# ActiveVisionLab/gaussctrl

Measured on AMD Instinct MI355X. Metric: edited views/sec @512x512 (ControlNet denoise + splat render+bwd), higher is better.
Workload: dtype bf16

## Files before the change

gaussctrl_amd/csrc/dn_gemm.hip:

```cpp
#include "dn_gemm_kernels.h"

namespace {

struct GemmVariant {
    int force_mt;
    int use8;
    int convsplit;
    bool no_wg2, no_persist, full_epilogue, no_lean_ln, tap_outer;
    int forced_pw, slice_mt, epi_abl;
    int undefined;
};
GemmVariant decode_variant(int kv)
{
    const auto bit = [kv](int b) { return (kv & b) != 0; };
    const auto field = [kv](int mask, int shift) { return (kv & mask) >> shift; };
    constexpr int flags = GC_GEMM_VAR_K4_ONLY | GC_GEMM_VAR_FORCE_K8 | GC_GEMM_VAR_NO_CONV_SLICES | GC_GEMM_VAR_NO_SMALL_CONV_SLICES | GC_GEMM_VAR_NO_WG2 |
                          GC_GEMM_VAR_NO_PERSIST | GC_GEMM_VAR_FULL_EPILOGUE | GC_GEMM_VAR_NO_LEAN_LN | GC_GEMM_VAR_TAP_OUTER;
    return {field(GC_GEMM_VAR_MT_MASK, GC_GEMM_VAR_MT_SHIFT), bit(GC_GEMM_VAR_K4_ONLY) ? 0 : bit(GC_GEMM_VAR_FORCE_K8) ? 2 : 1,
            bit(GC_GEMM_VAR_NO_CONV_SLICES) ? 0 : bit(GC_GEMM_VAR_NO_SMALL_CONV_SLICES) ? 1 : 2,
            bit(GC_GEMM_VAR_NO_WG2), bit(GC_GEMM_VAR_NO_PERSIST), bit(GC_GEMM_VAR_FULL_EPILOGUE), bit(GC_GEMM_VAR_NO_LEAN_LN), bit(GC_GEMM_VAR_TAP_OUTER),
            field(GC_GEMM_VAR_PW_MASK, GC_GEMM_VAR_PW_SHIFT), field(GC_GEMM_VAR_SLICE_MT_MASK, GC_GEMM_VAR_SLICE_MT_SHIFT), field(GC_GEMM_VAR_EPI_ABL_MASK, GC_GEMM_VAR_EPI_ABL_SHIFT),
            kv & ~(flags | GC_GEMM_VAR_MT_MASK | GC_GEMM_VAR_PW_MASK | GC_GEMM_VAR_SLICE_MT_MASK | GC_GEMM_VAR_EPI_ABL_MASK)};
}

int choose_splits(int64_t blocks, int nk)
{
    if (blocks >= 128 || nk < 32) return 1;
    int s = (int)((448 + blocks - 1) / blocks);
    if (s > nk / 8) s = nk / 8;
    if (s > 16) s = 16;
    return s < 2 ? 1 : s;
}

int choose_mt(int64_t M, int64_t N, int ntw, bool forced)
{
    const int64_t nbn = (N + 32 * ntw - 1) / (32 * ntw);
    if (((M + 127) / 128) * nbn < 96 && !forced) return 0;
    int best = 2;
    int64_t best_cost = -1;
    for (int mt = 2; mt <= 4; ++mt) {
        const int64_t tiles = ((M + 64 * mt - 1) / (64 * mt)) * nbn;
        const int64_t cost = ((tiles + 255) / 256) * (mt + 1);
        if (best_cost < 0 || cost < best_cost || (cost == best_cost && mt == 4)) { best = mt; best_cost = cost; }
    }
    return best;
}

int choose_pw(int64_t nbm, int64_t nbn, int64_t total_wgs, int conc, int64_t bm, int64_t bn, bool conv)
{
    int64_t r = total_wgs / 8 < 1 ? 1 : total_wgs / 8;
    if (r > conc) r = conc;
    const int64_t tiles = nbm * nbn;
    if (r >= tiles) return 0;
    const int64_t ca = conv ? bm : 9 * bm, cw = 9 * bn;
    int best = 0;
    int64_t best_cost = -1;
    for (int64_t pw = nbn; pw >= 1; --pw) {
        const int64_t per = nbm * pw;
        const int64_t cols = std::min<int64_t>(nbn, pw * ((r + per - 1) / per)), rows = std::min<int64_t>(nbm, (r + pw - 1) / pw);
        const int64_t cost = rows * ca + cols * cw;
        if (best_cost < 0 || cost < best_cost) { best = pw == nbn ? 0 : (int)pw; best_cost = cost; }
    }
    return best;
}

int pw_of(const gc_gemm_desc *d, const GemmVariant &v, int64_t nbm, int64_t nbn, int64_t total_wgs, int conc, int64_t bm, int64_t bn)
{
    if (v.forced_pw) return v.forced_pw - 1;
    return choose_pw(nbm, nbn, total_wgs, conc, bm, bn, d->mode == 1);
}

void plan(const gc_gemm_desc *d, int *ntw, int *splits, int *tps)
{
    *ntw = (d->N % 160 == 0 && d->N % 128 != 0 && !d->geglu) ? 5 : 4;
    if (d->softmax_keys > 0) *ntw = 5;
    const int bn = 32 * *ntw;
    const int64_t Msel = d->plan_rows > 0 ? d->plan_rows : d->M;
    const int64_t blocks = ((Msel + BM - 1) / BM) * ((d->N + bn - 1) / bn);
    const int nk = (int)((d->K + BK - 1) / BK);
    *splits = (d->geglu || d->w_set_rows > 0 || d->softmax_keys > 0) ? 1 : choose_splits(blocks, nk);
    *tps = (nk + *splits - 1) / *splits;
    *splits = (nk + *tps - 1) / *tps;
}


struct SelQ { int ntw, mt, splits, tps; };
void select_fp8(const gc_gemm_desc *d, const GemmVariant &v, SelQ *o, bool assume_ws)
{
    const int force_mt = v.force_mt;
    o->ntw = (d->N % 160 == 0 && d->N % 128 != 0 && !d->geglu) ? 5 : 4;
    int mt = force_mt ? force_mt : choose_mt(d->M, d->N, o->ntw, true);
    if (o->ntw == 5) mt = 2; else if (mt > 3) mt = 3;
    if (mt < 2) mt = 2;
    const int nkq = (int)(d->K / 128);
    o->splits = 1; o->tps = nkq;
    const bool plain = !d->geglu && !d->out_t && !d->out_fp8 && !d->out_f32 && d->out && !d->ln_row_stats && !d->out_row_stats && !d->out_group_stats && d->act == 0;
    const int64_t Msel = d->plan_rows > 0 ? d->plan_rows : d->M;
    const int64_t nbn = (d->N + 32 * o->ntw - 1) / (32 * o->ntw), tiles = ((Msel + 127) / 128) * nbn;
    if (plain && !force_mt && v.convsplit && tiles <= 128 && nkq >= 16) {
        int s = (int)std::min<int64_t>(tiles < 96 ? (256 + tiles - 1) / tiles : 256 / tiles, nkq / 8);
        if (s > 16) s = 16;
        if (s >= 2 && (assume_ws || (d->workspace && d->workspace_bytes >= sizeof(float) * (size_t)s * (size_t)d->M * (size_t)d->N))) {
            mt = 2; o->tps = (nkq + s - 1) / s; o->splits = (nkq + o->tps - 1) / o->tps;
        }
    }
    o->mt = mt;
}
}

extern "C" size_t gc_dn_gemm_workspace_bytes(const gc_gemm_desc *d)
{
    if (!d || d->M <= 0 || d->N <= 0 || d->K <= 0) return 0;
    if (d->fp8) {
        if (d->K % 128 != 0) return 0;
        const GemmVariant v = decode_variant(d->kernel_variant);
        SelQ q;
        select_fp8(d, v, &q, true);
        return q.splits > 1 ? sizeof(float) * (size_t)q.splits * (size_t)d->M * (size_t)d->N : 0;
    }
    int ntw, splits, tps;
    plan(d, &ntw, &splits, &tps);
    return splits > 1 ? sizeof(float) * (size_t)splits * (size_t)d->M * (size_t)d->N : 0;
}

namespace {
int ln_lean_kind(const gc_gemm_desc *d, const GemmVariant &v)
{
    if (v.no_lean_ln || d->fp8 || d->mode != 0 || d->K % 64 != 0 || d->out_group_stats || d->out_chan_parts || d->N < 4) return 0;
    if (d->out_row_stats && !d->ln_row_stats)
        return (!d->geglu && d->act == 0 && !d->out_f32 && !d->out_t && d->out && (!d->rowvec || d->rows_per_batch >= 256)) ? 1 : 0;
    if (d->ln_row_stats && !d->out_row_stats) return d->softmax_keys > 0 ? 3 : 2;
    return 0;
}
struct Sel { int mode, ntw, splits, tps, mt8; };
int select(const gc_gemm_desc *d, const GemmVariant &v, Sel *o, bool want_parts)
{
    int mode = 0;
    if (d->mode == 1) mode = (d->Cin % 64 == 0) ? 2 : 1;
    int ntw, splits, tps;
    plan(d, &ntw, &splits, &tps);
    if (splits > 1 && (!d->workspace || d->workspace_bytes < sizeof(float) * (size_t)splits * (size_t)d->M * (size_t)d->N)) {
        splits = 1; tps = (int)((d->K + BK - 1) / BK);
    }
    const int bn = 32 * ntw;
    const int64_t nbn = (d->N + bn - 1) / bn;
    const int nk_host = (int)((d->K + BK - 1) / BK);
    const int force_mt = v.force_mt, use8 = v.use8;
    o->mode = mode; o->ntw = ntw; o->splits = splits; o->tps = tps; o->mt8 = 0;
    if (use8 && d->zeros) {
        const int64_t Msel = d->plan_rows > 0 ? d->plan_rows : d->M;
        int mt = force_mt ? force_mt : choose_mt(Msel, d->N, ntw, use8 == 2);
        if (mt && !force_mt && Msel != d->M) mt = choose_mt(d->M, d->N, ntw, true);
        const int64_t tiles8 = ((Msel + 127) / 128) * nbn;
        const bool small = tiles8 < 96;
        if (!mt && mode == 0 && !force_mt) mt = 2;
        if (mode == 0 && !force_mt && ntw == 4 && d->K % 64 == 0 && !d->geglu && !d->out_t && !v.no_wg2 &&
            (!(d->ln_row_stats || d->out_row_stats || d->out_group_stats) || ln_lean_kind(d, v)) && !want_parts) {
            const int64_t t1 = ((d->M + 63) / 64) * nbn, t2 = ((d->M + 127) / 128) * nbn;
            if (mt == 2 && t2 <= 256 && t1 <= 512 && t1 > 128 && nk_host <= 24) mt = 1;
        }
        if (d->w_set_rows > 0 && mt) {
            int pick = 0;
            const int cand[5] = {mt, 4, 3, 2, (ntw == 4 && d->softmax_keys == 0) ? 1 : 2};
            for (int c = 0; c < 5 && !pick; ++c) if (d->w_set_rows % (64 * cand[c]) == 0) pick = cand[c];
            mt = pick ? pick : mt;
        }
        const bool want_split = !force_mt && use8 != 2 && !d->geglu && d->w_set_rows == 0 && d->softmax_keys == 0 && d->workspace && tiles8 <= 128 && (mode == 0 ? (!small || nk_host >= 24) : (v.convsplit >= (small ? 2 : 1)));
        int s8 = 1, tps8 = nk_host;
        if (want_split) {
            const bool img8 = mode != 0 && !small && d->Ho * d->Wo <= 64 && Msel % 256 == 0;
            const int mts = (v.slice_mt >= 2 && v.slice_mt <= 4) ? v.slice_mt : (img8 ? 4 : ((mode != 0 && !small) ? 3 : 2));
            const int64_t tiles_s = ((Msel + 64 * mts - 1) / (64 * mts)) * nbn;
            s8 = (int)std::min<int64_t>(std::max<int64_t>(256 / tiles_s, 2), nk_host / 12);
            if (s8 >= 2 && d->workspace_bytes >= sizeof(float) * (size_t)s8 * (size_t)d->M * (size_t)d->N) {
                mt = mts; tps8 = (nk_host + s8 - 1) / s8; s8 = (nk_host + tps8 - 1) / tps8;
            } else s8 = 1;
        }
        if (splits > 1 && s8 == 1 && !force_mt && use8 != 2) mt = 0;
        if (mt) { o->mt8 = mt; o->splits = s8; o->tps = tps8; }
    }
    return 0;
}
}

extern "C" int gc_dn_gemm_row_stat_slots(const gc_gemm_desc *d)
{
    if (!d || d->M <= 0 || d->N <= 0 || d->K <= 0) return 0;
    if (d->fp8) { const int ntw = (d->N % 160 == 0 && d->N % 128 != 0) ? 5 : 4; return (int)((d->N + 16 * ntw - 1) / (16 * ntw)); }
    const GemmVariant v = decode_variant(d->kernel_variant);
    Sel sel;
    select(d, v, &sel, false);
    return sel.splits > 1 ? (int)((d->N / 4 + 63) / 64) : (int)((d->N + 16 * sel.ntw - 1) / (16 * sel.ntw));
}

namespace {
void chan_parts_layout(const gc_gemm_desc *d, const GemmVariant &v, const Sel &sel, int64_t *rows, int *nslab, int *col_tile)
{
    *rows = 0; *nslab = 0; *col_tile = 0;
    const int64_t rpb = d->rows_per_batch;
    if (d->fp8) {
        SelQ q;
        select_fp8(d, v, &q, false);
        if (d->K % 128 != 0 || rpb < 256 || rpb % 32 != 0 || d->M % rpb != 0 || d->gn_groups < 1 || d->N % d->gn_groups != 0) return;
        const int64_t cpg = d->N / d->gn_groups;
        if (q.splits > 1) {
            if (cpg > 64) return;
            *rows = CS_RB; *nslab = (int)(rpb / CS_RB); *col_tile = 64;
            return;
        }
        const bool lean = d->mode == 1 && !d->upsample && !d->geglu && !d->out_t && !d->out_fp8 && !d->out_f32 && d->out && d->act == 0 &&
                          !d->ln_row_stats && !d->out_row_stats && !d->out_group_stats;
        const int64_t bm = 64 * q.mt;
        if (!lean || bm > rpb || cpg > 32 * q.ntw) return;
        *rows = bm;
        *nslab = (int)(rpb % bm == 0 ? rpb / bm : (rpb + bm - 1) / bm + 1);
        *col_tile = 32 * q.ntw;
        return;
    }
    if (d->geglu || d->act != 0 || d->out_t || !d->out || d->out_f32 || d->ln_row_stats || d->out_row_stats || d->out_group_stats) return;
    if (rpb < 256 || rpb % 32 != 0 || d->M % rpb != 0) return;
    if (d->gn_groups < 1 || d->N % d->gn_groups != 0) return;
    const int64_t cpg = d->N / d->gn_groups;
    if (sel.splits > 1) {
        if (cpg > 64) return;
        *rows = CS_RB; *nslab = (int)(rpb / CS_RB); *col_tile = 64;
        return;
    }
    if (!sel.mt8) return;
    if ((d->mode == 1 && d->upsample) || (d->mode == 0 && d->K % 64 != 0)) return;
    const int64_t bm = 64 * (sel.mt8 < 2 ? 2 : sel.mt8);
    if (bm > rpb || cpg > 32 * sel.ntw) return;
    *rows = bm;
    *nslab = (int)(rpb % bm == 0 ? rpb / bm : (rpb + bm - 1) / bm + 1);
    *col_tile = 32 * sel.ntw;
}
}

extern "C" int gc_dn_gemm_chan_parts_layout(const gc_gemm_desc *d, int64_t *rows_per_slab, int *nslab, int *col_tile)
{
    GC_REQUIRE(d && rows_per_slab && nslab && col_tile, "null argument");
    *rows_per_slab = 0; *nslab = 0; *col_tile = 0;
    if (d->M <= 0 || d->N <= 0 || d->K <= 0 || d->rows_per_batch <= 0) return GC_OK;
    const GemmVariant v = decode_variant(d->kernel_variant);
    Sel sel;
    select(d, v, &sel, true);
    chan_parts_layout(d, v, sel, rows_per_slab, nslab, col_tile);
    return GC_OK;
}

namespace {
struct Route { Sel sel; int lnk, persist; };
void route(const gc_gemm_desc *d, const GemmVariant &v, Route *r)
{
    Sel &sel = r->sel;
    select(d, v, &sel, d->out_chan_parts != nullptr);
    if (d->out_chan_parts && sel.mt8 == 1) sel.mt8 = 2;
    const bool fuse = d->ln_row_stats || d->out_row_stats || d->out_group_stats;
    r->lnk = (sel.mt8 && sel.splits == 1) ? ln_lean_kind(d, v) : 0;
    r->persist = 0;
    if (sel.mt8 == 4 && sel.ntw == 4 && sel.mode == 0 && sel.splits == 1 && d->K % 64 == 0 && d->K <= 64 * 24 && (!fuse || r->lnk == 2) && !d->out_chan_parts &&
        !d->rowvec && !d->out_t && !d->out_f32 && d->out && d->act != 2 && !v.no_persist) {
        const int64_t tiles = ((d->M + 255) / 256) * ((d->N + 32 * sel.ntw - 1) / (32 * sel.ntw));
        if (tiles > 256) r->persist = 256;
    }
}
}

extern "C" int gc_dn_gemm_selection(const gc_gemm_desc *d, gc_gemm_selection *out)
{
    GC_REQUIRE(d && out, "null argument");
    GC_REQUIRE(d->M > 0 && d->N > 0 && d->K > 0, "empty problem");
    const GemmVariant v = decode_variant(d->kernel_variant);
    if (const int rc = refuse_variant_bits(__func__, v.undefined)) return rc;
    *out = gc_gemm_selection{};
    int64_t rows = 0; int ns = 0, ct = 0;
    if (d->fp8) {
        GC_REQUIRE(d->K % 128 == 0, "fp8: K % 128 == 0");
        SelQ q;
        select_fp8(d, v, &q, false);
        out->kernel = GC_GEMM_SEL_FP8; out->m_tiles = q.mt; out->splits = q.splits; out->ntw = q.ntw;
        if (d->out_chan_parts) {
            chan_parts_layout(d, v, Sel{}, &rows, &ns, &ct);
            out->parts = rows > 0 ? (q.splits > 1 ? 1 : 2) : -1;
        }
        return GC_OK;
    }
    Route r;
    route(d, v, &r);
    out->kernel = !r.sel.mt8 ? GC_GEMM_SEL_K4 : r.sel.splits > 1 ? GC_GEMM_SEL_K8_SLICED : GC_GEMM_SEL_K8;
    out->m_tiles = r.sel.mt8; out->splits = r.sel.splits; out->ntw = r.sel.ntw; out->ln_kind = r.lnk; out->persist = r.persist;
    if (d->out_chan_parts) {
        chan_parts_layout(d, v, r.sel, &rows, &ns, &ct);
        out->parts = rows > 0 ? (r.sel.splits > 1 ? 1 : 2) : -1;
    }
    return GC_OK;
}

extern "C" int gc_dn_gemm(const gc_gemm_desc *d, void *stream)
{
    GC_REQUIRE(d && d->W && d->A, "null descriptor / operand");
    GC_REQUIRE(d->M > 0 && d->N > 0 && d->K > 0, "empty problem");
    GC_REQUIRE(d->K % 8 == 0, "K must be a multiple of 8 (pad channels on the host)");
    GC_REQUIRE(d->N % 4 == 0, "N must be a multiple of 4 (pad output channels on the host)");
    GC_REQUIRE(d->dtype == DT_BF16 || d->dtype == DT_F16, "dtype must be 0 (bf16) or 1 (f16)");
    const GemmVariant v = decode_variant(d->kernel_variant);
    if (const int rc = refuse_variant_bits(__func__, v.undefined)) return rc;
    GemmArgs g;
    g.pw = 0;
    g.M = d->M; g.N = d->N; g.K = d->K; g.A = d->A; g.lda = d->lda;
    g.B = d->B; g.Hi = d->Hi; g.Wi = d->Wi; g.Cin = d->Cin; g.Ho = d->Ho; g.Wo = d->Wo; g.stride = d->stride; g.ups = d->upsample; g.pad = d->pad_lo;
    g.W = d->W; g.bias = d->bias; g.rowvec = d->rowvec; g.ld_rowvec = d->ld_rowvec;
    g.rows_per_batch = d->rows_per_batch > 0 ? d->rows_per_batch : 1;
    g.residual = d->residual; g.ldr = d->ldr; g.out_scale = d->out_scale; g.act = d->act; g.geglu = d->geglu;
    g.out = d->out; g.ldc = d->ldc; g.out_f32 = d->out_f32; g.out_t = d->out_t; g.ldt = d->ldt; g.t_batch_stride = d->t_batch_stride; g.t_col0 = d->t_col0;
    g.row_stats = d->ln_row_stats; g.row_stat_slots = d->ln_row_stat_slots > 0 ? d->ln_row_stat_slots : 1;
    g.colsum = d->ln_colsum; g.ln_eps = d->ln_eps; g.ln_inv_k = 1.f / (float)d->K;
    g.out_row_stats = d->out_row_stats; g.out_group_stats = d->out_group_stats; g.gn_groups = d->gn_groups;
    g.gn_cpg = d->gn_groups > 0 ? (int)(d->N / d->gn_groups) : 1;
    g.w_scale = (const unsigned char *)d->w_scale; g.a_scale = d->a_scale;
    g.out_fp8 = d->out_fp8; g.out_qscale = d->out_fp8 > 0 ? exp2f((float)(127 - d->out_fp8)) : 1.f;
    GC_REQUIRE(d->out_fp8 >= 0 && d->out_fp8 < 255, "out_fp8 must be 0 (off) or an E8M0 byte 1 .. 254");
    GC_REQUIRE(!d->out_fp8 || (d->fp8 && d->mode == 0 && d->out && !d->out_f32 && !d->out_t && !d->out_chan_parts && !d->ln_row_stats && !d->out_row_stats &&
                               !d->out_group_stats && d->ldc % 4 == 0),
               "out_fp8: an fp8 linear with a plain output (no fp32 / transposed output, no statistics, no LayerNorm fold), ldc % 4 == 0");
    g.dbg = v.epi_abl;
    g.conv_korder = v.tap_outer ? 0 : 1;
    g.w_set_rows = d->w_set_rows; g.w_set_stride = d->w_set_stride; g.sm_keys = d->softmax_keys;
    GC_REQUIRE(d->w_set_rows >= 0 && d->softmax_keys >= 0 && d->softmax_keys <= 80, "bad weight-set / softmax arguments");
    GC_REQUIRE(!d->softmax_keys || (d->ln_row_stats && d->N % 80 == 0 && d->out && !d->out_f32 && !d->out_t && !d->geglu && !d->residual && d->act == 0),
               "softmax_keys: a LayerNorm-folded linear with N % 80 == 0 and a plain 2-byte output");
    GC_REQUIRE((d->ln_row_stats == nullptr) == (d->ln_colsum == nullptr), "ln_row_stats and ln_colsum must be given together");
    GC_REQUIRE(!d->ln_row_stats || d->mode == 0, "LayerNorm folding applies to linear GEMMs");
    GC_REQUIRE(!(d->out_row_stats || d->out_group_stats) || (!d->geglu && !d->out_t && d->out), "output statistics need a plain (non-GEGLU, non-transposed) output");
    GC_REQUIRE(!d->out_group_stats || (g.rows_per_batch % 16 == 0 && d->gn_groups >= 1 && d->gn_groups <= GS_MAXG && d->N % d->gn_groups == 0),
               "out_group_stats needs rows_per_batch % 16 == 0 and 1 <= gn_groups <= 32 dividing N");
    if (d->mode == 1) {
        GC_REQUIRE(d->Cin % 8 == 0 && d->K == 9 * (int64_t)d->Cin, "conv3x3: K must be 9*Cin with Cin % 8 == 0");
        GC_REQUIRE(d->M == (int64_t)d->B * d->Ho * d->Wo, "conv3x3: M must be B*Ho*Wo");
        GC_REQUIRE(d->pad_lo == 0 || d->pad_lo == 1, "conv3x3: pad_lo must be 0 or 1");
    } else {
        GC_REQUIRE(d->lda >= d->K && d->lda % 8 == 0, "linear: lda must be >= K and a multiple of 8");
    }
    GC_REQUIRE((d->mode == 1 ? (int64_t)d->B * d->Hi * d->Wi * d->Cin : d->M * d->lda) < ((int64_t)1 << 31) && (int64_t)d->N * d->K < ((int64_t)1 << 31),
               "operand too large for 32-bit element offsets: split the batch");
    if (d->geglu) GC_REQUIRE(d->N % 32 == 0 && !d->out_t, "geglu needs N % 32 == 0");
    GC_REQUIRE(v.force_mt <= 4, "kernel_variant: MT must be 0 .. 4");
    Route rt;
    route(d, v, &rt);
    const Sel &sel = rt.sel;
    g.chan_parts = d->out_chan_parts; g.cp_nslab = 0; g.cp_rows = 0;
    if (d->out_chan_parts) {
        int64_t rows; int ns, ct;
        chan_parts_layout(d, v, sel, &rows, &ns, &ct);
        GC_REQUIRE(rows > 0, "out_chan_parts: this problem cannot produce channel partials (see gc_dn_gemm_chan_parts_layout)");
        g.cp_nslab = ns; g.cp_rows = (int)rows;
    }
    if (fuse_of(g) && sel.mt8) {
        const bool upsampled = d->mode == 1 && d->upsample, ragged = d->mode == 0 && d->K % 64 != 0;
        GC_REQUIRE(!upsampled && !ragged, "row / group statistics and LayerNorm folding: not with upsample-fused convs or K % 64 != 0 linears");
    }
    hipStream_t s = gc::S(stream);
    g.zeros = d->zeros;
    if (d->fp8) {
        GC_REQUIRE(d->zeros && d->w_scale, "fp8: zeros page and per-row weight scales are required");
        GC_REQUIRE(d->K % 128 == 0, "fp8: K % 128 == 0");
        GC_REQUIRE(!(d->geglu || d->out_t) || (d->mode == 0 && !fuse_of(g)), "fp8: GEGLU / transposed output on linears with the plain epilogue only");
        GC_REQUIRE(d->mode == 0 || (d->Cin % 128 == 0 && !d->upsample), "fp8 conv: Cin (padded) % 128 == 0, no fused upsample");
        GC_REQUIRE(d->mode == 1 || d->lda % 16 == 0, "fp8 linear: lda % 16 == 0");
        GC_REQUIRE((int64_t)d->N * d->K < ((int64_t)1 << 31) && (d->mode == 1 ? (int64_t)d->B * d->Hi * d->Wi * d->Cin : d->M * d->lda) < ((int64_t)1 << 31), "fp8: 32-bit offsets");
        SelQ q;
        select_fp8(d, v, &q, false);
        const int ntw = q.ntw, mt = q.mt;
        g.splits = q.splits; g.tiles_per_split = q.tps; g.ws = q.splits > 1 ? (float *)d->workspace : nullptr;
        GC_REQUIRE(!d->out_chan_parts || q.splits > 1 || (d->mode == 1 && !fuse_of(g)), "fp8: channel partials come from k-sliced problems and fast convs");
        const int64_t nbn_q = (d->N + 32 * ntw - 1) / (32 * ntw), nbm_q = (d->M + 64 * mt - 1) / (64 * mt);
        const dim3 gq((unsigned)(nbm_q * nbn_q), (unsigned)q.splits);
        g.pw = pw_of(d, v, nbm_q, nbn_q, nbm_q * nbn_q * q.splits, 32, 64 * mt, 32 * ntw);
        dn_gemm_launch_fp8(g, d->dtype, d->mode == 1 ? 2 : 3, ntw, mt, gq, s);
        if (q.splits > 1) { if (g.chan_parts) dn_gemm_launch_splitk_epilogue_cs(g, d->dtype, s); else dn_gemm_launch_splitk_epilogue(g, d->dtype, s); }
        return gc::check_launch("gc_dn_gemm(fp8)");
    }
    g.splits = sel.splits; g.tiles_per_split = sel.tps; g.ws = (float *)d->workspace;
    const int bn = 32 * sel.ntw;
    const int64_t nbn = (d->N + bn - 1) / bn;
    g.persist = rt.persist;
    const int lnk = rt.lnk;
    if (d->w_set_rows > 0 || d->softmax_keys > 0) {
        GC_REQUIRE(lnk != 0, "weight sets / softmax_keys need a lean LayerNorm-fold problem (K % 64 == 0 linear with ln_row_stats or out_row_stats, no forced variant)");
        GC_REQUIRE(d->w_set_rows == 0 || (d->w_set_rows % (64 * sel.mt8) == 0 && d->M % d->w_set_rows == 0), "w_set_rows must be a multiple of the row tile and divide M");
    }
    if (sel.mt8) {
        const int64_t nbm8 = (d->M + 64 * sel.mt8 - 1) / (64 * sel.mt8);
        const dim3 grid8((unsigned)(nbm8 * nbn), (unsigned)sel.splits);
        g.pw = pw_of(d, v, nbm8, nbn, g.persist ? 8 * 32 : nbm8 * nbn * sel.splits, sel.mt8 == 1 ? 64 : 32, 64 * sel.mt8, bn);
        if (lnk) dn_gemm_launch_ln(g, d->dtype, lnk, lean_of(g, sel.mode) && g.persist == 0, sel.ntw, sel.mt8, grid8, s);
        else if (fuse_of(g)) dn_gemm_launch_fuse(g, d->dtype, sel.mode, sel.ntw, sel.mt8 < 2 ? 2 : sel.mt8, grid8, s);
        else if (g.chan_parts && sel.splits == 1) dn_gemm_launch_cs(g, d->dtype, sel.mode, sel.ntw, sel.mt8, grid8, s);
        else if (lean_of(g, sel.mode) && g.persist == 0 && !v.full_epilogue) dn_gemm_launch_lean(g, d->dtype, sel.mode, sel.ntw, sel.mt8, grid8, s);
        else dn_gemm_launch_plain(g, d->dtype, sel.mode, sel.ntw, sel.mt8, grid8, s);
    } else {
        const int64_t nbm = (d->M + BM - 1) / BM;
        const dim3 grid((unsigned)(nbm * nbn), (unsigned)sel.splits);
        g.pw = pw_of(d, v, nbm, nbn, nbm * nbn * sel.splits, 64, BM, bn);
        if (fuse_of(g)) dn_gemm_launch_fuse(g, d->dtype, sel.mode, sel.ntw, 0, grid, s); else dn_gemm_launch_plain(g, d->dtype, sel.mode, sel.ntw, 0, grid, s);
    }
    if (sel.splits > 1) { if (g.chan_parts) dn_gemm_launch_splitk_epilogue_cs(g, d->dtype, s); else dn_gemm_launch_splitk_epilogue(g, d->dtype, s); }
    return gc::check_launch("gc_dn_gemm");
}
```

gaussctrl_amd/csrc/dn_gemm_kernels.h:

```cpp
#pragma once
#include "dn_common.h"
#include <type_traits>

namespace dng {
struct GemmArgs {
    int64_t M, N, K;
    const void *A; int64_t lda;
    int B, Hi, Wi, Cin, Ho, Wo, stride, ups, pad;
    const void *W;
    const float *bias;
    const float *rowvec; int64_t ld_rowvec; int64_t rows_per_batch;
    const void *residual; int64_t ldr;
    float out_scale;
    int act, geglu;
    void *out; int64_t ldc; int out_f32;
    void *out_t; int64_t ldt; int64_t t_batch_stride; int64_t t_col0;
    int splits; int tiles_per_split;
    int persist;
    float *ws;
    const void *zeros;
    const float *row_stats; int row_stat_slots; const float *colsum; float ln_eps, ln_inv_k;
    float *out_row_stats;
    float *out_group_stats;
    int gn_groups, gn_cpg;
    const unsigned char *w_scale;
    int a_scale;
    int out_fp8; float out_qscale;
    int dbg;
    float *chan_parts; int cp_nslab; int cp_rows;
    int64_t w_set_rows, w_set_stride;
    int pw;
    int sm_keys;
    int conv_korder;
};

__device__ __forceinline__ void tile_coords(int64_t bid, int nbm, int nbn, int pw, int64_t &mblk, int64_t &nblk)
{
    if (pw <= 0 || pw >= nbn) { mblk = bid / nbn; nblk = bid % nbn; return; }
    const int64_t per = (int64_t)nbm * pw, p = bid / per, within = bid - p * per;
    const int64_t w = (nbn - p * pw) < pw ? (nbn - p * pw) : pw;
    mblk = within / w; nblk = p * pw + within % w;
}
__device__ __forceinline__ void wg_tile(const GemmArgs &g, int nbm, int nbn, int64_t &mblk, int64_t &nblk, int &slice)
{
    const int64_t tiles = gridDim.x, total = tiles * gridDim.y, lin = blockIdx.x + tiles * blockIdx.y;
    const int64_t xcd = lin & 7, qq = total >> 3, rr = total & 7;
    const int64_t L = (xcd < rr ? xcd * (qq + 1) : rr * (qq + 1) + (xcd - rr) * qq) + (lin >> 3);
    slice = (int)(L / tiles);
    tile_coords(L - (int64_t)slice * tiles, nbm, nbn, g.pw, mblk, nblk);
}
}

namespace {
using namespace dn;
using dng::GemmArgs;

template <int I, int N, class F> __device__ __forceinline__ void static_for(F &&f)
{
    if constexpr (I < N) {
        f(std::integral_constant<int, I>{});
        static_for<I + 1, N>(f);
    }
}

constexpr int BM = 128, BK = 64;
constexpr int NT = 256;


constexpr int GS_SLOTS = 20, GS_MAXG = 32;

__device__ __forceinline__ float row16_sum(float v)
{
    v += __builtin_bit_cast(float, __builtin_amdgcn_update_dpp(0, __builtin_bit_cast(int, v), 0x128, 0xf, 0xf, false));
    v += __builtin_bit_cast(float, __builtin_amdgcn_update_dpp(0, __builtin_bit_cast(int, v), 0x124, 0xf, 0xf, false));
    v += __builtin_bit_cast(float, __builtin_amdgcn_update_dpp(0, __builtin_bit_cast(int, v), 0x122, 0xf, 0xf, false));
    v += __builtin_bit_cast(float, __builtin_amdgcn_update_dpp(0, __builtin_bit_cast(int, v), 0x121, 0xf, 0xf, false));
    return v;
}

__device__ __forceinline__ int lds_off(int r, int c) { return r * 128 + ((c ^ ((r >> 1) & 7)) << 4); }

template <class T>
__device__ __forceinline__ void epilogue_store(const GemmArgs &g, int64_t m, int64_t n, int64_t on, float *v, const float *gate, const uint2 *res_pre = nullptr)
{
    const int64_t bidx = g.rowvec ? m / g.rows_per_batch : 0;
    if (g.row_stats) {
        float2 rs = make_float2(0.f, 0.f);
        for (int sl = 0; sl < g.row_stat_slots; ++sl) {
            const float2 t = *reinterpret_cast<const float2 *>(g.row_stats + ((int64_t)sl * g.M + m) * 2);
            rs.x += t.x; rs.y += t.y;
        }
        const float mean = rs.x * g.ln_inv_k, rstd = rsqrtf(fmaxf(rs.y * g.ln_inv_k - mean * mean, 0.f) + g.ln_eps);
#pragma unroll
        for (int r = 0; r < 4; ++r) v[r] = rstd * (v[r] - mean * g.colsum[n + r]);
    }
#pragma unroll
    for (int r = 0; r < 4; ++r) {
        if (g.bias) v[r] += g.bias[n + r];
        if (g.rowvec) v[r] += g.rowvec[bidx * g.ld_rowvec + n + r];
    }
    if (g.geglu) {
#pragma unroll
        for (int r = 0; r < 4; ++r) {
            float gt = gate[r];
            if (g.bias) gt += g.bias[n + 16 + r];
            v[r] = v[r] * gelu_erf(gt);
        }
    }
    if (g.act == 1) {
#pragma unroll
        for (int r = 0; r < 4; ++r) v[r] = silu(v[r]);
    } else if (g.act == 2) {
#pragma unroll
        for (int r = 0; r < 4; ++r) v[r] = fminf(fmaxf(v[r] * 0.5f + 0.5f, 0.f), 1.f);
    }
#pragma unroll
    for (int r = 0; r < 4; ++r) v[r] *= g.out_scale;
    if (g.residual) {
        const uint2 rr = res_pre ? *res_pre : *reinterpret_cast<const uint2 *>((const unsigned char *)g.residual + (m * g.ldr + on) * 2);
        v[0] += T::to_f((unsigned short)(rr.x & 0xffff)); v[1] += T::to_f((unsigned short)(rr.x >> 16));
        v[2] += T::to_f((unsigned short)(rr.y & 0xffff)); v[3] += T::to_f((unsigned short)(rr.y >> 16));
    }
    const bool to_t = g.out_t && on >= g.t_col0;
    const uint2 pk = make_uint2(pack2<T>(v[0], v[1]), pack2<T>(v[2], v[3]));
    if (g.out && !(to_t && g.t_col0 > 0)) {
        if (g.out_f32)
            *reinterpret_cast<float4 *>((float *)g.out + m * g.ldc + on) = make_float4(v[0], v[1], v[2], v[3]);
        else
            *reinterpret_cast<uint2 *>((unsigned char *)g.out + (m * g.ldc + on) * 2) = pk;
    }
    if (to_t) {
        const int64_t b = m / g.rows_per_batch, tok = m - b * g.rows_per_batch;
        unsigned short *o = (unsigned short *)g.out_t + b * g.t_batch_stride + tok;
#pragma unroll
        for (int r = 0; r < 4; ++r) o[(on - g.t_col0 + r) * g.ldt] = T::from_f(v[r]);
    }
    if (!g.out_f32) {
        v[0] = T::to_f((unsigned short)(pk.x & 0xffff)); v[1] = T::to_f((unsigned short)(pk.x >> 16));
        v[2] = T::to_f((unsigned short)(pk.y & 0xffff)); v[3] = T::to_f((unsigned short)(pk.y >> 16));
    }
}

template <int BM>
__device__ __forceinline__ void row_stats_prologue(const GemmArgs &g, int64_t m_base, float *srow)
{
    const int t = threadIdx.x, r = t & 255, half = t >> 8;
    if (t < 2 * BM) srow[t] = 0.f;
    asm volatile("s_waitcnt lgkmcnt(0)" ::: "memory");
    __builtin_amdgcn_s_barrier();
    if (r < BM) {
        const int64_t m = m_base + r < g.M ? m_base + r : g.M - 1;
        const float *rp = g.row_stats + m * 2;
        const int64_t st = g.M * 2;
        float sx = 0.f, sy = 0.f;
        int sl = half;
        for (; sl + 6 < g.row_stat_slots; sl += 8) {
            const float2 a = *reinterpret_cast<const float2 *>(rp + sl * st), b = *reinterpret_cast<const float2 *>(rp + (sl + 2) * st);
            const float2 c = *reinterpret_cast<const float2 *>(rp + (sl + 4) * st), d = *reinterpret_cast<const float2 *>(rp + (sl + 6) * st);
            sx += (a.x + b.x) + (c.x + d.x); sy += (a.y + b.y) + (c.y + d.y);
        }
        for (; sl < g.row_stat_slots; sl += 2) {
            const float2 a = *reinterpret_cast<const float2 *>(rp + sl * st);
            sx += a.x; sy += a.y;
        }
        __hip_atomic_fetch_add(srow + 2 * r, sx, __ATOMIC_RELAXED, __HIP_MEMORY_SCOPE_WORKGROUP);
        __hip_atomic_fetch_add(srow + 2 * r + 1, sy, __ATOMIC_RELAXED, __HIP_MEMORY_SCOPE_WORKGROUP);
    }
    asm volatile("s_waitcnt vmcnt(0) lgkmcnt(0)" ::: "memory");
}

template <class T, int NTW, int MT, int NTHREADS>
__device__ __forceinline__ void wave_epilogue(const GemmArgs &g, f32x4 (&acc)[NTW][MT], int64_t m_base, int64_t m_wave, int64_t n_wave, int lane,
// ... 40 lines not shown
        for (int nt = 0; nt < NTW; ++nt) {
            const int64_t n = n_lane + nt * 16;
            const bool okn = okm && n < g.N && !(g.geglu && (nt & 1));
            const int64_t on = g.geglu ? (n_wave + nt * 16) / 2 + fc * 4 : n;
            rs_all[mt][nt] = (g.residual && okn) ? *reinterpret_cast<const uint2 *>((const unsigned char *)g.residual + (mc * g.ldr + on) * 2) : make_uint2(0u, 0u);
        }
    }
    const bool want_cs = g.out_group_stats != nullptr;
    float *red = reinterpret_cast<float *>(smem);
    const int64_t b0 = want_cs ? m_base / g.rows_per_batch : 0;
    float cs[NTW][4], css[NTW][4];
#pragma unroll
    for (int nt = 0; nt < NTW; ++nt)
#pragma unroll
        for (int r = 0; r < 4; ++r) { cs[nt][r] = 0.f; css[nt][r] = 0.f; }
    int64_t cs_b = -1;
    auto flush_cs = [&]() __attribute__((always_inline)) {
        float *rb = red + (cs_b - b0) * (GS_MAXG * 2);
#pragma unroll
        for (int nt = 0; nt < NTW; ++nt) {
            const int64_t n = n_lane + nt * 16;
#pragma unroll
            for (int r = 0; r < 4; ++r) {
                const float a = (g.dbg & 4) ? cs[nt][r] : row16_sum(cs[nt][r]), b = (g.dbg & 4) ? css[nt][r] : row16_sum(css[nt][r]);
                if (fr == 0 && n + r < g.N && !(g.dbg & 2)) {
                    const int gi = (int)(n + r) / g.gn_cpg;
                    __hip_atomic_fetch_add(rb + 2 * gi, a, __ATOMIC_RELAXED, __HIP_MEMORY_SCOPE_WORKGROUP);
                    __hip_atomic_fetch_add(rb + 2 * gi + 1, b, __ATOMIC_RELAXED, __HIP_MEMORY_SCOPE_WORKGROUP);
                }
                cs[nt][r] = 0.f; css[nt][r] = 0.f;
            }
        }
    };
#pragma unroll
    for (int mt = 0; mt < MT; ++mt) {
        const int64_t m = m_wave + mt * 16 + fr;
        const int64_t m_tile = m_wave + mt * 16;
        if (m_tile >= g.M) break;
        const bool okm = m < g.M;
        if (want_cs) {
            const int64_t b = m_tile / g.rows_per_batch;
            if (cs_b >= 0 && b != cs_b) flush_cs();
            cs_b = b;
        }
        const uint2 *rs = rs_all[mt];
        float mean = 0.f, rstd = 1.f;
        if (g.row_stats) {
            float sx = 0.f, sy = 0.f;
            if (srow) {
                const float2 t = *reinterpret_cast<const float2 *>(srow + 2 * (okm ? (int)(m - m_base) : 0));
                sx = t.x; sy = t.y;
            } else {
                const float *rp = g.row_stats + (okm ? m : 0) * 2;
                for (int sl = 0; sl < g.row_stat_slots; ++sl) {
                    const float2 t = *reinterpret_cast<const float2 *>(rp + (int64_t)sl * g.M * 2);
                    sx += t.x; sy += t.y;
                }
            }
            mean = sx * g.ln_inv_k;
            rstd = rsqrtf(fmaxf(sy * g.ln_inv_k - mean * mean, 0.f) + g.ln_eps);
        }
        float4 rv[NTW];
        const int64_t bidx = (g.rowvec && okm) ? m / g.rows_per_batch : 0;
#pragma unroll
        for (int nt = 0; nt < NTW; ++nt) {
            const int64_t n = n_lane + nt * 16;
            rv[nt] = (g.rowvec && n < g.N) ? *reinterpret_cast<const float4 *>(g.rowvec + bidx * g.ld_rowvec + n) : make_float4(0.f, 0.f, 0.f, 0.f);
        }
        float rsum = 0.f, rsq = 0.f;
#pragma unroll
        for (int nt = 0; nt < NTW; ++nt) {
            const int64_t n = n_lane + nt * 16;
            if (n >= g.N) continue;
            if (g.geglu && (nt & 1)) continue;
            float a0 = acc[nt][mt][0], a1 = acc[nt][mt][1], a2 = acc[nt][mt][2], a3 = acc[nt][mt][3];
            if (g.row_stats) {
                a0 = rstd * (a0 - mean * csm[nt].x); a1 = rstd * (a1 - mean * csm[nt].y);
                a2 = rstd * (a2 - mean * csm[nt].z); a3 = rstd * (a3 - mean * csm[nt].w);
            }
            float v[4] = {a0 + bia[nt].x + rv[nt].x, a1 + bia[nt].y + rv[nt].y, a2 + bia[nt].z + rv[nt].z, a3 + bia[nt].w + rv[nt].w};
            int64_t on = n;
            if (g.geglu) {
                constexpr int NP = NTW - 1;
                const int np = nt + 1 < NTW ? nt + 1 : NP;
                float g0 = acc[np][mt][0], g1 = acc[np][mt][1], g2 = acc[np][mt][2], g3 = acc[np][mt][3];
                if (g.row_stats) {
                    g0 = rstd * (g0 - mean * csm[np].x); g1 = rstd * (g1 - mean * csm[np].y);
                    g2 = rstd * (g2 - mean * csm[np].z); g3 = rstd * (g3 - mean * csm[np].w);
                }
                v[0] *= gelu_erf(g0 + bia[np].x); v[1] *= gelu_erf(g1 + bia[np].y);
                v[2] *= gelu_erf(g2 + bia[np].z); v[3] *= gelu_erf(g3 + bia[np].w);
                on = (n_wave + nt * 16) / 2 + fc * 4;
            }
            if (g.act == 1) {
#pragma unroll
                for (int r = 0; r < 4; ++r) v[r] = silu(v[r]);
            } else if (g.act == 2) {
#pragma unroll
                for (int r = 0; r < 4; ++r) v[r] = fminf(fmaxf(v[r] * 0.5f + 0.5f, 0.f), 1.f);
            }
#pragma unroll
            for (int r = 0; r < 4; ++r) v[r] *= g.out_scale;
            if (g.residual) {
                v[0] += T::to_f((unsigned short)(rs[nt].x & 0xffff)); v[1] += T::to_f((unsigned short)(rs[nt].x >> 16));
                v[2] += T::to_f((unsigned short)(rs[nt].y & 0xffff)); v[3] += T::to_f((unsigned short)(rs[nt].y >> 16));
            }
            if (!okm) continue;
            const bool to_t = g.out_t && on >= g.t_col0;
            const uint2 pk = make_uint2(pack2<T>(v[0], v[1]), pack2<T>(v[2], v[3]));
            if (g.out && !(to_t && g.t_col0 > 0)) {
                if (g.out_f32)
                    *reinterpret_cast<float4 *>((float *)g.out + m * g.ldc + on) = make_float4(v[0], v[1], v[2], v[3]);
                else
                    *reinterpret_cast<uint2 *>((unsigned char *)g.out + (m * g.ldc + on) * 2) = pk;
            }
            if (to_t) {
                const int64_t b = m / g.rows_per_batch, tok = m - b * g.rows_per_batch;
                unsigned short *o = (unsigned short *)g.out_t + b * g.t_batch_stride + tok;
#pragma unroll
                for (int r = 0; r < 4; ++r) o[(on - g.t_col0 + r) * g.ldt] = T::from_f(v[r]);
            }
            if (g.out_row_stats || want_cs) {
                float t[4];
                if (g.out_f32) { t[0] = v[0]; t[1] = v[1]; t[2] = v[2]; t[3] = v[3]; }
                else {
                    t[0] = T::to_f((unsigned short)(pk.x & 0xffff)); t[1] = T::to_f((unsigned short)(pk.x >> 16));
                    t[2] = T::to_f((unsigned short)(pk.y & 0xffff)); t[3] = T::to_f((unsigned short)(pk.y >> 16));
                }
#pragma unroll
                for (int r = 0; r < 4; ++r) {
                    rsum += t[r]; rsq += t[r] * t[r];
                    cs[nt][r] += t[r]; css[nt][r] += t[r] * t[r];
                }
            }
        }
        if (g.out_row_stats && n_wave < g.N) {
            rsum += __shfl_xor(rsum, 16, 64); rsq += __shfl_xor(rsq, 16, 64);
            rsum += __shfl_xor(rsum, 32, 64); rsq += __shfl_xor(rsq, 32, 64);
            const int64_t slot = n_wave / (16 * NTW);
            if (fc == 0 && okm) *reinterpret_cast<float2 *>(g.out_row_stats + (slot * g.M + m) * 2) = make_float2(rsum, rsq);
        }
    }
    if (want_cs) {
        if (cs_b >= 0) flush_cs();
        asm volatile("s_waitcnt lgkmcnt(0)" ::: "memory");
        __builtin_amdgcn_s_barrier();
        for (int idx = threadIdx.x; idx < GS_SLOTS * GS_MAXG * 2; idx += NTHREADS) {
            const float v = red[idx];
            if (v != 0.f && !(g.dbg & 1)) {
                const int sl = idx / (GS_MAXG * 2), rem = idx - sl * (GS_MAXG * 2);
                unsafeAtomicAdd(g.out_group_stats + ((b0 + sl) * g.gn_groups) * 2 + rem, v);
            }
        }
    }
}

template <class T, int MODE, int NTW, bool FUSE>
__global__ __launch_bounds__(NT, 2) void k_gemm(const GemmArgs g)
{
    constexpr int BN = 32 * NTW;
    constexpr int WCH = BN * 8 / NT;
    constexpr int STAGE = BM * 128 + BN * 128;
    extern __shared__ __attribute__((aligned(16))) unsigned char smem[];
    const int tid = threadIdx.x, lane = tid & 63, wid = tid >> 6;
    const int wm = wid >> 1, wn = wid & 1;
    const int nbn = (int)((g.N + BN - 1) / BN);
    int64_t mblk, nblk;
    int slice;
    wg_tile(g, (int)((g.M + BM - 1) / BM), nbn, mblk, nblk, slice);
    const int64_t m_base = mblk * BM, n_base = nblk * BN;
    const int nk = (int)((g.K + BK - 1) / BK);
    const int kt0 = slice * g.tiles_per_split, kt1 = min(nk, kt0 + g.tiles_per_split);
    if (kt0 >= kt1) return;

    int a_row[4], a_chunk[4];
    int a_off[4];
    int a_y[4], a_x[4];
    bool a_ok[4];
    int w_off[WCH];
    bool w_ok[WCH];
#pragma unroll
    for (int i = 0; i < 4; ++i) {
        const int q = tid + NT * i;
        a_row[i] = q >> 3; a_chunk[i] = q & 7;
        const int64_t m = m_base + a_row[i];
        a_ok[i] = m < g.M;
        const int mm = a_ok[i] ? (int)m : 0;
        if (MODE != 0) {
            const int hw = g.Ho * g.Wo;
            const int b = mm / hw;
            const int rem = mm - b * hw;
            const int oy = rem / g.Wo;
            a_y[i] = oy * g.stride - g.pad; a_x[i] = (rem - oy * g.Wo) * g.stride - g.pad;
            a_off[i] = b * g.Hi * g.Wi * g.Cin + (MODE == 2 ? a_chunk[i] * 8 : 0);
            if (MODE == 2 && !g.ups) a_off[i] += (a_y[i] * g.Wi + a_x[i]) * g.Cin;
        } else {
            a_off[i] = mm * (int)g.lda + a_chunk[i] * 8;
            a_y[i] = a_x[i] = 0;
        }
    }
#pragma unroll
    for (int i = 0; i < WCH; ++i) {
        const int q = tid + NT * i;
        const int64_t n = n_base + (q >> 3);
        w_ok[i] = n < g.N;
        w_off[i] = (w_ok[i] ? (int)n : 0) * (int)g.K + (q & 7) * 8;
    }
    const int Hin = g.ups ? g.Hi * 2 : g.Hi, Win = g.ups ? g.Wi * 2 : g.Wi;
    const unsigned char *Ab = (const unsigned char *)g.A, *Wb = (const unsigned char *)g.W;
    const int ktl = kt1 - 1;
    int ld_tap = 0, ld_ci = 0;
    if (MODE == 2) { ld_tap = (kt0 * BK) / g.Cin; ld_ci = kt0 * BK - ld_tap * g.Cin; }

    auto load_tile = [&](int kt, uint4 *ra, uint4 *rw, unsigned &mask) __attribute__((always_inline)) {
        const int kb = kt * BK;
        int dy_u = 0, dx_u = 0, tap_off = 0;
        if (MODE == 2) {
            dy_u = ld_tap / 3; dx_u = ld_tap - dy_u * 3;
            tap_off = g.ups ? ld_ci : (dy_u * g.Wi + dx_u) * g.Cin + ld_ci;
            if (kt < ktl) { ld_ci += BK; if (ld_ci >= g.Cin) { ld_ci -= g.Cin; ++ld_tap; } }
        }
        unsigned mk = 0;
#pragma unroll
        for (int i = 0; i < 4; ++i) {
            bool ok;
            int off;
            if (MODE == 2) {
                int yi = a_y[i] + dy_u, xi = a_x[i] + dx_u;
                ok = a_ok[i] && (unsigned)yi < (unsigned)Hin && (unsigned)xi < (unsigned)Win;
                off = a_off[i] + tap_off;
                if (g.ups) off += ((yi >> 1) * g.Wi + (xi >> 1)) * g.Cin;
            } else if (MODE == 1) {
                const int k0 = kb + a_chunk[i] * 8;
                const int kc = k0 < (int)g.K ? k0 : 0;
                const int tap = kc / g.Cin;
                const int ci = kc - tap * g.Cin;
                const int dy = tap / 3, dx = tap - dy * 3;
                int yi = a_y[i] + dy, xi = a_x[i] + dx;
                ok = a_ok[i] && k0 < (int)g.K && (unsigned)yi < (unsigned)Hin && (unsigned)xi < (unsigned)Win;
                if (g.ups) { yi >>= 1; xi >>= 1; }
                off = a_off[i] + (yi * g.Wi + xi) * g.Cin + ci;
            } else {
                ok = a_ok[i] && (kb + a_chunk[i] * 8) < (int)g.K;
                off = a_off[i] + kb;
            }
            ra[i] = *reinterpret_cast<const uint4 *>(Ab + (size_t)(unsigned)((ok ? off : 0) * 2));
            mk |= (ok ? 1u : 0u) << i;
        }
#pragma unroll
        for (int i = 0; i < WCH; ++i) {
            const int q = tid + NT * i;
            const bool ok = w_ok[i] && (kb + (q & 7) * 8) < (int)g.K;
            rw[i] = *reinterpret_cast<const uint4 *>(Wb + (size_t)(unsigned)((ok ? w_off[i] + kb : 0) * 2));
            mk |= (ok ? 1u : 0u) << (8 + i);
        }
        mask = mk;
    };
    constexpr unsigned FULL = 0xFu | (((1u << WCH) - 1u) << 8);
    int sa_off[4], sw_off[WCH];
#pragma unroll
    for (int i = 0; i < 4; ++i) sa_off[i] = lds_off(a_row[i], a_chunk[i]);
#pragma unroll
    for (int i = 0; i < WCH; ++i) { const int q = tid + NT * i; sw_off[i] = BM * 128 + lds_off(q >> 3, q & 7); }
    auto store_tile = [&](int buf, uint4 *ra, uint4 *rw, unsigned mask) __attribute__((always_inline)) {
        unsigned char *sa = smem + buf * STAGE;
        if (!__all(mask == FULL)) {
#pragma unroll
            for (int i = 0; i < 4; ++i) {
                const unsigned km = 0u - ((mask >> i) & 1u);
                ra[i] = make_uint4(ra[i].x & km, ra[i].y & km, ra[i].z & km, ra[i].w & km);
            }
#pragma unroll
            for (int i = 0; i < WCH; ++i) {
                const unsigned km = 0u - ((mask >> (8 + i)) & 1u);
                rw[i] = make_uint4(rw[i].x & km, rw[i].y & km, rw[i].z & km, rw[i].w & km);
            }
        }
#pragma unroll
        for (int i = 0; i < 4; ++i) *reinterpret_cast<uint4 *>(sa + sa_off[i]) = ra[i];
#pragma unroll
        for (int i = 0; i < WCH; ++i) *reinterpret_cast<uint4 *>(sa + sw_off[i]) = rw[i];
    };

    f32x4 acc[NTW][4];
#pragma unroll
    for (int a = 0; a < NTW; ++a)
#pragma unroll
        for (int b = 0; b < 4; ++b) acc[a][b] = f32x4{0.f, 0.f, 0.f, 0.f};
    const int fr = lane & 15, fc = lane >> 4;
    const int swz = (fr >> 1) & 7;
    const int fx0 = ((fc ^ swz) << 4), fx1 = (((fc + 4) ^ swz) << 4);
    const int aw0 = BM * 128 + (wn * (16 * NTW) + fr) * 128, aa0 = (wm * 64 + fr) * 128;
    auto compute = [&](int buf) __attribute__((always_inline)) {
        const unsigned char *sb = smem + buf * STAGE;
#pragma unroll
        for (int ks = 0; ks < 2; ++ks) {
            const int fx = ks ? fx1 : fx0;
            uint4 fw[NTW], fa[4];
#pragma unroll
            for (int t = 0; t < NTW; ++t) fw[t] = *reinterpret_cast<const uint4 *>(sb + aw0 + fx + t * 2048);
#pragma unroll
            for (int t = 0; t < 4; ++t) fa[t] = *reinterpret_cast<const uint4 *>(sb + aa0 + fx + t * 2048);
#pragma unroll
            for (int nt = 0; nt < NTW; ++nt)
#pragma unroll
                for (int mt = 0; mt < 4; ++mt) acc[nt][mt] = T::mfma(fw[nt], fa[mt], acc[nt][mt]);
        }
    };

    uint4 raA[4], rwA[WCH], raB[4], rwB[WCH];
    unsigned mkA = 0, mkB = 0;
    load_tile(kt0, raA, rwA, mkA);
    load_tile(min(kt0 + 1, ktl), raB, rwB, mkB);
    store_tile(0, raA, rwA, mkA);
    __syncthreads();
    for (int kt = kt0; kt < kt1; kt += 2) {
        load_tile(min(kt + 2, ktl), raA, rwA, mkA);
        compute(0);
        store_tile(1, raB, rwB, mkB);
        __syncthreads();
        if (kt + 1 >= kt1) break;
        load_tile(min(kt + 3, ktl), raB, rwB, mkB);
        compute(1);
        store_tile(0, raA, rwA, mkA);
        __syncthreads();
    }

    if constexpr (FUSE) {
        wave_epilogue<T, NTW, 4, NT>(g, acc, m_base, m_base + wm * 64, n_base + wn * (16 * NTW), lane, smem, nullptr, slice);
        return;
    }
    const int64_t n_lane = n_base + wn * (16 * NTW) + fc * 4;
    if (g.splits > 1) {
#pragma unroll
        for (int mt = 0; mt < 4; ++mt) {
            const int64_t m = m_base + wm * 64 + mt * 16 + fr;
            if (m >= g.M) continue;
#pragma unroll
            for (int nt = 0; nt < NTW; ++nt) {
                const int64_t n = n_lane + nt * 16;
                if (n < g.N)
                    *reinterpret_cast<float4 *>(g.ws + ((int64_t)slice * g.M + m) * g.N + n) =
                        make_float4(acc[nt][mt][0], acc[nt][mt][1], acc[nt][mt][2], acc[nt][mt][3]);
            }
        }
        return;
    }
    float4 bia[NTW];
#pragma unroll
    for (int nt = 0; nt < NTW; ++nt) {
        const int64_t n = n_lane + nt * 16;
        bia[nt] = (g.bias && n < g.N) ? *reinterpret_cast<const float4 *>(g.bias + n) : make_float4(0.f, 0.f, 0.f, 0.f);
    }
    uint2 rs_all[4][NTW];
#pragma unroll
    for (int mt = 0; mt < 4; ++mt) {
        const int64_t m = m_base + wm * 64 + mt * 16 + fr;
        const bool okm = m < g.M;
        const int64_t mc = okm ? m : 0;
#pragma unroll
        for (int nt = 0; nt < NTW; ++nt) {
            const int64_t n = n_lane + nt * 16;
            const bool okn = okm && n < g.N && !(g.geglu && (nt & 1));
            const int64_t on = g.geglu ? (n_base + wn * (16 * NTW) + nt * 16) / 2 + fc * 4 : n;
            rs_all[mt][nt] = (g.residual && okn) ? *reinterpret_cast<const uint2 *>((const unsigned char *)g.residual + (mc * g.ldr + on) * 2) : make_uint2(0u, 0u);
        }
    }
#pragma unroll
    for (int mt = 0; mt < 4; ++mt) {
        const int64_t m = m_base + wm * 64 + mt * 16 + fr;
        if (m >= g.M) continue;
        const uint2 *rs = rs_all[mt];
        float4 rv[NTW];
        const int64_t bidx = g.rowvec ? m / g.rows_per_batch : 0;
#pragma unroll
        for (int nt = 0; nt < NTW; ++nt) {
            const int64_t n = n_lane + nt * 16;
            rv[nt] = (g.rowvec && n < g.N) ? *reinterpret_cast<const float4 *>(g.rowvec + bidx * g.ld_rowvec + n) : make_float4(0.f, 0.f, 0.f, 0.f);
        }
#pragma unroll
        for (int nt = 0; nt < NTW; ++nt) {
            const int64_t n = n_lane + nt * 16;
            if (n >= g.N) continue;
            if (g.geglu && (nt & 1)) continue;
            float v[4] = {acc[nt][mt][0] + bia[nt].x + rv[nt].x, acc[nt][mt][1] + bia[nt].y + rv[nt].y,
                          acc[nt][mt][2] + bia[nt].z + rv[nt].z, acc[nt][mt][3] + bia[nt].w + rv[nt].w};
            int64_t on = n;
            if (g.geglu) {
                constexpr int NP = NTW - 1;
                const int np = nt + 1 < NTW ? nt + 1 : NP;
                v[0] *= gelu_erf(acc[np][mt][0] + bia[np].x); v[1] *= gelu_erf(acc[np][mt][1] + bia[np].y);
                v[2] *= gelu_erf(acc[np][mt][2] + bia[np].z); v[3] *= gelu_erf(acc[np][mt][3] + bia[np].w);
                on = (n_base + wn * (16 * NTW) + nt * 16) / 2 + fc * 4;
            }
            if (g.act == 1) {
#pragma unroll
                for (int r = 0; r < 4; ++r) v[r] = silu(v[r]);
            } else if (g.act == 2) {
#pragma unroll
                for (int r = 0; r < 4; ++r) v[r] = fminf(fmaxf(v[r] * 0.5f + 0.5f, 0.f), 1.f);
            }
#pragma unroll
            for (int r = 0; r < 4; ++r) v[r] *= g.out_scale;
            if (g.residual) {
                v[0] += T::to_f((unsigned short)(rs[nt].x & 0xffff)); v[1] += T::to_f((unsigned short)(rs[nt].x >> 16));
                v[2] += T::to_f((unsigned short)(rs[nt].y & 0xffff)); v[3] += T::to_f((unsigned short)(rs[nt].y >> 16));
            }
            const bool to_t = g.out_t && on >= g.t_col0;
            if (g.out && !(to_t && g.t_col0 > 0)) {
                if (g.out_f32)
                    *reinterpret_cast<float4 *>((float *)g.out + m * g.ldc + on) = make_float4(v[0], v[1], v[2], v[3]);
                else
                    *reinterpret_cast<uint2 *>((unsigned char *)g.out + (m * g.ldc + on) * 2) = make_uint2(pack2<T>(v[0], v[1]), pack2<T>(v[2], v[3]));
            }
            if (to_t) {
                const int64_t b = m / g.rows_per_batch, tok = m - b * g.rows_per_batch;
                unsigned short *o = (unsigned short *)g.out_t + b * g.t_batch_stride + tok;
#pragma unroll
                for (int r = 0; r < 4; ++r) o[(on - g.t_col0 + r) * g.ldt] = T::from_f(v[r]);
            }
        }
    }
}

__device__ __forceinline__ void glds16(const void *gsrc, unsigned lds_dst)
{
    unsigned keep;
    asm volatile("s_mov_b32 %0, m0\n\ts_mov_b32 m0, %2\n\ts_nop 0\n\tglobal_load_lds_dwordx4 %1, off\n\ts_mov_b32 m0, %0"
                 : "=&s"(keep) : "v"(gsrc), "s"(lds_dst) : "memory");
}

__device__ __forceinline__ void glds16_s(const void *sbase, unsigned voff, unsigned lds_dst)
{
    asm volatile("s_mov_b32 m0, %2\n\ts_nop 0\n\tglobal_load_lds_dwordx4 %0, %1" :: "v"(voff), "s"(sbase), "s"(lds_dst) : "memory");
}

template <class T, int MODE, int NTW, int MT, bool FUSE, bool CS = false, bool LEAN_ = false, int LNV = 0>
__global__ __launch_bounds__(512, MT <= 2 ? 2 : 1) void k_gemm8(const GemmArgs g)
{
    static_assert(!(FUSE && CS), "one statistics epilogue at a time");
    static_assert(LNV == 0 || (!FUSE && !CS && MODE == 3), "lean LayerNorm fold: K % 64 == 0 linears on the non-FUSE epilogues");
    static_assert(LNV != 1 || LEAN_, "row partials come from the lean epilogue");
    static_assert(LNV != 3 || (NTW == 5 && !LEAN_), "softmax-heads epilogue: one 80-column head block per wave column");
    constexpr bool LNIN = LNV >= 2;
    constexpr bool LEAN = LEAN_ || CS;
    constexpr int BM = 64 * MT;
    constexpr bool CONVF = MODE == 2 || MODE == 4, UPS = MODE == 4;
    constexpr int BN = 32 * NTW;
    constexpr int STAGE = BM * 128 + BN * 128;
    constexpr int NS = 3;
    constexpr int AG = BM / 8, WG = BN / 8;
    constexpr int AI = AG / 8, WI = (WG + 7) / 8;
    extern __shared__ __attribute__((aligned(16))) unsigned char smem[];
    const int tid = threadIdx.x, lane = tid & 63;
    const int wid = __builtin_amdgcn_readfirstlane(tid >> 6);
    const int wm = wid >> 1, wn = wid & 1;
    const int nbn = (int)((g.N + BN - 1) / BN);
    int64_t mblk, nblk;
    int slice;
    wg_tile(g, (int)((g.M + BM - 1) / BM), nbn, mblk, nblk, slice);
    const int64_t m_base = mblk * BM, n_base = nblk * BN;
    const int nk_all = (int)((g.K + BK - 1) / BK);
    const int kt0 = slice * g.tiles_per_split;
    const int nk = min(nk_all, kt0 + g.tiles_per_split) - kt0;
    const unsigned lds0 = (unsigned)(size_t)(__attribute__((address_space(3))) unsigned char *)smem;
    float *srow = reinterpret_cast<float *>(smem + NS * STAGE);
    if constexpr (FUSE) {
        if (g.row_stats && g.splits == 1) row_stats_prologue<BM>(g, m_base, srow);
    }
    float *ctab = reinterpret_cast<float *>(smem + NS * STAGE);
    if constexpr (CS) {
        for (int i = tid; i < 4 * BN; i += 512) ctab[i] = 0.f;
    }

    const int lr = lane >> 3, ls = lane & 7;
    int a_off[AI], a_y[AI], a_x[AI], a_ck[AI];
    bool a_ok[AI];
#pragma unroll
    for (int i = 0; i < AI; ++i) {
        const int row = (wid + 8 * i) * 8 + lr;
        a_ck[i] = ls ^ ((row >> 1) & 7);
        const int64_t m = m_base + row;
        a_ok[i] = m < g.M;
        const int mm = a_ok[i] ? (int)m : 0;
        if (MODE == 1 || CONVF) {
            const int hw = g.Ho * g.Wo;
            const int b = mm / hw;
            const int rem = mm - b * hw;
            const int oy = rem / g.Wo;
            a_y[i] = oy * g.stride - g.pad; a_x[i] = (rem - oy * g.Wo) * g.stride - g.pad;
            a_off[i] = b * g.Hi * g.Wi * g.Cin + (CONVF ? a_ck[i] * 8 : 0);
            if (MODE == 2) a_off[i] += (a_y[i] * g.Wi + a_x[i]) * g.Cin;
        } else {
            a_off[i] = mm * (int)g.lda + a_ck[i] * 8;
            if (MODE == 3) a_off[i] = (int)(m < g.M ? m : g.M - 1) * (int)g.lda + a_ck[i] * 8;
            a_y[i] = a_x[i] = 0;
        }
    }
// ... 53 lines not shown
    };
    auto issue_a = [&](const TileSrc &t, int i) __attribute__((always_inline)) {
        const unsigned dst = t.sbase + (unsigned)((wid + 8 * i) * 1024);
        if (MODE == 3) { glds16_s(Ab + (size_t)t.kb * 2, (unsigned)(a_off[i] * 2), dst); return; }
        if (MODE == 2) {
            const bool okm = (a_vm[i] >> t.tap) & 1u;
            glds16(okm ? a_ptr[i] + (int64_t)t.tap_off * 2 : Zp, dst);
            return;
        }
        bool ok;
        int off;
        if (MODE == 4) {
            int yi = a_y[i] + t.dy_u, xi = a_x[i] + t.dx_u;
            ok = a_ok[i] && (unsigned)yi < (unsigned)Hin && (unsigned)xi < (unsigned)Win;
            off = a_off[i] + t.tap_off;
            off += ((yi >> 1) * g.Wi + (xi >> 1)) * g.Cin;
        } else if (MODE == 1) {
            const int k0 = t.kb + a_ck[i] * 8;
            const int kc = k0 < (int)g.K ? k0 : 0;
            const int tap = kc / g.Cin;
            const int ci = kc - tap * g.Cin;
            const int dy = tap / 3, dx = tap - dy * 3;
            int yi = a_y[i] + dy, xi = a_x[i] + dx;
            ok = a_ok[i] && k0 < (int)g.K && (unsigned)yi < (unsigned)Hin && (unsigned)xi < (unsigned)Win;
            if (g.ups) { yi >>= 1; xi >>= 1; }
            off = a_off[i] + (yi * g.Wi + xi) * g.Cin + ci;
        } else {
            ok = a_ok[i] && (t.kb + a_ck[i] * 8) < (int)g.K;
            off = a_off[i] + t.kb;
        }
        const unsigned char *src = ok ? Ab + (size_t)(unsigned)(off * 2) : Zp;
        glds16(src, dst);
    };
    auto issue_w = [&](const TileSrc &t, int i, bool has) __attribute__((always_inline)) {
        if (has) {
            const unsigned dst = t.sbase + (unsigned)(BM * 128 + (wid + 8 * i) * 1024);
            if (MODE == 3 || CONVF) { glds16_s(Wb + (size_t)t.kb * 2, (unsigned)(w_off[i] * 2), dst); return; }
            const bool ok = w_ok[i] && (t.kb + w_ck[i] * 8) < (int)g.K;
            const unsigned char *src = ok ? Wb + (size_t)(unsigned)((w_off[i] + t.kb) * 2) : Zp;
            glds16(src, dst);
        }
    };
    auto issue = [&](int kt, int stage) __attribute__((always_inline)) {
        const TileSrc t = issue_begin(kt, stage);
#pragma unroll
        for (int i = 0; i < AI; ++i) issue_a(t, i);
#pragma unroll
        for (int i = 0; i < WI; ++i) issue_w(t, i, wid + 8 * i < WG);
    };

    f32x4 acc[NTW][MT];
#pragma unroll
    for (int a = 0; a < NTW; ++a)
#pragma unroll
        for (int b = 0; b < MT; ++b) acc[a][b] = f32x4{0.f, 0.f, 0.f, 0.f};
    const int fr = lane & 15, fc = lane >> 4;
    const int swz = (fr >> 1) & 7;
    const int fx0 = ((fc ^ swz) << 4), fx1 = (((fc + 4) ^ swz) << 4);
    const int aw0 = BM * 128 + (wn * (16 * NTW) + fr) * 128, aa0 = (wm * (16 * MT) + fr) * 128;
    struct Frag { uint4 w[NTW], a[MT]; };
    auto load_frag = [&](Frag &f, int stage, int ks) __attribute__((always_inline)) {
        const unsigned char *sb = smem + stage * STAGE;
        const int fx = ks ? fx1 : fx0;
#pragma unroll
        for (int t = 0; t < NTW; ++t) f.w[t] = *reinterpret_cast<const uint4 *>(sb + aw0 + fx + t * 2048);
#pragma unroll
        for (int t = 0; t < MT; ++t) f.a[t] = *reinterpret_cast<const uint4 *>(sb + aa0 + fx + t * 2048);
    };
    constexpr int NMM = NTW * MT, NPC = AI + WI;
    auto block = [&](const Frag &f, Frag &fn, int st_next, int ks_next, bool load_next, const TileSrc &t, auto dma_tag, auto w3_tag) __attribute__((always_inline)) {
        constexpr bool DMA = decltype(dma_tag)::value, W3 = decltype(w3_tag)::value;
        static_for<0, NMM>([&](auto m_) __attribute__((always_inline)) {
            constexpr int m = decltype(m_)::value, nt = m / MT, mt = m % MT;
            acc[nt][mt] = T::mfma(f.w[nt], f.a[mt], acc[nt][mt]);
            if constexpr (m == 0) {
                __builtin_amdgcn_sched_barrier(0);
                if (load_next) load_frag(fn, st_next, ks_next);
                __builtin_amdgcn_sched_barrier(0);
            } else if constexpr (DMA && m >= 2) {
                static_for<0, NPC>([&](auto p_) __attribute__((always_inline)) {
                    constexpr int pp = decltype(p_)::value;
                    if constexpr (m == 2 + (pp * (NMM - 3)) / NPC) {
                        __builtin_amdgcn_sched_barrier(0);
                        if constexpr (pp < AI) issue_a(t, pp); else issue_w(t, pp - AI, (pp - AI) < WI - 1 || W3 || WG % 8 == 0);
                        __builtin_amdgcn_sched_barrier(0);
                    }
                });
            }
        });
    };

    const bool w3 = (wid + 8 * (WI - 1)) < WG;
    Frag f0, f1;
    const TileSrc tnone = {0, 0, 0, 0, 0, 0u};
    auto run = [&](auto w3_tag) __attribute__((always_inline)) {
        constexpr bool W3 = decltype(w3_tag)::value;
        constexpr int GRPW = AI + ((W3 || WG % 8 == 0) ? WI : WI - 1);
        static_assert(2 * GRPW < 64, "vmcnt range");
        auto wait_tiles = [&](auto n_) __attribute__((always_inline)) {
            asm volatile("s_waitcnt vmcnt(%0)" ::"n"(decltype(n_)::value * GRPW) : "memory");
        };
        issue(0, 0);
        if (nk > 1) issue(1, 1);
        if (nk > 2) issue(2, 2);
        if constexpr (LNIN) row_stats_prologue<BM>(g, m_base, srow);
        if (nk > 2) wait_tiles(std::integral_constant<int, 2>{}); else if (nk > 1) wait_tiles(std::integral_constant<int, 1>{}); else wait_tiles(std::integral_constant<int, 0>{});
        __builtin_amdgcn_s_barrier();
        load_frag(f0, 0, 0);
        int st = 0, kt = 0;
        for (; kt + 3 < nk; ++kt) {
            const int st1 = st + 1 == NS ? 0 : st + 1;
            block(f0, f1, st, 1, true, tnone, std::false_type{}, w3_tag);
            wait_tiles(std::integral_constant<int, 1>{});
            asm volatile("s_waitcnt lgkmcnt(0)" ::: "memory");
            __builtin_amdgcn_s_barrier();
            const TileSrc t = issue_begin(kt + 3, st);
            block(f1, f0, st1, 0, true, t, std::true_type{}, w3_tag);
            st = st1;
        }
        for (; kt < nk; ++kt) {
            const int st1 = st + 1 == NS ? 0 : st + 1;
            block(f0, f1, st, 1, true, tnone, std::false_type{}, w3_tag);
            if (kt + 1 < nk) {
                if (kt + 2 < nk) wait_tiles(std::integral_constant<int, 1>{}); else wait_tiles(std::integral_constant<int, 0>{});
                asm volatile("s_waitcnt lgkmcnt(0)" ::: "memory");
                __builtin_amdgcn_s_barrier();
                block(f1, f0, st1, 0, true, tnone, std::false_type{}, w3_tag);
            } else {
                block(f1, f0, st1, 0, false, tnone, std::false_type{}, w3_tag);
            }
            st = st1;
        }
    };
    if (w3) run(std::true_type{}); else run(std::false_type{});

    if constexpr (FUSE) {
        wave_epilogue<T, NTW, MT, 512>(g, acc, m_base, m_base + wm * (16 * MT), n_base + wn * (16 * NTW), lane, smem,
                                       (g.row_stats && g.splits == 1) ? srow : nullptr, slice);
        return;
    }
    const int64_t n_lane = n_base + wn * (16 * NTW) + fc * 4;
    if (g.splits > 1) {
#pragma unroll
        for (int mt = 0; mt < MT; ++mt) {
            const int64_t m = m_base + wm * (16 * MT) + mt * 16 + fr;
            if (m >= g.M) continue;
#pragma unroll
            for (int nt = 0; nt < NTW; ++nt) {
                const int64_t n = n_lane + nt * 16;
                if (n < g.N)
                    *reinterpret_cast<float4 *>(g.ws + ((int64_t)slice * g.M + m) * g.N + n) =
                        make_float4(acc[nt][mt][0], acc[nt][mt][1], acc[nt][mt][2], acc[nt][mt][3]);
            }
        }
        return;
    }
    if constexpr (LNV == 3) {
        const float *biasp = g.bias + wset * g.N, *csp = g.colsum + wset * g.N;
        float4 bia[NTW], csm[NTW];
#pragma unroll
        for (int nt = 0; nt < NTW; ++nt) {
            const int64_t n = n_lane + nt * 16, nc = n < g.N ? n : g.N - 4;
            bia[nt] = *reinterpret_cast<const float4 *>(biasp + nc);
            csm[nt] = *reinterpret_cast<const float4 *>(csp + nc);
        }
#pragma unroll
        for (int mt = 0; mt < MT; ++mt) {
            const int64_t m = m_base + wm * (16 * MT) + mt * 16 + fr;
            const float2 st = *reinterpret_cast<const float2 *>(srow + 2 * (wm * (16 * MT) + mt * 16 + fr));
            const float mean = st.x * g.ln_inv_k, rstd = rsqrtf(fmaxf(st.y * g.ln_inv_k - mean * mean, 0.f) + g.ln_eps);
            float v[NTW][4];
            float mx = -3.0e38f;
#pragma unroll
            for (int nt = 0; nt < NTW; ++nt) {
                v[nt][0] = rstd * (acc[nt][mt][0] - mean * csm[nt].x) + bia[nt].x; v[nt][1] = rstd * (acc[nt][mt][1] - mean * csm[nt].y) + bia[nt].y;
                v[nt][2] = rstd * (acc[nt][mt][2] - mean * csm[nt].z) + bia[nt].z; v[nt][3] = rstd * (acc[nt][mt][3] - mean * csm[nt].w) + bia[nt].w;
#pragma unroll
                for (int r = 0; r < 4; ++r) {
                    const bool key = nt * 16 + fc * 4 + r < g.sm_keys;
                    v[nt][r] = key ? v[nt][r] : -3.0e38f;
                    mx = fmaxf(mx, v[nt][r]);
                }
            }
            mx = fmaxf(mx, __shfl_xor(mx, 16, 64)); mx = fmaxf(mx, __shfl_xor(mx, 32, 64));
            float sum = 0.f;
#pragma unroll
            for (int nt = 0; nt < NTW; ++nt)
#pragma unroll
                for (int r = 0; r < 4; ++r) { v[nt][r] = exp2f(v[nt][r] - mx); sum += v[nt][r]; }
            sum += __shfl_xor(sum, 16, 64); sum += __shfl_xor(sum, 32, 64);
            const float inv = 1.f / sum;
#pragma unroll
            for (int nt = 0; nt < NTW; ++nt) {
                const int64_t n = n_lane + nt * 16;
                if (m < g.M && n < g.N)
                    *reinterpret_cast<uint2 *>((unsigned char *)g.out + (m * g.ldc + n) * 2) =
                        make_uint2(pack2<T>(v[nt][0] * inv, v[nt][1] * inv), pack2<T>(v[nt][2] * inv, v[nt][3] * inv));
            }
        }
        return;
    }
    if constexpr (LEAN) {
        const unsigned char *zp = (const unsigned char *)g.zeros;
        const bool has_b = g.bias != nullptr, has_rv = g.rowvec != nullptr, has_res = g.residual != nullptr;
        const float *biasp = has_b ? g.bias + (LNV != 0 ? wset * g.N : 0) : reinterpret_cast<const float *>(zp);
        const float *rvp = has_rv ? g.rowvec : reinterpret_cast<const float *>(zp);
        const unsigned char *resp = has_res ? (const unsigned char *)g.residual : zp;
        const int64_t bA = m_base / g.rows_per_batch, b_last = (g.M - 1) / g.rows_per_batch;
        const int64_t bB = bA + 1 < b_last ? bA + 1 : b_last;
        const int64_t m_rv = (bA + 1) * g.rows_per_batch;
        float4 bia[NTW], rvA[NTW], rvB[NTW];
        uint2 rs[MT][NTW];
#pragma unroll
        for (int nt = 0; nt < NTW; ++nt) {
            const int64_t n = n_lane + nt * 16, nc = n < g.N ? n : g.N - 4;
            bia[nt] = *reinterpret_cast<const float4 *>(biasp + (has_b ? nc : 0));
            rvA[nt] = *reinterpret_cast<const float4 *>(rvp + (has_rv ? bA * g.ld_rowvec + nc : 0));
            rvB[nt] = *reinterpret_cast<const float4 *>(rvp + (has_rv ? bB * g.ld_rowvec + nc : 0));
        }
#pragma unroll
        for (int mt = 0; mt < MT; ++mt) {
            const int64_t m = m_base + wm * (16 * MT) + mt * 16 + fr, mc = m < g.M ? m : g.M - 1;
#pragma unroll
            for (int nt = 0; nt < NTW; ++nt) {
                const int64_t n = n_lane + nt * 16, nc = n < g.N ? n : g.N - 4;
                rs[mt][nt] = *reinterpret_cast<const uint2 *>(resp + (has_res ? (mc * g.ldr + nc) * 2 : 0));
            }
        }
        float4 csm[LNV == 2 ? NTW : 1];
        if constexpr (LNV == 2) {
#pragma unroll
            for (int nt = 0; nt < NTW; ++nt) {
                const int64_t n = n_lane + nt * 16, nc = n < g.N ? n : g.N - 4;
                csm[nt] = *reinterpret_cast<const float4 *>(g.colsum + wset * g.N + nc);
            }
        }
        uint2 pks[CS ? MT : 1][CS ? NTW : 1];
#pragma unroll
        for (int mt = 0; mt < MT; ++mt) {
            const int64_t m = m_base + wm * (16 * MT) + mt * 16 + fr;
            const bool second = m >= m_rv;
            float mean = 0.f, rstd = 1.f;
            if constexpr (LNV == 2) {
                const float2 st = *reinterpret_cast<const float2 *>(srow + 2 * (wm * (16 * MT) + mt * 16 + fr));
                mean = st.x * g.ln_inv_k;
                rstd = rsqrtf(fmaxf(st.y * g.ln_inv_k - mean * mean, 0.f) + g.ln_eps);
            }
            float rsum = 0.f, rsq = 0.f;
#pragma unroll
            for (int nt = 0; nt < NTW; ++nt) {
                const int64_t n = n_lane + nt * 16;
                const float4 rv = second ? rvB[nt] : rvA[nt];
                float a0 = acc[nt][mt][0], a1 = acc[nt][mt][1], a2 = acc[nt][mt][2], a3 = acc[nt][mt][3];
                if constexpr (LNV == 2) {
                    a0 = rstd * (a0 - mean * csm[nt].x); a1 = rstd * (a1 - mean * csm[nt].y);
                    a2 = rstd * (a2 - mean * csm[nt].z); a3 = rstd * (a3 - mean * csm[nt].w);
                }
                float v[4] = {a0 + bia[nt].x + rv.x, a1 + bia[nt].y + rv.y, a2 + bia[nt].z + rv.z, a3 + bia[nt].w + rv.w};
#pragma unroll
                for (int r = 0; r < 4; ++r) v[r] *= g.out_scale;
                v[0] += T::to_f((unsigned short)(rs[mt][nt].x & 0xffff)); v[1] += T::to_f((unsigned short)(rs[mt][nt].x >> 16));
                v[2] += T::to_f((unsigned short)(rs[mt][nt].y & 0xffff)); v[3] += T::to_f((unsigned short)(rs[mt][nt].y >> 16));
                const uint2 pk = make_uint2(pack2<T>(v[0], v[1]), pack2<T>(v[2], v[3]));
                const bool ok = m < g.M && n < g.N;
                if (ok) *reinterpret_cast<uint2 *>((unsigned char *)g.out + (m * g.ldc + n) * 2) = pk;
                if constexpr (CS) pks[mt][nt] = ok ? pk : make_uint2(0u, 0u);
                if constexpr (LNV == 1) {
                    const float w_ = n < g.N ? 1.f : 0.f;
                    const float t0 = w_ * T::to_f((unsigned short)(pk.x & 0xffff)), t1 = w_ * T::to_f((unsigned short)(pk.x >> 16));
                    const float t2 = w_ * T::to_f((unsigned short)(pk.y & 0xffff)), t3 = w_ * T::to_f((unsigned short)(pk.y >> 16));
                    rsum += (t0 + t1) + (t2 + t3); rsq += (t0 * t0 + t1 * t1) + (t2 * t2 + t3 * t3);
                }
            }
            if constexpr (LNV == 1) {
                rsum += __shfl_xor(rsum, 16, 64); rsq += __shfl_xor(rsq, 16, 64);
                rsum += __shfl_xor(rsum, 32, 64); rsq += __shfl_xor(rsq, 32, 64);
                const int64_t slot = (n_base + wn * (16 * NTW)) / (16 * NTW);
                if (fc == 0 && m < g.M && n_base + wn * (16 * NTW) < g.N)
                    *reinterpret_cast<float2 *>(g.out_row_stats + (slot * g.M + m) * 2) = make_float2(rsum, rsq);
            }
        }
        if constexpr (CS) {
            const int64_t m_split = (m_base / g.rows_per_batch + 1) * g.rows_per_batch;
            const int64_t m_end = m_base + BM < g.M ? m_base + BM : g.M;
            const int npass = m_split < m_end ? 2 : 1;
    #pragma unroll 1
            for (int pass = 0; pass < npass; ++pass) {
                float cs[NTW][4], cq[NTW][4];
    #pragma unroll
                for (int nt = 0; nt < NTW; ++nt)
    #pragma unroll
                    for (int r = 0; r < 4; ++r) { cs[nt][r] = 0.f; cq[nt][r] = 0.f; }
    #pragma unroll
                for (int mt = 0; mt < MT; ++mt) {
                    const int64_t m_tile = m_base + wm * (16 * MT) + mt * 16;
                    const float wgt = ((m_tile >= m_split ? 1 : 0) == pass) ? 1.f : 0.f;
    #pragma unroll
                    for (int nt = 0; nt < NTW; ++nt) {
                        const uint2 pk = pks[mt][nt];
                        const float t0 = wgt != 0.f ? T::to_f((unsigned short)(pk.x & 0xffff)) : 0.f, t1 = wgt != 0.f ? T::to_f((unsigned short)(pk.x >> 16)) : 0.f;
                        const float t2 = wgt != 0.f ? T::to_f((unsigned short)(pk.y & 0xffff)) : 0.f, t3 = wgt != 0.f ? T::to_f((unsigned short)(pk.y >> 16)) : 0.f;
                        cs[nt][0] += t0; cq[nt][0] += t0 * t0; cs[nt][1] += t1; cq[nt][1] += t1 * t1;
                        cs[nt][2] += t2; cq[nt][2] += t2 * t2; cs[nt][3] += t3; cq[nt][3] += t3 * t3;
                    }
                }
                float *tb = ctab + (pass * BN + wn * (16 * NTW) + fc * 4) * 2;
// ... 391 lines not shown
        w_off[i] = (int)(n < g.N ? n : g.N - 1) * (int)g.K + (ls ^ ((row >> 1) & 7)) * 16;
    }
    const unsigned char *Ab = (const unsigned char *)g.A, *Wb = (const unsigned char *)g.W, *Zp = (const unsigned char *)g.zeros;
    const bool tap_inner = MODE == 2 && g.conv_korder != 0;
    int ld_tap = 0, ld_ci = 0;
    if (MODE == 2) {
        if (tap_inner) { ld_tap = k0 % 9; ld_ci = (k0 / 9) * BKB; }
        else { ld_tap = (k0 * BKB) / g.Cin; ld_ci = (k0 * BKB) % g.Cin; }
    }
    struct TileSrc { int kb, tap, tap_off; unsigned sbase; };
    auto issue_begin = [&](int kt, int stage) __attribute__((always_inline)) -> TileSrc {
        TileSrc t;
        t.kb = (k0 + kt) * BKB; t.tap = 0; t.tap_off = 0;
        if (MODE == 2) {
            t.tap = ld_tap;
            t.kb = __builtin_amdgcn_readfirstlane(ld_tap * g.Cin + ld_ci);
            const int dy = ld_tap / 3, dx = ld_tap - dy * 3;
            t.tap_off = (dy * g.Wi + dx) * g.Cin + ld_ci;
            if (tap_inner) { if (++ld_tap == 9) { ld_tap = 0; ld_ci += BKB; } }
            else { ld_ci += BKB; if (ld_ci >= g.Cin) { ld_ci -= g.Cin; ++ld_tap; } }
        }
        t.sbase = lds0 + stage * STAGE;
        return t;
    };
    auto issue_a = [&](const TileSrc &t, int i) __attribute__((always_inline)) {
        const unsigned dst = t.sbase + (unsigned)((wid + 8 * i) * 1024);
        if (MODE == 3) { glds16_s(Ab + (size_t)t.kb, (unsigned)a_off[i], dst); return; }
        const bool okm = (a_vm[i] >> t.tap) & 1u;
        glds16(okm ? a_ptr[i] + (int64_t)t.tap_off : Zp, dst);
    };
    auto issue_w = [&](const TileSrc &t, int i, bool has) __attribute__((always_inline)) {
        if (has) glds16_s(Wb + (size_t)t.kb, (unsigned)w_off[i], t.sbase + (unsigned)(BM * 128 + (wid + 8 * i) * 1024));
    };
    auto issue = [&](int kt, int stage) __attribute__((always_inline)) {
        const TileSrc t = issue_begin(kt, stage);
#pragma unroll
        for (int i = 0; i < AI; ++i) issue_a(t, i);
#pragma unroll
        for (int i = 0; i < WI; ++i) issue_w(t, i, wid + 8 * i < WG);
    };

    f32x4 acc[NTW][MT];
#pragma unroll
    for (int a = 0; a < NTW; ++a)
#pragma unroll
        for (int b = 0; b < MT; ++b) acc[a][b] = f32x4{0.f, 0.f, 0.f, 0.f};
    const int fr = lane & 15, fc = lane >> 4;
    const int swz = (fr >> 1) & 7;
    const int fx0 = ((fc ^ swz) << 4), fx1 = (((fc + 4) ^ swz) << 4);
    const int aw0 = BM * 128 + (wn * (16 * NTW) + fr) * 128, aa0 = (wm * (16 * MT) + fr) * 128;
    typedef __attribute__((ext_vector_type(4))) int i32x4;
    struct Frag { i32x8 w[NTW], a[MT]; };
    auto ld32 = [&](const unsigned char *p0, const unsigned char *p1) __attribute__((always_inline)) -> i32x8 {
        const i32x4 lo = *reinterpret_cast<const i32x4 *>(p0), hi = *reinterpret_cast<const i32x4 *>(p1);
        return __builtin_shufflevector(lo, hi, 0, 1, 2, 3, 4, 5, 6, 7);
    };
    auto load_frag = [&](Frag &f, int stage) __attribute__((always_inline)) {
        const unsigned char *sb = smem + stage * STAGE;
#pragma unroll
        for (int t = 0; t < NTW; ++t) f.w[t] = ld32(sb + aw0 + fx0 + t * 2048, sb + aw0 + fx1 + t * 2048);
#pragma unroll
        for (int t = 0; t < MT; ++t) f.a[t] = ld32(sb + aa0 + fx0 + t * 2048, sb + aa0 + fx1 + t * 2048);
    };
    int sw[NTW];
#pragma unroll
    for (int t = 0; t < NTW; ++t) {
        const int64_t n = n_base + wn * (16 * NTW) + t * 16 + fr;
        sw[t] = g.w_scale[n < g.N ? n : g.N - 1];
    }
    asm volatile("s_waitcnt vmcnt(0)" ::: "memory");
#pragma unroll
    for (int t = 0; t < NTW; ++t) asm volatile("" : "+v"(sw[t]));
    const int sa = g.a_scale;
    constexpr int NMM = NTW * MT, NPC = AI + WI;
    auto block = [&](const Frag &f, Frag &fn, int st_next, bool load_next, const TileSrc &t, auto dma_tag, auto w3_tag) __attribute__((always_inline)) {
        constexpr bool DMA = decltype(dma_tag)::value, W3 = decltype(w3_tag)::value;
        static_for<0, NMM>([&](auto m_) __attribute__((always_inline)) {
            constexpr int m = decltype(m_)::value, nt = m / MT, mt = m % MT;
            acc[nt][mt] = __builtin_amdgcn_mfma_scale_f32_16x16x128_f8f6f4(f.w[nt], f.a[mt], acc[nt][mt], 0, 0, 0, sw[nt], 0, sa);
            if constexpr (m == 0) {
                __builtin_amdgcn_sched_barrier(0);
                if (load_next) load_frag(fn, st_next);
                __builtin_amdgcn_sched_barrier(0);
            } else if constexpr (DMA && m >= 2) {
                static_for<0, NPC>([&](auto p_) __attribute__((always_inline)) {
                    constexpr int pp = decltype(p_)::value;
                    if constexpr (m == 2 + (pp * (NMM - 3)) / NPC) {
                        __builtin_amdgcn_sched_barrier(0);
                        if constexpr (pp < AI) issue_a(t, pp); else issue_w(t, pp - AI, (pp - AI) < WI - 1 || W3 || WG % 8 == 0);
                        __builtin_amdgcn_sched_barrier(0);
                    }
                });
            }
        });
    };
    const bool w3 = (wid + 8 * (WI - 1)) < WG;
    Frag f0, f1;
    const TileSrc tnone = {0, 0, 0, 0u};
    auto run = [&](auto w3_tag) __attribute__((always_inline)) {
        constexpr bool W3 = decltype(w3_tag)::value;
        constexpr int GRPW = AI + ((W3 || WG % 8 == 0) ? WI : WI - 1);
        auto wait_tiles = [&](auto n_) __attribute__((always_inline)) {
            asm volatile("s_waitcnt vmcnt(%0)" ::"n"(decltype(n_)::value * GRPW) : "memory");
        };
        issue(0, 0);
        if (nk > 1) issue(1, 1);
        if (nk > 2) issue(2, 2);
        if (nk > 2) wait_tiles(std::integral_constant<int, 2>{}); else if (nk > 1) wait_tiles(std::integral_constant<int, 1>{}); else wait_tiles(std::integral_constant<int, 0>{});
        __builtin_amdgcn_s_barrier();
        load_frag(f0, 0);
        int st = 0, kt = 0;
        auto step = [&](Frag &fc_, Frag &fn_) __attribute__((always_inline)) {
            const int st1 = st + 1 == NS ? 0 : st + 1;
            if (kt + 3 < nk) {
                wait_tiles(std::integral_constant<int, 1>{});
                asm volatile("s_waitcnt lgkmcnt(0)" ::: "memory");
                __builtin_amdgcn_s_barrier();
                const TileSrc t = issue_begin(kt + 3, st);
                block(fc_, fn_, st1, true, t, std::true_type{}, w3_tag);
            } else if (kt + 1 < nk) {
                if (kt + 2 < nk) wait_tiles(std::integral_constant<int, 1>{}); else wait_tiles(std::integral_constant<int, 0>{});
                asm volatile("s_waitcnt lgkmcnt(0)" ::: "memory");
                __builtin_amdgcn_s_barrier();
                block(fc_, fn_, st1, true, tnone, std::false_type{}, w3_tag);
            } else {
                block(fc_, fn_, st1, false, tnone, std::false_type{}, w3_tag);
            }
            st = st1; ++kt;
        };
        while (kt < nk) {
            step(f0, f1);
            if (kt < nk) step(f1, f0);
        }
    };
    if (w3) run(std::true_type{}); else run(std::false_type{});
    if constexpr (FUSE) {
        wave_epilogue<T, NTW, MT, 512>(g, acc, m_base, m_base + wm * (16 * MT), n_base + wn * (16 * NTW), lane, smem, g.row_stats ? srow : nullptr, slice);
        return;
    }
    const int64_t n_lane = n_base + wn * (16 * NTW) + fc * 4;
    if (g.splits > 1) {
#pragma unroll
        for (int mt = 0; mt < MT; ++mt) {
            const int64_t m = m_base + wm * (16 * MT) + mt * 16 + fr;
            if (m >= g.M) continue;
#pragma unroll
            for (int nt = 0; nt < NTW; ++nt) {
                const int64_t n = n_lane + nt * 16;
                if (n < g.N)
                    *reinterpret_cast<float4 *>(g.ws + ((int64_t)slice * g.M + m) * g.N + n) =
                        make_float4(acc[nt][mt][0], acc[nt][mt][1], acc[nt][mt][2], acc[nt][mt][3]);
            }
        }
        return;
    }
    if constexpr (CS) {
        const unsigned char *zp = (const unsigned char *)g.zeros;
        const bool has_b = g.bias != nullptr, has_rv = g.rowvec != nullptr, has_res = g.residual != nullptr;
        const float *biasp = has_b ? g.bias : reinterpret_cast<const float *>(zp);
        const float *rvp = has_rv ? g.rowvec : reinterpret_cast<const float *>(zp);
        const unsigned char *resp = has_res ? (const unsigned char *)g.residual : zp;
        const int64_t bA = m_base / g.rows_per_batch, b_last = (g.M - 1) / g.rows_per_batch;
        const int64_t bB = bA + 1 < b_last ? bA + 1 : b_last;
        const int64_t m_rv = (bA + 1) * g.rows_per_batch;
        float4 bia[NTW], rvA[NTW], rvB[NTW];
        uint2 rs[MT][NTW];
#pragma unroll
        for (int nt = 0; nt < NTW; ++nt) {
            const int64_t n = n_lane + nt * 16, nc = n < g.N ? n : g.N - 4;
            bia[nt] = *reinterpret_cast<const float4 *>(biasp + (has_b ? nc : 0));
            rvA[nt] = *reinterpret_cast<const float4 *>(rvp + (has_rv ? bA * g.ld_rowvec + nc : 0));
            rvB[nt] = *reinterpret_cast<const float4 *>(rvp + (has_rv ? bB * g.ld_rowvec + nc : 0));
        }
#pragma unroll
        for (int mt = 0; mt < MT; ++mt) {
            const int64_t m = m_base + wm * (16 * MT) + mt * 16 + fr, mc = m < g.M ? m : g.M - 1;
#pragma unroll
            for (int nt = 0; nt < NTW; ++nt) {
                const int64_t n = n_lane + nt * 16, nc = n < g.N ? n : g.N - 4;
                rs[mt][nt] = *reinterpret_cast<const uint2 *>(resp + (has_res ? (mc * g.ldr + nc) * 2 : 0));
            }
        }
        uint2 pks[MT][NTW];
#pragma unroll
        for (int mt = 0; mt < MT; ++mt) {
            const int64_t m = m_base + wm * (16 * MT) + mt * 16 + fr;
            const bool second = m >= m_rv;
#pragma unroll
            for (int nt = 0; nt < NTW; ++nt) {
                const int64_t n = n_lane + nt * 16;
                const float4 rv = second ? rvB[nt] : rvA[nt];
                float v[4] = {acc[nt][mt][0] + bia[nt].x + rv.x, acc[nt][mt][1] + bia[nt].y + rv.y,
                              acc[nt][mt][2] + bia[nt].z + rv.z, acc[nt][mt][3] + bia[nt].w + rv.w};
#pragma unroll
                for (int r = 0; r < 4; ++r) v[r] *= g.out_scale;
                v[0] += T::to_f((unsigned short)(rs[mt][nt].x & 0xffff)); v[1] += T::to_f((unsigned short)(rs[mt][nt].x >> 16));
                v[2] += T::to_f((unsigned short)(rs[mt][nt].y & 0xffff)); v[3] += T::to_f((unsigned short)(rs[mt][nt].y >> 16));
                const uint2 pk = make_uint2(pack2<T>(v[0], v[1]), pack2<T>(v[2], v[3]));
                const bool ok = m < g.M && n < g.N;
                if (ok) *reinterpret_cast<uint2 *>((unsigned char *)g.out + (m * g.ldc + n) * 2) = pk;
                pks[mt][nt] = ok ? pk : make_uint2(0u, 0u);
            }
        }
        {
            const int64_t m_split = (m_base / g.rows_per_batch + 1) * g.rows_per_batch;
            const int64_t m_end = m_base + BM < g.M ? m_base + BM : g.M;
            const int npass = m_split < m_end ? 2 : 1;
    #pragma unroll 1
            for (int pass = 0; pass < npass; ++pass) {
                float cs[NTW][4], cq[NTW][4];
    #pragma unroll
                for (int nt = 0; nt < NTW; ++nt)
    #pragma unroll
                    for (int r = 0; r < 4; ++r) { cs[nt][r] = 0.f; cq[nt][r] = 0.f; }
    #pragma unroll
                for (int mt = 0; mt < MT; ++mt) {
                    const int64_t m_tile = m_base + wm * (16 * MT) + mt * 16;
                    const float wgt = ((m_tile >= m_split ? 1 : 0) == pass) ? 1.f : 0.f;
    #pragma unroll
                    for (int nt = 0; nt < NTW; ++nt) {
                        const uint2 pk = pks[mt][nt];
                        const float t0 = wgt != 0.f ? T::to_f((unsigned short)(pk.x & 0xffff)) : 0.f, t1 = wgt != 0.f ? T::to_f((unsigned short)(pk.x >> 16)) : 0.f;
                        const float t2 = wgt != 0.f ? T::to_f((unsigned short)(pk.y & 0xffff)) : 0.f, t3 = wgt != 0.f ? T::to_f((unsigned short)(pk.y >> 16)) : 0.f;
                        cs[nt][0] += t0; cq[nt][0] += t0 * t0; cs[nt][1] += t1; cq[nt][1] += t1 * t1;
                        cs[nt][2] += t2; cq[nt][2] += t2 * t2; cs[nt][3] += t3; cq[nt][3] += t3 * t3;
                    }
                }
                float *tb = ctab + (pass * BN + wn * (16 * NTW) + fc * 4) * 2;
    #pragma unroll
                for (int nt = 0; nt < NTW; ++nt)
    #pragma unroll
                    for (int r = 0; r < 4; ++r) {
                        const float sa = row16_sum(cs[nt][r]), sb = row16_sum(cq[nt][r]);
                        if (fr == 0) {
                            __hip_atomic_fetch_add(tb + (nt * 16 + r) * 2, sa, __ATOMIC_RELAXED, __HIP_MEMORY_SCOPE_WORKGROUP);
                            __hip_atomic_fetch_add(tb + (nt * 16 + r) * 2 + 1, sb, __ATOMIC_RELAXED, __HIP_MEMORY_SCOPE_WORKGROUP);
                        }
                    }
            }
            asm volatile("s_waitcnt lgkmcnt(0)" ::: "memory");
            __builtin_amdgcn_s_barrier();
            const int64_t b0 = m_base / g.rows_per_batch;
            const int cpg = g.gn_cpg, G = (int)(g.N / cpg);
            const int n_hi = (int)(n_base + BN < g.N ? n_base + BN : g.N);
            const int g_first = (int)n_base / cpg, ng = (n_hi - 1) / cpg - g_first + 1;
            for (int i = tid; i < 2 * ng; i += 512) {
                const int slot = i >= ng ? 1 : 0, gg = g_first + i - slot * ng;
                if (slot == 1 && !(m_split < m_end)) continue;
                const int c_lo = gg * cpg > (int)n_base ? gg * cpg : (int)n_base, c_hi = (gg + 1) * cpg < n_hi ? (gg + 1) * cpg : n_hi;
                float s1 = 0.f, s2 = 0.f;
                for (int c = c_lo; c < c_hi; ++c) { const float2 t = *reinterpret_cast<const float2 *>(ctab + (slot * BN + c - (int)n_base) * 2); s1 += t.x; s2 += t.y; }
                const int64_t b = b0 + slot;
                const int64_t slab = mblk - (b * g.rows_per_batch) / BM;
                const int half = gg * cpg < (int)n_base ? 1 : 0;
                *reinterpret_cast<float2 *>(g.chan_parts + ((((b * g.cp_nslab + slab) * G + gg) * 2 + half) * 2)) = make_float2(s1, s2);
            }
        }
        return;
    }
    float4 bia[NTW];
#pragma unroll
    for (int nt = 0; nt < NTW; ++nt) {
        const int64_t n = n_lane + nt * 16;
        bia[nt] = (g.bias && n < g.N) ? *reinterpret_cast<const float4 *>(g.bias + n) : make_float4(0.f, 0.f, 0.f, 0.f);
    }
#pragma unroll
    for (int mt = 0; mt < MT; ++mt) {
        const int64_t m = m_base + wm * (16 * MT) + mt * 16 + fr;
        if (m >= g.M) continue;
        float4 rv[NTW];
        uint2 rs[NTW];
        const int64_t bidx = g.rowvec ? m / g.rows_per_batch : 0;
#pragma unroll
        for (int nt = 0; nt < NTW; ++nt) {
            const int64_t n = n_lane + nt * 16;
            const bool okn = n < g.N && !(g.geglu && (nt & 1));
            const int64_t on = g.geglu ? (n_base + wn * (16 * NTW) + nt * 16) / 2 + fc * 4 : n;
            rv[nt] = (g.rowvec && n < g.N) ? *reinterpret_cast<const float4 *>(g.rowvec + bidx * g.ld_rowvec + n) : make_float4(0.f, 0.f, 0.f, 0.f);
            rs[nt] = (g.residual && okn) ? *reinterpret_cast<const uint2 *>((const unsigned char *)g.residual + (m * g.ldr + on) * 2) : make_uint2(0u, 0u);
        }
#pragma unroll
        for (int nt = 0; nt < NTW; ++nt) {
            const int64_t n = n_lane + nt * 16;
            if (n >= g.N) continue;
            if (g.geglu && (nt & 1)) continue;
            float v[4] = {acc[nt][mt][0] + bia[nt].x + rv[nt].x, acc[nt][mt][1] + bia[nt].y + rv[nt].y,
                          acc[nt][mt][2] + bia[nt].z + rv[nt].z, acc[nt][mt][3] + bia[nt].w + rv[nt].w};
            int64_t on = n;
            if (g.geglu) {
                constexpr int NP = NTW - 1;
                const int np = nt + 1 < NTW ? nt + 1 : NP;
                v[0] *= gelu_erf(acc[np][mt][0] + bia[np].x); v[1] *= gelu_erf(acc[np][mt][1] + bia[np].y);
                v[2] *= gelu_erf(acc[np][mt][2] + bia[np].z); v[3] *= gelu_erf(acc[np][mt][3] + bia[np].w);
                on = (n_base + wn * (16 * NTW) + nt * 16) / 2 + fc * 4;
            }
            if (g.act == 1) {
#pragma unroll
                for (int r = 0; r < 4; ++r) v[r] = silu(v[r]);
            } else if (g.act == 2) {
#pragma unroll
                for (int r = 0; r < 4; ++r) v[r] = fminf(fmaxf(v[r] * 0.5f + 0.5f, 0.f), 1.f);
            }
#pragma unroll
            for (int r = 0; r < 4; ++r) v[r] *= g.out_scale;
            if (g.residual) {
                v[0] += T::to_f((unsigned short)(rs[nt].x & 0xffff)); v[1] += T::to_f((unsigned short)(rs[nt].x >> 16));
                v[2] += T::to_f((unsigned short)(rs[nt].y & 0xffff)); v[3] += T::to_f((unsigned short)(rs[nt].y >> 16));
            }
            const bool to_t = g.out_t && on >= g.t_col0;
            if (g.out_fp8) {
                const float q0 = fminf(fmaxf(v[0] * g.out_qscale, -448.f), 448.f), q1 = fminf(fmaxf(v[1] * g.out_qscale, -448.f), 448.f);
                const float q2 = fminf(fmaxf(v[2] * g.out_qscale, -448.f), 448.f), q3 = fminf(fmaxf(v[3] * g.out_qscale, -448.f), 448.f);
                int w8 = 0;
                w8 = __builtin_amdgcn_cvt_pk_fp8_f32(q0, q1, w8, false); w8 = __builtin_amdgcn_cvt_pk_fp8_f32(q2, q3, w8, true);
                *reinterpret_cast<int *>((unsigned char *)g.out + m * g.ldc + on) = w8;
            } else if (g.out && !(to_t && g.t_col0 > 0)) {
                if (g.out_f32)
                    *reinterpret_cast<float4 *>((float *)g.out + m * g.ldc + on) = make_float4(v[0], v[1], v[2], v[3]);
                else
                    *reinterpret_cast<uint2 *>((unsigned char *)g.out + (m * g.ldc + on) * 2) = make_uint2(pack2<T>(v[0], v[1]), pack2<T>(v[2], v[3]));
            }
            if (to_t) {
                const int64_t b = m / g.rows_per_batch, tok = m - b * g.rows_per_batch;
                unsigned short *o = (unsigned short *)g.out_t + b * g.t_batch_stride + tok;
#pragma unroll
                for (int r = 0; r < 4; ++r) o[(on - g.t_col0 + r) * g.ldt] = T::from_f(v[r]);
            }
        }
    }
}

constexpr int ZC = 8;
template <class T>
__global__ __launch_bounds__(256) void k_splitk_epilogue_plain(const GemmArgs g)
{
    const int64_t nq = g.N / 4;
    for (int64_t q = (int64_t)blockIdx.x * 256 + threadIdx.x; q < g.M * nq; q += (int64_t)gridDim.x * 256) {
        const int64_t m = q / nq, n = (q - m * nq) * 4;
        float v[4] = {0.f, 0.f, 0.f, 0.f};
        const uint2 rpre = g.residual ? *reinterpret_cast<const uint2 *>((const unsigned char *)g.residual + (m * g.ldr + n) * 2) : make_uint2(0u, 0u);
        for (int z0 = 0; z0 < g.splits; z0 += ZC) {
            float4 a[ZC];
#pragma unroll
            for (int u = 0; u < ZC; ++u)
                if (z0 + u < g.splits) a[u] = *reinterpret_cast<const float4 *>(g.ws + ((int64_t)(z0 + u) * g.M + m) * g.N + n);
#pragma unroll
            for (int u = 0; u < ZC; ++u)
                if (z0 + u < g.splits) { v[0] += a[u].x; v[1] += a[u].y; v[2] += a[u].z; v[3] += a[u].w; }
        }
        float gate[4] = {0.f, 0.f, 0.f, 0.f};
        epilogue_store<T>(g, m, n, n, v, gate, &rpre);
    }
}

template <class T>
__global__ __launch_bounds__(256) void k_splitk_epilogue(const GemmArgs g)
{
    __shared__ float red[GS_MAXG * 2];
    constexpr int RPB = 16;
    const int64_t nq = g.N / 4;
    const int cl = threadIdx.x & 63, rl = threadIdx.x >> 6;
    const int64_t cq = (int64_t)blockIdx.x * 64 + cl;
    const int64_t m0 = (int64_t)blockIdx.y * RPB;
    const bool okc = cq < nq;
    const int64_t n = (okc ? cq : 0) * 4;
    if (g.out_group_stats) {
        if (threadIdx.x < GS_MAXG * 2) red[threadIdx.x] = 0.f;
        __syncthreads();
    }
    float v[4][4];
#pragma unroll
    for (int i = 0; i < 4; ++i) { v[i][0] = 0.f; v[i][1] = 0.f; v[i][2] = 0.f; v[i][3] = 0.f; }
    if (okc) {
        for (int z0 = 0; z0 < g.splits; z0 += ZC / 2) {
            float4 a[ZC / 2][4];
#pragma unroll
            for (int u = 0; u < ZC / 2; ++u)
#pragma unroll
                for (int i = 0; i < 4; ++i) {
                    const int64_t m = m0 + rl + 4 * i;
                    if (z0 + u < g.splits && m < g.M) a[u][i] = *reinterpret_cast<const float4 *>(g.ws + ((int64_t)(z0 + u) * g.M + m) * g.N + n);
                }
#pragma unroll
            for (int u = 0; u < ZC / 2; ++u)
#pragma unroll
                for (int i = 0; i < 4; ++i) {
                    const int64_t m = m0 + rl + 4 * i;
                    if (z0 + u < g.splits && m < g.M) { v[i][0] += a[u][i].x; v[i][1] += a[u][i].y; v[i][2] += a[u][i].z; v[i][3] += a[u][i].w; }
                }
        }
    }
    float cs[8] = {0.f, 0.f, 0.f, 0.f, 0.f, 0.f, 0.f, 0.f};
#pragma unroll
    for (int i = 0; i < 4; ++i) {
        const int64_t m = m0 + rl + 4 * i;
        if (m >= g.M) break;
        if (okc) {
            float gate[4] = {0.f, 0.f, 0.f, 0.f};
            epilogue_store<T>(g, m, n, n, v[i], gate);
        }
        if (g.out_row_stats) {
            const float a = wave_sum_f(okc ? (v[i][0] + v[i][1]) + (v[i][2] + v[i][3]) : 0.f);
            const float b = wave_sum_f(okc ? (v[i][0] * v[i][0] + v[i][1] * v[i][1]) + (v[i][2] * v[i][2] + v[i][3] * v[i][3]) : 0.f);
            if (cl == 0) *reinterpret_cast<float2 *>(g.out_row_stats + ((int64_t)blockIdx.x * g.M + m) * 2) = make_float2(a, b);
        }
        if (okc) {
#pragma unroll
            for (int r = 0; r < 4; ++r) { cs[2 * r] += v[i][r]; cs[2 * r + 1] += v[i][r] * v[i][r]; }
        }
    }
    if (g.out_group_stats) {
        if (okc) {
#pragma unroll
            for (int r = 0; r < 4; ++r) {
                const int gi = (int)(n + r) / g.gn_cpg;
                __hip_atomic_fetch_add(red + 2 * gi, cs[2 * r], __ATOMIC_RELAXED, __HIP_MEMORY_SCOPE_WORKGROUP);
                __hip_atomic_fetch_add(red + 2 * gi + 1, cs[2 * r + 1], __ATOMIC_RELAXED, __HIP_MEMORY_SCOPE_WORKGROUP);
            }
        }
        __syncthreads();
        if (threadIdx.x < GS_MAXG * 2) {
            const float t = red[threadIdx.x];
            if (t != 0.f) unsafeAtomicAdd(g.out_group_stats + (m0 / g.rows_per_batch) * g.gn_groups * 2 + threadIdx.x, t);
        }
    }
}


constexpr int CS_RB = 32;
template <class T>
__global__ __launch_bounds__(256) void k_splitk_epilogue_cs(const GemmArgs g)
{
    __shared__ float red[16][16][8];
    constexpr int RPT = CS_RB / 16;
    const int64_t nq = g.N / 4;
    const int cl = threadIdx.x & 15, rl = threadIdx.x >> 4;
    const int64_t cq4 = (int64_t)blockIdx.x * 16 + cl;
    const int64_t m0 = (int64_t)blockIdx.y * CS_RB;
    const bool okc = cq4 < nq;
    const int64_t n = (okc ? cq4 : 0) * 4;
    float cs[8] = {0.f, 0.f, 0.f, 0.f, 0.f, 0.f, 0.f, 0.f};
    float v[RPT][4];
#pragma unroll
    for (int i = 0; i < RPT; ++i) { v[i][0] = 0.f; v[i][1] = 0.f; v[i][2] = 0.f; v[i][3] = 0.f; }
    if (okc) {
        uint2 rpre[RPT];
#pragma unroll
        for (int i = 0; i < RPT; ++i) {
            const int64_t m = m0 + rl + 16 * i;
            rpre[i] = (g.residual && m < g.M) ? *reinterpret_cast<const uint2 *>((const unsigned char *)g.residual + (m * g.ldr + n) * 2) : make_uint2(0u, 0u);
        }
        for (int z0 = 0; z0 < g.splits; z0 += ZC) {
            float4 a[ZC][RPT];
#pragma unroll
            for (int u = 0; u < ZC; ++u)
#pragma unroll
                for (int i = 0; i < RPT; ++i) {
                    const int64_t m = m0 + rl + 16 * i;
                    if (z0 + u < g.splits && m < g.M) a[u][i] = *reinterpret_cast<const float4 *>(g.ws + ((int64_t)(z0 + u) * g.M + m) * g.N + n);
                }
#pragma unroll
            for (int u = 0; u < ZC; ++u)
#pragma unroll
                for (int i = 0; i < RPT; ++i) {
                    const int64_t m = m0 + rl + 16 * i;
                    if (z0 + u < g.splits && m < g.M) { v[i][0] += a[u][i].x; v[i][1] += a[u][i].y; v[i][2] += a[u][i].z; v[i][3] += a[u][i].w; }
                }
        }
#pragma unroll
        for (int i = 0; i < RPT; ++i) {
            const int64_t m = m0 + rl + 16 * i;
            if (m >= g.M) break;
            float gate[4] = {0.f, 0.f, 0.f, 0.f};
            epilogue_store<T>(g, m, n, n, v[i], gate, &rpre[i]);
#pragma unroll
            for (int r = 0; r < 4; ++r) { cs[2 * r] += v[i][r]; cs[2 * r + 1] += v[i][r] * v[i][r]; }
        }
    }
#pragma unroll
    for (int j = 0; j < 8; ++j) red[rl][cl][j] = cs[j];
    __syncthreads();
    __shared__ float chs[64][2];
    if (threadIdx.x < 128) {
        const int c2 = threadIdx.x >> 3, j = threadIdx.x & 7;
        float o = 0.f;
#pragma unroll
        for (int r = 0; r < 16; ++r) o += red[r][c2][j];
        chs[c2 * 4 + (j >> 1)][j & 1] = o;
    }
    __syncthreads();
    if (m0 < g.M) {
        const int cpg = g.gn_cpg, G = (int)(g.N / cpg);
        const int n_base = (int)blockIdx.x * 64, n_hi = n_base + 64 < (int)g.N ? n_base + 64 : (int)g.N;
        const int g_first = n_base / cpg, ng = (n_hi - 1) / cpg - g_first + 1;
        if ((int)threadIdx.x < ng) {
            const int gg = g_first + threadIdx.x;
            const int c_lo = gg * cpg > n_base ? gg * cpg : n_base, c_hi = (gg + 1) * cpg < n_hi ? (gg + 1) * cpg : n_hi;
            float s1 = 0.f, s2 = 0.f;
            for (int c = c_lo; c < c_hi; ++c) { s1 += chs[c - n_base][0]; s2 += chs[c - n_base][1]; }
            const int64_t b = m0 / g.rows_per_batch, slab = (m0 - b * g.rows_per_batch) / CS_RB;
            const int half = gg * cpg < n_base ? 1 : 0;
            *reinterpret_cast<float2 *>(g.chan_parts + ((((b * g.cp_nslab + slab) * G + gg) * 2 + half) * 2)) = make_float2(s1, s2);
        }
    }
}


inline bool fuse_of(const GemmArgs &g) { return g.row_stats || g.out_row_stats || g.out_group_stats; }

template <class F>
void with_wave_tile(int ntw, int mt, F &&f)
{
    const auto with_mt = [&](auto ntw_) {
        if (mt == 4) f(ntw_, std::integral_constant<int, 4>{}); else if (mt == 3) f(ntw_, std::integral_constant<int, 3>{}); else f(ntw_, std::integral_constant<int, 2>{});
    };
    if (ntw == 5) with_mt(std::integral_constant<int, 5>{}); else with_mt(std::integral_constant<int, 4>{});
}

template <class T, int MODE, int NTW, bool FUSE>
void launch4(const GemmArgs &g, dim3 grid, hipStream_t s)
{
    constexpr size_t lds = 2 * (BM * 128 + 32 * NTW * 128);
    static gc::AttrOnce once;
    gc::ensure_dynamic_lds(once, (const void *)k_gemm<T, MODE, NTW, FUSE>, (int)lds);
    hipLaunchKernelGGL((k_gemm<T, MODE, NTW, FUSE>), grid, dim3(NT), lds, s, g);
}

template <class T, int MODE, int NTW, int MT, bool FUSE, bool CS = false, bool LEAN = false, int LNV = 0>
void launch8(const GemmArgs &g, dim3 grid, hipStream_t s)
{
    constexpr size_t lds = 3 * (64 * MT * 128 + 32 * NTW * 128) + ((FUSE || LNV >= 2) ? 64 * MT * 8 : 0) + (CS ? 32 * NTW * 16 : 0);
    static_assert(lds <= 160 * 1024, "LDS ring");
    static gc::AttrOnce once;
    gc::ensure_dynamic_lds(once, (const void *)k_gemm8<T, MODE, NTW, MT, FUSE, CS, LEAN, LNV>, (int)lds);
    hipLaunchKernelGGL((k_gemm8<T, MODE, NTW, MT, FUSE, CS, LEAN, LNV>), grid, dim3(512), lds, s, g);
}

inline bool ln_lean_producer_of(const GemmArgs &g, int mode, int splits)
{
    return g.out_row_stats && !g.row_stats && !g.out_group_stats && !g.chan_parts && splits == 1 && mode == 0 && g.K % 64 == 0 && !g.geglu &&
           g.act == 0 && !g.out_f32 && !g.out_t && g.out && g.N >= 4 && (!g.rowvec || g.rows_per_batch >= 256);
}
inline bool ln_lean_consumer_of(const GemmArgs &g, int mode, int splits)
{
    return g.row_stats && !g.out_row_stats && !g.out_group_stats && !g.chan_parts && splits == 1 && mode == 0 && g.K % 64 == 0 && g.N >= 4;
}
template <class T, int NTW, int MT>
void dispatch8ln_m(const GemmArgs &g, int lnv, bool lean, dim3 grid, hipStream_t s)
{
    if (lnv == 3) { if constexpr (NTW == 5) launch8<T, 3, 5, MT, false, false, false, 3>(g, grid, s); return; }
    if (lnv == 1) launch8<T, 3, NTW, MT, false, false, true, 1>(g, grid, s);
    else if (lean) launch8<T, 3, NTW, MT, false, false, true, 2>(g, grid, s);
    else launch8<T, 3, NTW, MT, false, false, false, 2>(g, grid, s);
}
template <class T>
void dispatch8ln(const GemmArgs &g, int lnv, bool lean, int ntw, int mt, dim3 grid, hipStream_t s)
{
    if (lnv == 2 && g.persist > 0 && ntw == 4 && mt == 4) { launch8p<T, 4, 4, 2>(g, g.persist, s); return; }
    if (mt == 1 && ntw == 4) { dispatch8ln_m<T, 4, 1>(g, lnv, lean, grid, s); return; }
    with_wave_tile(ntw, mt, [&](auto ntw_, auto mt_) { dispatch8ln_m<T, decltype(ntw_)::value, decltype(mt_)::value>(g, lnv, lean, grid, s); });
}

inline bool lean_of(const GemmArgs &g, int mode)
{
    return !g.geglu && g.act == 0 && !g.out_f32 && !g.out_t && g.out && mode != 1 && (mode != 0 || g.K % 64 == 0) && g.N >= 4 &&
           (!g.rowvec || g.rows_per_batch >= 256);
}
template <class T, int NTW, int MT>
void dispatch8lean_m(const GemmArgs &g, int mode, dim3 grid, hipStream_t s)
{
    if (mode == 0) launch8<T, 3, NTW, MT, false, false, true>(g, grid, s);
    else if (g.ups) launch8<T, 4, NTW, MT, false, false, true>(g, grid, s);
    else launch8<T, 2, NTW, MT, false, false, true>(g, grid, s);
}
template <class T>
void dispatch8lean(const GemmArgs &g, int mode, int ntw, int mt, dim3 grid, hipStream_t s)
{
    if (mt == 1 && ntw == 4 && mode == 0) { launch8<T, 3, 4, 1, false, false, true>(g, grid, s); return; }
    with_wave_tile(ntw, mt, [&](auto ntw_, auto mt_) { dispatch8lean_m<T, decltype(ntw_)::value, decltype(mt_)::value>(g, mode, grid, s); });
}

template <class T, int NTW, int MT>
void dispatch8cs_m(const GemmArgs &g, int mode, dim3 grid, hipStream_t s)
{
    if (mode == 0) launch8<T, 3, NTW, MT, false, true>(g, grid, s);
    else if (mode == 1) launch8<T, 1, NTW, MT, false, true>(g, grid, s);
    else launch8<T, 2, NTW, MT, false, true>(g, grid, s);
}
template <class T>
void dispatch8cs(const GemmArgs &g, int mode, int ntw, int mt, dim3 grid, hipStream_t s)
{
    with_wave_tile(ntw, mt, [&](auto ntw_, auto mt_) { dispatch8cs_m<T, decltype(ntw_)::value, decltype(mt_)::value>(g, mode, grid, s); });
}

template <class T, int NTW, int MT, bool FUSE>
void dispatch8m(const GemmArgs &g, int mode, dim3 grid, hipStream_t s)
{
    if constexpr (FUSE) {
        if (mode == 0) launch8<T, 3, NTW, MT, true>(g, grid, s);
        else if (mode == 1) launch8<T, 1, NTW, MT, true>(g, grid, s);
        else launch8<T, 2, NTW, MT, true>(g, grid, s);
    } else {
        if (mode == 0) { if (g.K % 64 == 0) launch8<T, 3, NTW, MT, false>(g, grid, s); else launch8<T, 0, NTW, MT, false>(g, grid, s); }
        else if (mode == 1) launch8<T, 1, NTW, MT, false>(g, grid, s);
        else if (g.ups) launch8<T, 4, NTW, MT, false>(g, grid, s); else launch8<T, 2, NTW, MT, false>(g, grid, s);
    }
}
template <class T, bool FUSE>
void dispatch8(const GemmArgs &g, int mode, int ntw, int mt, dim3 grid, hipStream_t s)
{
    if constexpr (!FUSE) {
        if (mt == 1 && ntw == 4 && mode == 0 && g.K % 64 == 0) { launch8<T, 3, 4, 1, false>(g, grid, s); return; }
        if (g.persist > 0 && ntw == 4 && mt == 4 && mode == 0) { launch8p<T, 4, 4>(g, g.persist, s); return; }
    }
    with_wave_tile(ntw, mt, [&](auto ntw_, auto mt_) { dispatch8m<T, decltype(ntw_)::value, decltype(mt_)::value, FUSE>(g, mode, grid, s); });
}

template <class T, bool FUSE>
void dispatch4(const GemmArgs &g, int mode, int ntw, dim3 grid, hipStream_t s)
{
    if (ntw == 5) {
        if (mode == 0) launch4<T, 0, 5, FUSE>(g, grid, s); else if (mode == 1) launch4<T, 1, 5, FUSE>(g, grid, s); else launch4<T, 2, 5, FUSE>(g, grid, s);
    } else {
        if (mode == 0) launch4<T, 0, 4, FUSE>(g, grid, s); else if (mode == 1) launch4<T, 1, 4, FUSE>(g, grid, s); else launch4<T, 2, 4, FUSE>(g, grid, s);
    }
}

}

using dng::GemmArgs;
void dn_gemm_launch_plain(const GemmArgs &g, int dtype, int mode, int ntw, int mt8, dim3 grid, hipStream_t s);
void dn_gemm_launch_fuse(const GemmArgs &g, int dtype, int mode, int ntw, int mt8, dim3 grid, hipStream_t s);
void dn_gemm_launch_fp8(const GemmArgs &g, int dtype, int mode, int ntw, int mt, dim3 grid, hipStream_t s);
void dn_gemm_launch_splitk_epilogue(const GemmArgs &g, int dtype, hipStream_t s);
void dn_gemm_launch_cs(const GemmArgs &g, int dtype, int mode, int ntw, int mt8, dim3 grid, hipStream_t s);
void dn_gemm_launch_splitk_epilogue_cs(const GemmArgs &g, int dtype, hipStream_t s);
void dn_gemm_launch_lean(const GemmArgs &g, int dtype, int mode, int ntw, int mt8, dim3 grid, hipStream_t s);
void dn_gemm_launch_ln(const GemmArgs &g, int dtype, int lnv, bool lean, int ntw, int mt8, dim3 grid, hipStream_t s);
```

gaussctrl_amd/sd/ops.py:

```python
from __future__ import annotations

import ctypes as C
import dataclasses
import os
import sys
import types

import torch

from .. import _lib as L


class GemmDesc(C.Structure):
    _fields_ = [("dtype", C.c_int), ("mode", C.c_int), ("M", C.c_int64), ("N", C.c_int64), ("K", C.c_int64),
                ("A", C.c_void_p), ("lda", C.c_int64),
                ("B", C.c_int), ("Hi", C.c_int), ("Wi", C.c_int), ("Cin", C.c_int), ("Ho", C.c_int), ("Wo", C.c_int),
                ("stride", C.c_int), ("upsample", C.c_int), ("pad_lo", C.c_int),
                ("W", C.c_void_p), ("bias", C.c_void_p), ("rowvec", C.c_void_p), ("ld_rowvec", C.c_int64),
                ("rows_per_batch", C.c_int64), ("residual", C.c_void_p), ("ldr", C.c_int64), ("out_scale", C.c_float),
                ("act", C.c_int), ("geglu", C.c_int), ("out", C.c_void_p), ("ldc", C.c_int64), ("out_f32", C.c_int),
                ("out_t", C.c_void_p), ("ldt", C.c_int64), ("t_batch_stride", C.c_int64), ("t_col0", C.c_int64),
                ("workspace", C.c_void_p), ("workspace_bytes", C.c_size_t), ("zeros", C.c_void_p),
                ("ln_row_stats", C.c_void_p), ("ln_row_stat_slots", C.c_int), ("ln_colsum", C.c_void_p), ("ln_eps", C.c_float),
                ("out_row_stats", C.c_void_p), ("out_group_stats", C.c_void_p), ("gn_groups", C.c_int),
                ("fp8", C.c_int), ("w_scale", C.c_void_p), ("a_scale", C.c_int),
                ("kernel_variant", C.c_int), ("out_chan_parts", C.c_void_p), ("plan_rows", C.c_int64), ("out_fp8", C.c_int),
                ("w_set_rows", C.c_int64), ("w_set_stride", C.c_int64), ("softmax_keys", C.c_int)]


class AttnDesc(C.Structure):
    _fields_ = [("dtype", C.c_int), ("batch", C.c_int), ("heads", C.c_int), ("head_dim", C.c_int), ("Lq", C.c_int),
                ("Lk", C.c_int), ("frames_per_half", C.c_int), ("nsets", C.c_int), ("set_kind", C.c_int * 5),
                ("set_weight", C.c_float * 5), ("scale", C.c_float),
                ("Q", C.c_void_p), ("ldq", C.c_int64), ("q_batch_stride", C.c_int64),
                ("K", C.c_void_p), ("ldk", C.c_int64), ("k_batch_stride", C.c_int64),
                ("Vt", C.c_void_p), ("ldvt", C.c_int64), ("vt_batch_stride", C.c_int64),
                ("O", C.c_void_p), ("ldo", C.c_int64), ("o_batch_stride", C.c_int64),
                ("Kref", C.c_void_p), ("kref_batch_stride", C.c_int64), ("Vtref", C.c_void_p),
                ("vtref_batch_stride", C.c_int64), ("ref_frames_per_half", C.c_int), ("q_prescaled", C.c_int),
                ("kernel_variant", C.c_int), ("workspace", C.c_void_p), ("workspace_bytes", C.c_size_t)]


class GemmSelection(C.Structure):
    _fields_ = [(n, C.c_int) for n in ("kernel", "m_tiles", "splits", "ntw", "parts", "ln_kind", "persist")]


GEMM_KERNELS = {1: "k4", 2: "k8", 3: "k8_sliced", 4: "fp8"}
ATTN_KERNELS = {1: "attn5", 2: "attn4", 3: "attn3", 4: "wide+combine", 5: "attn+combine", 6: "attn"}

GC_GEMM_VAR_MT_MASK, GC_GEMM_VAR_MT_SHIFT = 0x7, 0
GC_GEMM_VAR_K4_ONLY, GC_GEMM_VAR_FORCE_K8, GC_GEMM_VAR_NO_CONV_SLICES, GC_GEMM_VAR_NO_SMALL_CONV_SLICES = 0x10, 0x20, 0x40, 0x80
GC_GEMM_VAR_NO_WG2, GC_GEMM_VAR_NO_PERSIST, GC_GEMM_VAR_FULL_EPILOGUE, GC_GEMM_VAR_NO_LEAN_LN, GC_GEMM_VAR_TAP_OUTER = 0x100, 0x200, 0x400, 0x800, 0x1000
GC_GEMM_VAR_PW_MASK, GC_GEMM_VAR_PW_SHIFT = 0xff0000, 16
GC_GEMM_VAR_SLICE_MT_MASK, GC_GEMM_VAR_SLICE_MT_SHIFT = 0x7000000, 24
GC_GEMM_VAR_EPI_ABL_MASK, GC_GEMM_VAR_EPI_ABL_SHIFT = 0x70000000, 28
GC_ATTN_VAR_ONLINE_ONLY, GC_ATTN_VAR_D40_K3, GC_ATTN_VAR_K4_8WAVE, GC_ATTN_VAR_K4_Q64, GC_ATTN_VAR_K4 = 1, 2, 4, 8, 16
GC_ATTN_VAR_RING4, GC_ATTN_VAR_RING8, GC_ATTN_VAR_D160_Q64 = 32, 64, 128
GC_ATTN_VAR_ABL_MASK, GC_ATTN_VAR_ABL_SHIFT = 0xff00, 8
GC_ATTN_VAR_CSHIFT_MASK, GC_ATTN_VAR_CSHIFT_SHIFT = 0x1f0000, 16


def gemm_selection(d):
    sel = GemmSelection()
    L.check(L.lib().gc_dn_gemm_selection(C.byref(d), C.byref(sel)), "gc_dn_gemm_selection")
    r = {n: getattr(sel, n) for n, _ in GemmSelection._fields_}
    r["kernel"] = GEMM_KERNELS[sel.kernel]
    return r


def attention_selection(d):
    k = C.c_int(0)
    L.check(L.lib().gc_dn_attention_selection(C.byref(d), C.byref(k)), "gc_dn_attention_selection")
    return ATTN_KERNELS[k.value]


SELECTION_LOG = None


@dataclasses.dataclass
class KernelOptions:
    gemm_variant: int = 0
    attn_variant: int = 0
    batch_invariant: bool = False
    fused_head: bool = True
    fused_tail: bool = True
    two_streams: bool = True
    gn_parts: bool = True
    tail_in_rows: bool = True
    q_only: bool = True
    ffout_merge: bool = True
    text_fold: bool = True
    cfg_share: bool = True
    fp8_min_hw: int = 256
    ablate: frozenset = frozenset()


OPTIONS = KernelOptions()


def configure(options: KernelOptions | None = None, **kw) -> KernelOptions:
    global OPTIONS
    if options is not None:
        OPTIONS = options
    if kw:
        OPTIONS = dataclasses.replace(OPTIONS, **kw)
    return OPTIONS


def options_from_env(env=None) -> KernelOptions:
    e = os.environ if env is None else env
    on = lambda k, d: e.get(k, d) not in ("", "0")
    field = lambda k, mask, shift, bias=0: ((int(e[k]) + bias) << shift) & mask if e.get(k, "") != "" else 0
    g = field("GC_GEMM_MT", GC_GEMM_VAR_MT_MASK, GC_GEMM_VAR_MT_SHIFT)
    g |= {"0": GC_GEMM_VAR_K4_ONLY, "2": GC_GEMM_VAR_FORCE_K8}.get(e.get("GC_GEMM8"), 0)
    g |= {"0": GC_GEMM_VAR_NO_CONV_SLICES, "1": GC_GEMM_VAR_NO_SMALL_CONV_SLICES}.get(e.get("GC_GEMM_CONVSPLIT"), 0)
    dbg = int(e.get("GC_GEMM_DBG", "0"))
    dbg_bits = (GC_GEMM_VAR_NO_WG2, GC_GEMM_VAR_NO_PERSIST, GC_GEMM_VAR_FULL_EPILOGUE, GC_GEMM_VAR_NO_LEAN_LN, GC_GEMM_VAR_TAP_OUTER)
    if dbg < 0 or dbg >> len(dbg_bits):
        raise ValueError(f"GC_GEMM_DBG={dbg}: an OR of 1 (no two-workgroup linears), 2 (no persistent GEMM), 4 (full epilogue), 8 (no lean LayerNorm fold), 16 (tap-outer convs)")
    g |= sum(b for i, b in enumerate(dbg_bits) if dbg >> i & 1)
    g |= field("GC_GEMM_EPI_ABL", GC_GEMM_VAR_EPI_ABL_MASK, GC_GEMM_VAR_EPI_ABL_SHIFT)
    g |= field("GC_GEMM_SPLIT_MT", GC_GEMM_VAR_SLICE_MT_MASK, GC_GEMM_VAR_SLICE_MT_SHIFT)
    g |= field("GC_GEMM_PW", GC_GEMM_VAR_PW_MASK, GC_GEMM_VAR_PW_SHIFT, 1)
    a = (GC_ATTN_VAR_ONLINE_ONLY if on("GC_ATTN_SAFE", "0") else 0) | (GC_ATTN_VAR_D40_K3 if on("GC_ATTN_16", "0") else 0)
    a |= int(e.get("GC_ATTN_V", "0")) * GC_ATTN_VAR_K4_8WAVE
    return KernelOptions(gemm_variant=g, attn_variant=a, batch_invariant=on("GC_BATCH_INVARIANT", "0"),
                         fused_head=on("GC_FUSED_HEAD", "1"), fused_tail=on("GC_FUSED_TAIL", "1"), two_streams=on("GC_DN_STREAMS", "1"),
                         gn_parts=on("GC_GN_PARTS", "1"), cfg_share=on("GC_CFG_SHARE", "1"), text_fold=on("GC_TEXT_FOLD", "1"), ffout_merge=on("GC_FFOUT_MERGE", "1"), q_only=on("GC_Q_ONLY", "1"), tail_in_rows=on("GC_TAIL_INROWS", "1"),
                         ablate=frozenset(x for x in e.get("GC_ABLATE", "").split(",") if x))


class _CompatNames(types.ModuleType):
    @property
    def KERNEL_VARIANT(self):
        return {"gemm": OPTIONS.gemm_variant, "attn": OPTIONS.attn_variant}

    @property
    def BATCH_INVARIANT(self):
        return OPTIONS.batch_invariant

    @BATCH_INVARIANT.setter
    def BATCH_INVARIANT(self, on):
        configure(batch_invariant=bool(on))


sys.modules[__name__].__class__ = _CompatNames


DT = {torch.bfloat16: 0, torch.float16: 1}
_abl_cache = {}


def _ablated(cls, shape, dtype, device):
    if cls not in OPTIONS.ablate:
        return None
    key = (cls, tuple(shape), dtype, device, stream_handle())
    t = _abl_cache.get(key)
    if t is None:
        t = _abl_cache[key] = torch.zeros(tuple(shape), dtype=dtype, device=device)
    return t


def _dt(t):
    try:
        return DT[t.dtype]
    except KeyError:
        raise L.GaussCtrlHipError(f"denoise kernels take bf16 / f16 activations, got {t.dtype}")


def _p(t):
    return None if t is None else C.c_void_p(t.data_ptr())


def _gpu(*ts):
    for t in ts:
        if t is not None and not t.is_cuda:
            raise L.GaussCtrlHipError("denoise ops need GPU tensors (HIP path only; no CPU fallback)")


_raw_stream = getattr(torch._C, "_cuda_getCurrentRawStream", None)


def stream_handle():
    if _raw_stream is not None:
        return _raw_stream(torch.cuda.current_device())
    return torch.cuda.current_stream().cuda_stream


def _stream():
    return C.c_void_p(stream_handle())


_zero_page = {}


class ChanParts:
    __slots__ = ("buf", "rows", "nslab", "mode", "col_tile", "groups")

    def __init__(self, buf, rows, nslab, mode, col_tile, groups):
        self.buf, self.rows, self.nslab, self.mode, self.col_tile, self.groups = buf, rows, nslab, mode, col_tile, groups


class RowStats:
    __slots__ = ("buf", "slots")

    def __init__(self):
        self.buf, self.slots = None, 0


DEBUG_FILL = None


def _run_gemm(d, dev, what, row_stats=None, want_parts=False, gn_groups=32):
    lib = L.lib()
    z = _zero_page.get(dev)
    if z is None:
        z = _zero_page[dev] = torch.zeros(64, dtype=torch.uint8, device=dev)
    d.zeros = z.data_ptr()
    d.kernel_variant = OPTIONS.gemm_variant
    wsb = lib.gc_dn_gemm_workspace_bytes(C.byref(d))
    ws = None
    if wsb:
        ws = torch.empty(wsb, dtype=torch.uint8, device=dev)
        d.workspace = ws.data_ptr(); d.workspace_bytes = wsb
    if row_stats is not None:
        row_stats.slots = int(lib.gc_dn_gemm_row_stat_slots(C.byref(d)))
        row_stats.buf = torch.empty(row_stats.slots, d.M, 2, dtype=torch.float32, device=dev)
        if DEBUG_FILL is not None:
            row_stats.buf.fill_(DEBUG_FILL)
        d.out_row_stats = row_stats.buf.data_ptr()
    parts = None
    if want_parts and d.rows_per_batch >= 256:
        rows, ns, ct = C.c_int64(0), C.c_int(0), C.c_int(0)
        d.gn_groups = gn_groups
        L.check(lib.gc_dn_gemm_chan_parts_layout(C.byref(d), C.byref(rows), C.byref(ns), C.byref(ct)), "gc_dn_gemm_chan_parts_layout")
        if 0 < rows.value and ns.value <= 64:
            parts = ChanParts(torch.empty(d.M // d.rows_per_batch, ns.value, gn_groups, 2, 2, dtype=torch.float32, device=dev), rows.value, ns.value,
                              0, ct.value, gn_groups)
            if DEBUG_FILL is not None:
                parts.buf.fill_(DEBUG_FILL)
            d.out_chan_parts = parts.buf.data_ptr()
        else:
            d.gn_groups = 0
    if SELECTION_LOG is not None:
        SELECTION_LOG.append(("gemm", d.M, gemm_selection(d)))
    L.check(lib.gc_dn_gemm(C.byref(d), _stream()), what)
    return parts


def _stats_args(d, ln, group_stats):
    if ln is not None:
        d.ln_row_stats = ln[0].buf.data_ptr(); d.ln_row_stat_slots = ln[0].slots; d.ln_colsum = ln[1].data_ptr(); d.ln_eps = ln[2]
    if group_stats is not None:
        d.out_group_stats = group_stats.data_ptr(); d.gn_groups = group_stats.shape[-2]


def linear(x, w, bias=None, residual=None, act=0, geglu=False, out_f32=False, scale=1.0, rowvec=None, rows_per_batch=0,
           ld_rowvec=None, out=None, want_out=True, out_t=None, ldt=0, t_batch_stride=0, t_col0=0, out_cols=None,
           ln=None, row_stats=None, group_stats=None, chan_parts=False, gn_groups=32, w_set_rows=0, softmax_keys=0):
    _gpu(x, w)
    K = x.shape[-1]
    M = x.numel() // K
    N = w.shape[-2]
    lda = x.stride(-2) if x.dim() > 1 else K
    d = GemmDesc()
    d.dtype = _dt(x); d.mode = 0; d.M, d.N, d.K = M, N, K
    d.A = x.data_ptr(); d.lda = lda; d.W = w.data_ptr()
    d.bias = None if bias is None else bias.data_ptr()
    if w_set_rows:
        assert w.dim() == 3 and w.is_contiguous() and (bias is None or bias.shape == (w.shape[0], N)) and M == w.shape[0] * w_set_rows
        d.w_set_rows = int(w_set_rows); d.w_set_stride = N * K
    d.softmax_keys = int(softmax_keys)
    if rowvec is not None:
        d.rowvec = rowvec.data_ptr(); d.ld_rowvec = rowvec.stride(0) if ld_rowvec is None else ld_rowvec
    d.rows_per_batch = rows_per_batch
    if OPTIONS.batch_invariant and x.dim() >= 3:
        d.plan_rows = M // x.shape[0]
    No = N // 2 if geglu else (N if out_cols is None else out_cols)
    if OPTIONS.ablate and out is None and row_stats is None and M >= 256:
        z = _ablated("linear", x.shape[:-1] + (No,), torch.float32 if out_f32 else x.dtype, x.device)
        z = _ablated(f"linear_k{K}", x.shape[:-1] + (No,), torch.float32 if out_f32 else x.dtype, x.device) if z is None else z
        if z is not None:
            return ((z if want_out else None), None) if chan_parts else (z if want_out else None)
    if residual is not None:
        d.residual = residual.data_ptr(); d.ldr = residual.stride(-2)
    d.out_scale = scale; d.act = act; d.geglu = int(geglu)
    if want_out:
        if out is None:
            out = torch.empty(x.shape[:-1] + (No,), dtype=torch.float32 if out_f32 else x.dtype, device=x.device)
        d.out = out.data_ptr(); d.ldc = out.stride(-2); d.out_f32 = int(out_f32)
    if out_t is not None:
        d.out_t = out_t.data_ptr(); d.ldt = ldt; d.t_batch_stride = t_batch_stride; d.t_col0 = t_col0
    _stats_args(d, ln, group_stats)
    parts = _run_gemm(d, x.device, "gc_dn_gemm", row_stats, want_parts=chan_parts and not OPTIONS.batch_invariant, gn_groups=gn_groups)
    return (out, parts) if chan_parts else out


def conv3x3(x, w, bias=None, stride=1, upsample=False, rowvec=None, ld_rowvec=None, residual=None, act=0, scale=1.0,
            out_f32=False, pad_lo=1, group_stats=None, chan_parts=False, gn_groups=32):
    _gpu(x, w)
    B, H, W_, Cin = x.shape
    Hin, Win = (2 * H, 2 * W_) if upsample else (H, W_)
    Ho, Wo = (Hin + pad_lo + 1 - 3) // stride + 1, (Win + pad_lo + 1 - 3) // stride + 1
    N = w.shape[0]
    if OPTIONS.ablate:
        z = _ablated("conv", (B, Ho, Wo, N), torch.float32 if out_f32 else x.dtype, x.device)
        z = _ablated(f"conv_hw{Ho}", (B, Ho, Wo, N), torch.float32 if out_f32 else x.dtype, x.device) if z is None else z
        if z is not None:
            return (z, None) if chan_parts else z
    out = torch.empty(B, Ho, Wo, N, dtype=torch.float32 if out_f32 else x.dtype, device=x.device)
    d = GemmDesc()
    d.dtype = _dt(x); d.mode = 1; d.M, d.N, d.K = B * Ho * Wo, N, 9 * Cin
    d.A = x.data_ptr(); d.lda = Cin
    d.B, d.Hi, d.Wi, d.Cin, d.Ho, d.Wo, d.stride, d.upsample = B, H, W_, Cin, Ho, Wo, stride, int(upsample)
    d.pad_lo = pad_lo
    d.W = w.data_ptr(); d.bias = None if bias is None else bias.data_ptr()
    if rowvec is not None:
        d.rowvec = rowvec.data_ptr(); d.ld_rowvec = rowvec.stride(0) if ld_rowvec is None else ld_rowvec
    d.rows_per_batch = Ho * Wo
    if OPTIONS.batch_invariant:
        d.plan_rows = Ho * Wo
    if residual is not None:
        d.residual = residual.data_ptr(); d.ldr = N
    d.out_scale = scale; d.act = act
    d.out = out.data_ptr(); d.ldc = N; d.out_f32 = int(out_f32)
    _stats_args(d, None, group_stats)
    parts = _run_gemm(d, x.device, "gc_dn_gemm(conv3x3)", want_parts=chan_parts and not OPTIONS.batch_invariant, gn_groups=gn_groups)
    return (out, parts) if chan_parts else out


_gn_ws = {}


def groupnorm(x, gamma, beta, groups, eps, silu, parts=None):
    _gpu(x)
    B, Cc = x.shape[0], x.shape[-1]
    HW = x.numel() // (B * Cc)
    if OPTIONS.ablate:
        z = _ablated("gn", x.shape, x.dtype, x.device)
        if z is not None:
            return z
    if parts is not None:
        assert parts.groups == groups
        y = torch.empty_like(x)
        L.check(L.lib().gc_dn_groupnorm_apply_parts(_dt(x), _p(x), _p(y), C.c_int64(B), C.c_int64(HW), Cc, groups, _p(gamma), _p(beta), C.c_float(eps),
                                                    int(silu), _p(parts.buf), C.c_int64(parts.rows), parts.nslab, parts.mode, parts.col_tile, _stream()),
                "gc_dn_groupnorm_apply_parts")
        return y
    key = (x.device, B, HW, Cc, stream_handle())
    ws = _gn_ws.get(key)
    if ws is None:
        nbytes = L.lib().gc_dn_groupnorm_workspace_bytes(C.c_int64(B), C.c_int64(HW), Cc)
        ws = _gn_ws[key] = torch.empty(nbytes // 4, dtype=torch.float32, device=x.device)
    y = torch.empty_like(x)
    L.check(L.lib().gc_dn_groupnorm(_dt(x), _p(x), _p(y), C.c_int64(B), C.c_int64(HW), Cc, groups, _p(gamma), _p(beta),
                                    C.c_float(eps), int(silu) | (0x100 if OPTIONS.batch_invariant else 0), _p(ws), _stream()), "gc_dn_groupnorm")
    return y


def groupnorm_apply(x, group_stats, gamma, beta, groups, eps, silu):
    _gpu(x, group_stats)
    chan_stats = group_stats
    B, Cc = x.shape[0], x.shape[-1]
    HW = x.numel() // (B * Cc)
    y = torch.empty_like(x)
    L.check(L.lib().gc_dn_groupnorm_apply(_dt(x), _p(x), _p(y), C.c_int64(B), C.c_int64(HW), Cc, groups, _p(gamma), _p(beta),
                                          C.c_float(eps), int(silu), _p(chan_stats), _stream()), "gc_dn_groupnorm_apply")
    return y


def pad128(c):
    return (c + 127) // 128 * 128


def groupnorm_apply_fp8(x, group_stats, gamma, beta, groups, eps, silu, a_scale=127):
    _gpu(x, group_stats)
    B, Cc = x.shape[0], x.shape[-1]
# ... 308 lines not shown
```

include/gaussctrl_hip.h:

```cpp
#ifndef GAUSSCTRL_HIP_H
#define GAUSSCTRL_HIP_H

#include <stddef.h>
#include <stdint.h>

#ifdef __cplusplus
extern "C" {
#endif

#define GC_OK 0
#define GC_EINVAL (-1)
#define GC_ELAUNCH (-2)
#define GC_ENOSPC (-3)

const char *gc_last_error_string(void);
int gc_abi_version(void);


int gc_project_gaussians_fwd(int64_t N, const float *means3d, const float *scales, float glob_scale,
                             const float *quats, const float *viewmat, const float *projmat,
                             float fx, float fy, float cx, float cy, int img_h, int img_w,
                             int tiles_x, int tiles_y, float clip_thresh,
                             float *cov3d, float *xys, float *depths, int32_t *radii, float *conics,
                             int32_t *num_tiles_hit, void *stream);
// ... 46 lines not shown
                            int64_t *isect_ids_sorted, void *workspace, size_t workspace_bytes, void *stream);
int gc_raster_bin_tiles_boxes(int64_t N, int64_t M, const int32_t *count_dev, int32_t *overflow_dev,
                              const int32_t *depth_order, const int32_t *cum_sorted, const uint32_t *tile_boxes,
                              const float *depths, int tiles_x, int tiles_y, int32_t *gaussian_ids_sorted, int32_t *tile_bins,
                              int64_t *isect_ids_sorted, void *workspace, size_t workspace_bytes, void *stream);


int gc_rasterize_fwd(int img_h, int img_w, int tiles_x, int tiles_y,
                     const int32_t *gaussian_ids_sorted, const int32_t *tile_bins,
                     const float *xys, const float *conics, const float *colors, const float *opacities,
                     const float *extra, const float *background,
                     float *out_img, float *out_extra, float *final_Ts, int32_t *final_index, void *stream);

int gc_rasterize_bwd(int img_h, int img_w, int tiles_x, int tiles_y, int64_t N,
                     const int32_t *gaussian_ids_sorted, const int32_t *tile_bins,
                     const float *xys, const float *conics, const float *colors, const float *opacities,
                     const float *background, const float *final_Ts, const int32_t *final_index,
                     const float *v_out, const float *v_out_alpha,
                     float *v_xy, float *v_conic, float *v_colors, float *v_opacity, void *stream);
int gc_rasterize_bwd_clamped(int img_h, int img_w, int tiles_x, int tiles_y, int64_t N,
                             const int32_t *gaussian_ids_sorted, const int32_t *tile_bins,
                             const float *xys, const float *conics, const float *colors, const float *opacities,
                             const float *background, const float *final_Ts, const int32_t *final_index,
                             const float *v_out, const float *v_out_alpha, const float *pre_clamp,
                             float *v_xy, float *v_conic, float *v_colors, float *v_opacity, void *stream);

int gc_rasterize_nd_fwd(int img_h, int img_w, int tiles_x, int tiles_y, int channels,
                        const int32_t *gaussian_ids_sorted, const int32_t *tile_bins,
                        const float *xys, const float *conics, const float *colors, const float *opacities,
                        const float *background, float *out_img, float *final_Ts, int32_t *final_index, void *stream);
int gc_rasterize_nd_bwd(int img_h, int img_w, int tiles_x, int tiles_y, int64_t N, int channels,
                        const int32_t *gaussian_ids_sorted, const int32_t *tile_bins,
                        const float *xys, const float *conics, const float *colors, const float *opacities,
                        const float *background, const float *final_Ts, const int32_t *final_index,
                        const float *v_out, const float *v_out_alpha,
                        float *v_xy, float *v_conic, float *v_colors, float *v_opacity, void *stream);

int gc_project_sh_fwd(int64_t N, const float *means, const float *log_scales, const float *quats,
                      const float *opacity_logits, const float *features_dc, const float *features_rest,
                      int sh_degree, int degrees_to_use, const float *viewmat, const float *projmat,
                      const float *cam_origin, float fx, float fy, float cx, float cy, int img_h, int img_w,
                      int tiles_x, int tiles_y, float clip_thresh,
                      float *xys, float *depths, int32_t *radii, float *conics, int32_t *num_tiles_hit,
                      float *rgbs, float *opac, void *stream);
int gc_project_sh_fwd_boxes(int64_t N, const float *means, const float *log_scales, const float *quats,
                            const float *opacity_logits, const float *features_dc, const float *features_rest,
                            int sh_degree, int degrees_to_use, const float *viewmat, const float *projmat,
                            const float *cam_origin, float fx, float fy, float cx, float cy, int img_h, int img_w,
                            int tiles_x, int tiles_y, float clip_thresh, float *xys, float *depths, int32_t *radii,
                            float *conics, int32_t *num_tiles_hit, float *rgbs, float *opac, uint32_t *tile_boxes, void *stream);


int gc_project_sh_bwd(int64_t N, const float *means, const float *log_scales, const float *quats,
                      const float *opacity_logits, const float *rgbs,
                      int sh_degree, int degrees_to_use, const float *viewmat, const float *projmat,
                      const float *cam_origin, float fx, float fy, float cx, float cy, int img_h, int img_w,
                      const int32_t *radii, const float *conics,
                      const float *v_xy, const float *v_conic, const float *v_rgbs, const float *v_opac,
                      float *v_means, float *v_log_scales, float *v_quats, float *v_opacity_logits,
                      float *v_features_dc, float *v_features_rest, void *stream);
int gc_project_sh_bwd_accumulate(int64_t N, const float *means, const float *log_scales, const float *quats,
                      const float *opacity_logits, const float *rgbs,
                      int sh_degree, int degrees_to_use, const float *viewmat, const float *projmat,
                      const float *cam_origin, float fx, float fy, float cx, float cy, int img_h, int img_w,
                      const int32_t *radii, const float *conics,
                      const float *v_xy, const float *v_conic, const float *v_rgbs, const float *v_opac,
                      float *v_means, float *v_log_scales, float *v_quats, float *v_opacity_logits,
                      float *v_features_dc, float *v_features_rest, void *stream);

int gc_raster_finalize(int64_t num_pixels, float *out_img, float *out_extra, const float *final_Ts,
                       float *alpha, void *stream);
int gc_raster_finalize_into(int64_t num_pixels, const float *img_raw, float *img_clamped, float *out_extra,
                            const float *final_Ts, float *alpha, void *stream);

size_t gc_l1_ssim_workspace_bytes(int H, int W, int C);
int gc_l1_ssim_fwd_bwd(const float *pred, const float *target, int H, int W, int C, float lambda_, float grad_scale,
                       int valid_window, float *loss_sums, float *v_pred, void *workspace, size_t workspace_bytes, void *stream);
int gc_adam_step(float *param, const float *grad, float *exp_avg, float *exp_avg_sq, int64_t n, float lr, float beta1,
                 float beta2, float eps, int step, void *stream);

#define GC_VIEW_CAM_FLOATS 35

int gc_project_sh_fwd_views(int64_t N, int C, const float *means, const float *log_scales, const float *quats,
                            const float *opacity_logits, const float *features_dc, const float *features_rest,
                            int sh_degree, int degrees_to_use, const float *cams, int img_h, int img_w,
                            int tiles_x, int tiles_y, float clip_thresh, float *xys, float *depths, int32_t *radii,
                            float *conics, int32_t *num_tiles_hit, float *rgbs, float *opac, uint32_t *tile_boxes,
                            uint32_t *depth_pairs, void *stream);
int gc_project_sh_bwd_views(int64_t N, int C, int accumulate, const float *means, const float *log_scales, const float *quats,
                            const float *opacity_logits, const float *rgbs, int sh_degree, int degrees_to_use, const float *cams,
                            int img_h, int img_w, const int32_t *radii, const float *conics, const float *v_xy, const float *v_conic,
                            const float *v_rgbs, const float *v_opac, float *v_means, float *v_log_scales, float *v_quats,
                            float *v_opacity_logits, float *v_features_dc, float *v_features_rest, void *stream);
int gc_raster_scan_tiles_views(int64_t N, int C, const int32_t *num_tiles_hit, const int32_t *order, int32_t *cum_tiles_hit,
                               int32_t *count_dev, void *workspace, size_t workspace_bytes, int64_t ws_view_stride, void *stream);
size_t gc_raster_depth_order_views_workspace_bytes(int64_t N, int C);
int gc_raster_depth_order_views(int64_t N, int C, const float *depths, const int32_t *radii, const uint32_t *depth_pairs,
                                const int32_t *num_tiles_hit, int32_t *depth_order, int32_t *cum_sorted, int32_t *count_dev,
                                void *workspace, size_t workspace_bytes, void *stream);
size_t gc_raster_bin_views_workspace_bytes(int64_t M_cap, int C);
int gc_raster_bin_tiles_views(int64_t N, int C, int64_t M_cap, const int32_t *count_dev, int32_t *overflow_dev,
                              const int32_t *depth_order, const int32_t *cum_sorted, const uint32_t *tile_boxes, const float *depths,
                              int tiles_x, int tiles_y, int32_t *gaussian_ids_sorted, int32_t *tile_bins, int64_t *isect_ids_sorted,
                              void *workspace, size_t workspace_bytes, void *stream);
size_t gc_raster_order_boxes_views_workspace_bytes(int64_t N, int C);
int gc_raster_order_boxes_views(int64_t N, int C, const uint32_t *depth_pairs, const uint32_t *tile_boxes, int32_t *depth_order,
                                uint32_t *boxes_sorted, int32_t *cum_sorted, int32_t *count_dev, int32_t *visible_dev, void *workspace,
                                size_t workspace_bytes, void *stream);
int gc_raster_bin_sorted_views(int64_t N, int C, int64_t M_cap, const int32_t *count_dev, int32_t *overflow_dev, const int32_t *visible_dev,
                               const int32_t *depth_order, const uint32_t *boxes_sorted, const int32_t *cum_sorted, int tiles_x, int tiles_y,
                               int32_t *gaussian_ids_sorted, int32_t *tile_bins, void *workspace, size_t workspace_bytes, void *stream);
int gc_rasterize_fwd_views(int C, int64_t N, int64_t M_cap, int shared_opacities, int shared_background, int img_h, int img_w,
                           int tiles_x, int tiles_y, const int32_t *gaussian_ids_sorted, const int32_t *tile_bins, const float *xys,
                           const float *conics, const float *colors, const float *opacities, const float *extra,
                           const float *background, float *out_img, float *out_extra, float *final_Ts, int32_t *final_index,
                           void *stream);
int gc_rasterize_bwd_views(int C, int64_t N, int64_t M_cap, int shared_opacities, int shared_background, int img_h, int img_w,
                           int tiles_x, int tiles_y, const int32_t *gaussian_ids_sorted, const int32_t *tile_bins, const float *xys,
                           const float *conics, const float *colors, const float *opacities, const float *background,
                           const float *final_Ts, const int32_t *final_index, const float *v_out, const float *v_out_alpha,
                           const float *pre_clamp, float *v_xy, float *v_conic, float *v_colors, float *v_opacity, void *stream);
size_t gc_l1_ssim_views_workspace_bytes(int B, int H, int W, int C);
int gc_l1_ssim_fwd_bwd_views(int B, const float *pred, const float *target, int H, int W, int C, float lambda_, float grad_scale,
                             int valid_window, float *loss_out, float *v_pred, void *workspace, size_t workspace_bytes, void *stream);

int gc_rasterize_bwd_depth_views(int C, int64_t N, int64_t M_cap, int shared_opacities, int shared_background, int img_h, int img_w,
                                 int tiles_x, int tiles_y, const int32_t *gaussian_ids_sorted, const int32_t *tile_bins, const float *xys,
                                 const float *conics, const float *colors, const float *opacities, const float *background,
                                 const float *final_Ts, const int32_t *final_index, const float *v_out, const float *v_out_alpha,
                                 const float *pre_clamp, float *v_xy, float *v_conic, float *v_colors, float *v_opacity, const float *extra,
                                 const float *depth, const float *v_depth, float *v_extra, void *stream);
int gc_project_sh_bwd_depth_views(int64_t N, int C, int accumulate, const float *means, const float *log_scales, const float *quats,
                                  const float *opacity_logits, const float *rgbs, int sh_degree, int degrees_to_use, const float *cams,
                                  int img_h, int img_w, const int32_t *radii, const float *conics, const float *v_xy, const float *v_conic,
                                  const float *v_rgbs, const float *v_opac, float *v_means, float *v_log_scales, float *v_quats,
                                  float *v_opacity_logits, float *v_features_dc, float *v_features_rest, const float *v_depths,
                                  void *stream);
size_t gc_depth_l1_views_workspace_bytes(int B, int H, int W);
int gc_depth_l1_fwd_bwd_views(int B, const float *pred, const float *target, int H, int W, float grad_scale, float *loss_out, float *v_pred,
                              void *workspace, size_t workspace_bytes, void *stream);



enum { GC_GEMM_VAR_MT_MASK = 0x7, GC_GEMM_VAR_MT_SHIFT = 0,
       GC_GEMM_VAR_K4_ONLY = 0x10,
       GC_GEMM_VAR_FORCE_K8 = 0x20,
       GC_GEMM_VAR_NO_CONV_SLICES = 0x40,
       GC_GEMM_VAR_NO_SMALL_CONV_SLICES = 0x80,
       GC_GEMM_VAR_NO_WG2 = 0x100,
       GC_GEMM_VAR_NO_PERSIST = 0x200,
       GC_GEMM_VAR_FULL_EPILOGUE = 0x400,
       GC_GEMM_VAR_NO_LEAN_LN = 0x800,
       GC_GEMM_VAR_TAP_OUTER = 0x1000,
       GC_GEMM_VAR_PW_MASK = 0xff0000, GC_GEMM_VAR_PW_SHIFT = 16,
       GC_GEMM_VAR_SLICE_MT_MASK = 0x7000000, GC_GEMM_VAR_SLICE_MT_SHIFT = 24,
       GC_GEMM_VAR_EPI_ABL_MASK = 0x70000000, GC_GEMM_VAR_EPI_ABL_SHIFT = 28 };
typedef struct gc_gemm_desc {
    int dtype;
    int mode;
    int64_t M, N, K;
    const void *A;
    int64_t lda;
    int B, Hi, Wi, Cin, Ho, Wo, stride, upsample;
    int pad_lo;
    const void *W;
    const float *bias;
    const float *rowvec;
    int64_t ld_rowvec;
    int64_t rows_per_batch;
    const void *residual;
    int64_t ldr;
    float out_scale;
    int act;
    int geglu;
    void *out;
    int64_t ldc;
    int out_f32;
    void *out_t;
    int64_t ldt;
    int64_t t_batch_stride;
    int64_t t_col0;
    void *workspace;
    size_t workspace_bytes;
    const void *zeros;
    const float *ln_row_stats;
    int ln_row_stat_slots;
    const float *ln_colsum;
    float ln_eps;
    float *out_row_stats;
    float *out_group_stats;
    int gn_groups;
    int fp8;
    const void *w_scale;
    int a_scale;
    int kernel_variant;
    float *out_chan_parts;
    int64_t plan_rows;
    int out_fp8;
    int64_t w_set_rows, w_set_stride;
    int softmax_keys;
} gc_gemm_desc;
size_t gc_dn_gemm_workspace_bytes(const gc_gemm_desc *desc);
int gc_dn_gemm_row_stat_slots(const gc_gemm_desc *desc);
int gc_dn_gemm_chan_parts_layout(const gc_gemm_desc *desc, int64_t *rows_per_slab, int *nslab, int *col_tile);
enum { GC_GEMM_SEL_K4 = 1,
       GC_GEMM_SEL_K8 = 2,
       GC_GEMM_SEL_K8_SLICED = 3,
       GC_GEMM_SEL_FP8 = 4 };
typedef struct gc_gemm_selection {
    int kernel;
    int m_tiles;
    int splits;
    int ntw;
    int parts;
    int ln_kind;
    int persist;
} gc_gemm_selection;
int gc_dn_gemm_selection(const gc_gemm_desc *desc, gc_gemm_selection *out);
int gc_dn_gemm(const gc_gemm_desc *desc, void *stream);

enum { GC_ATTN_VAR_ONLINE_ONLY = 1,
       GC_ATTN_VAR_D40_K3 = 2,
       GC_ATTN_VAR_K4_8WAVE = 4,
       GC_ATTN_VAR_K4_Q64 = 8,
       GC_ATTN_VAR_K4 = 16,
       GC_ATTN_VAR_RING4 = 32, GC_ATTN_VAR_RING8 = 64,
       GC_ATTN_VAR_D160_Q64 = 128,
       GC_ATTN_VAR_ABL_MASK = 0xff00, GC_ATTN_VAR_ABL_SHIFT = 8,
       GC_ATTN_VAR_CSHIFT_MASK = 0x1f0000, GC_ATTN_VAR_CSHIFT_SHIFT = 16 };
typedef struct gc_attn_desc {
    int dtype;
    int batch, heads, head_dim;
    int Lq, Lk;
    int frames_per_half;
    int nsets;
    int set_kind[5];
    float set_weight[5];
    float scale;
    const void *Q; int64_t ldq, q_batch_stride;
    const void *K; int64_t ldk, k_batch_stride;
    const void *Vt; int64_t ldvt, vt_batch_stride;
    void *O; int64_t ldo, o_batch_stride;
    const void *Kref; int64_t kref_batch_stride;
    const void *Vtref; int64_t vtref_batch_stride;
    int ref_frames_per_half;
    int q_prescaled;
    int kernel_variant;
    void *workspace;
    size_t workspace_bytes;
} gc_attn_desc;
size_t gc_dn_attention_workspace_bytes(const gc_attn_desc *desc);
enum { GC_ATTN_SEL_K5 = 1,
       GC_ATTN_SEL_K4 = 2,
       GC_ATTN_SEL_K3 = 3,
       GC_ATTN_SEL_WIDE_SPLIT = 4,
       GC_ATTN_SEL_SPLIT = 5,
       GC_ATTN_SEL_ONLINE = 6 };
int gc_dn_attention_selection(const gc_attn_desc *desc, int *kernel);
int gc_dn_attention(const gc_attn_desc *desc, void *stream);

typedef struct gc_ttail_desc {
    int dtype;
    int channels, heads;
    int64_t M;
    int64_t rows_per_frame;
    int frames_per_half;
    int text_len;
    float ln_eps;
    const void *attn_out;
    const void *resid;
    const void *x_in;
    void *out;
    const void *w_a;
    const void *w_kv;
    const void *w_b;
    const float *params;
    int stop_after;
    int resid_fragment_layout;
    int64_t in_rows;
} gc_ttail_desc;
int gc_dn_transformer_tail(const gc_ttail_desc *desc, void *stream);
void gc_dn_transformer_tail_layout(int64_t *blocks_a, int64_t *blocks_kv, int64_t *blocks_b, int64_t *param_floats);

typedef struct gc_thead_desc {
    int dtype;
    int channels;
    int64_t M;
    int64_t rows_per_frame;
    float ln_eps;
    const void *x;
    const float *gn_coef;
    void *h;
    void *qk;
    void *vt;
    int64_t ldvt, vt_batch_stride;
    const void *w;
    const float *params;
    int h_fragment_layout;
} gc_thead_desc;
int gc_dn_transformer_head(const gc_thead_desc *desc, void *stream);

size_t gc_dn_groupnorm_workspace_bytes(int64_t B, int64_t HW, int C);
int gc_dn_groupnorm(int dtype, const void *x, void *y, int64_t B, int64_t HW, int C, int G, const float *gamma,
                    const float *beta, float eps, int act, float *stats_ws, void *stream);
int gc_dn_groupnorm_coef(int dtype, const void *x, int64_t B, int64_t HW, int C, int G, const float *gamma, const float *beta, float eps,
                         float *stats_ws, float *coef, void *stream);
int gc_dn_groupnorm_apply(int dtype, const void *x, void *y, int64_t B, int64_t HW, int C, int G, const float *gamma,
                          const float *beta, float eps, int act, const float *group_stats, void *stream);
int gc_dn_groupnorm_apply_fp8(int dtype, const void *x, void *y8, int64_t B, int64_t HW, int C, int C_padded, int G, const float *gamma,
                              const float *beta, float eps, int act, const float *group_stats, int a_scale, void *stream);
int gc_dn_group_stats(int dtype, const void *x, int64_t B, int64_t HW, int C, int G, float *group_stats, void *stream);
int gc_dn_layernorm(int dtype, const void *x, void *y, int64_t M, int C, const float *gamma, const float *beta,
                    float eps, void *stream);
int gc_dn_layernorm_fp8(int dtype, const void *x, void *y8, int64_t M, int C, const float *gamma, const float *beta,
                        float eps, int a_scale, void *stream);
int gc_dn_concat_add(int dtype, const void *a, int C1, const void *b, const void *c, int C2, void *out, int64_t M,
                     int64_t rows_per_batch, float *group_stats, int gn_groups, void *stream);

int gc_dn_groupnorm_apply_parts(int dtype, const void *x, void *y, int64_t B, int64_t HW, int C, int G, const float *gamma, const float *beta,
                                float eps, int act, const float *parts, int64_t rows_per_slab, int nslab, int slab_mode, int col_tile, void *stream);
int gc_dn_groupnorm_apply_parts_fp8(int dtype, const void *x, void *y8, int64_t B, int64_t HW, int C, int C_padded, int G, const float *gamma,
                                    const float *beta, float eps, int act, const float *parts, int64_t rows_per_slab, int nslab, int slab_mode,
                                    int col_tile, int a_scale, void *stream);
int gc_dn_groupnorm_coef_parts(int64_t B, int64_t HW, int C, int G, const float *gamma, const float *beta, float eps, const float *parts,
                               int64_t rows_per_slab, int nslab, int slab_mode, int col_tile, float *coef, void *stream);
int gc_dn_concat_parts_layout(int64_t rows_per_batch, int C, int gn_groups, int64_t *rows_per_slab, int *nslab, int *col_tile);
int gc_dn_concat_add_parts(int dtype, const void *a, int C1, const void *b, const void *c, int C2, void *out, int64_t M, int64_t rows_per_batch,
                           int gn_groups, float *parts, void *stream);
int gc_dn_axpby(int dtype, const void *a, float sa, const void *b, float sb, int act, void *out, int64_t n, void *stream);
int gc_dn_cast_f32(int dtype, const float *a, int act, void *out, int64_t n, void *stream);
int gc_dn_softmax_rows(int dtype, void *s, int64_t M, int64_t N, int64_t ld, float scale, void *stream);
int gc_dn_depth_to_disparity(int dtype, const float *depth, int64_t HW, void *out, unsigned *max_ws, void *stream);
int gc_dn_mask_composite(const float *edited, int ld_e, const float *unedited, const float *mask, float *out, int64_t HW,
                         void *stream);
int gc_dn_cfg_ddim_step(int dtype, const float *eps, int ld_eps, int64_t frames, int64_t HW, float guidance, int cfg,
                        float alpha_t, float alpha_prev, float *latents, void *xin, int nrep, void *stream);

#ifdef __cplusplus
}
#endif
#endif
```

Measured before the change: 10.80.

## Fuse split-K reduction into GEMM via per-tile ticket counters

Split-K GEMMs now keep a per-tile atomic ticket array at the head of the workspace. The last slice to finish a tile sums all partial slabs and runs the epilogue (including channel partials) inside the same kernel, so the separate split-K epilogue launch is skipped. The Python side also caches one workspace per device and stream with the tickets zeroed once, instead of allocating a fresh workspace per call. The cost is an extra fence, atomic and block sync per tile, plus a serial reduction tail on the last-arriving block. The old two-kernel path stays available behind a variant flag.

```diff
diff --git a/gaussctrl_amd/csrc/dn_gemm.hip b/gaussctrl_amd/csrc/dn_gemm.hip
--- a/gaussctrl_amd/csrc/dn_gemm.hip
+++ b/gaussctrl_amd/csrc/dn_gemm.hip
@@ -6,7 +6,7 @@
     int force_mt;
     int use8;
     int convsplit;
-    bool no_wg2, no_persist, full_epilogue, no_lean_ln, tap_outer;
+    bool no_wg2, no_persist, full_epilogue, no_lean_ln, tap_outer, two_kernel_reduce;
     int forced_pw, slice_mt, epi_abl;
     int undefined;
 };
@@ -15,12 +15,23 @@
     const auto bit = [kv](int b) { return (kv & b) != 0; };
     const auto field = [kv](int mask, int shift) { return (kv & mask) >> shift; };
     constexpr int flags = GC_GEMM_VAR_K4_ONLY | GC_GEMM_VAR_FORCE_K8 | GC_GEMM_VAR_NO_CONV_SLICES | GC_GEMM_VAR_NO_SMALL_CONV_SLICES | GC_GEMM_VAR_NO_WG2 |
-                          GC_GEMM_VAR_NO_PERSIST | GC_GEMM_VAR_FULL_EPILOGUE | GC_GEMM_VAR_NO_LEAN_LN | GC_GEMM_VAR_TAP_OUTER;
+                          GC_GEMM_VAR_NO_PERSIST | GC_GEMM_VAR_FULL_EPILOGUE | GC_GEMM_VAR_NO_LEAN_LN | GC_GEMM_VAR_TAP_OUTER | GC_GEMM_VAR_TWO_KERNEL_REDUCE;
     return {field(GC_GEMM_VAR_MT_MASK, GC_GEMM_VAR_MT_SHIFT), bit(GC_GEMM_VAR_K4_ONLY) ? 0 : bit(GC_GEMM_VAR_FORCE_K8) ? 2 : 1,
             bit(GC_GEMM_VAR_NO_CONV_SLICES) ? 0 : bit(GC_GEMM_VAR_NO_SMALL_CONV_SLICES) ? 1 : 2,
-            bit(GC_GEMM_VAR_NO_WG2), bit(GC_GEMM_VAR_NO_PERSIST), bit(GC_GEMM_VAR_FULL_EPILOGUE), bit(GC_GEMM_VAR_NO_LEAN_LN), bit(GC_GEMM_VAR_TAP_OUTER),
+            bit(GC_GEMM_VAR_NO_WG2), bit(GC_GEMM_VAR_NO_PERSIST), bit(GC_GEMM_VAR_FULL_EPILOGUE), bit(GC_GEMM_VAR_NO_LEAN_LN), bit(GC_GEMM_VAR_TAP_OUTER), bit(GC_GEMM_VAR_TWO_KERNEL_REDUCE),
             field(GC_GEMM_VAR_PW_MASK, GC_GEMM_VAR_PW_SHIFT), field(GC_GEMM_VAR_SLICE_MT_MASK, GC_GEMM_VAR_SLICE_MT_SHIFT), field(GC_GEMM_VAR_EPI_ABL_MASK, GC_GEMM_VAR_EPI_ABL_SHIFT),
             kv & ~(flags | GC_GEMM_VAR_MT_MASK | GC_GEMM_VAR_PW_MASK | GC_GEMM_VAR_SLICE_MT_MASK | GC_GEMM_VAR_EPI_ABL_MASK)};
+}
+
+size_t slab_bytes(const gc_gemm_desc *d, int splits) { return sizeof(float) * (size_t)splits * (size_t)d->M * (size_t)d->N; }
+bool has_ticket_head(const gc_gemm_desc *d, int splits) { return d->workspace && d->workspace_bytes >= GC_GEMM_TICKET_BYTES + slab_bytes(d, splits); }
+float *slabs_of(const gc_gemm_desc *d, int splits) { return (float *)((char *)d->workspace + (has_ticket_head(d, splits) ? GC_GEMM_TICKET_BYTES : 0)); }
+bool fixup_in_kernel(const gc_gemm_desc *d, bool two_kernel_reduce, int splits, int64_t tiles, int ntw)
+{
+    if (splits < 2 || two_kernel_reduce || d->ln_row_stats || d->out_row_stats || d->out_group_stats) return false;
+    if (!has_ticket_head(d, splits) || tiles > GC_GEMM_TICKET_WORDS) return false;
+    if (d->out_chan_parts && ntw == 5 && (d->gn_groups < 1 || d->N % d->gn_groups != 0 || 160 % (d->N / d->gn_groups) != 0)) return false;
+    return true;
 }
 
 int choose_splits(int64_t blocks, int nk)
@@ -116,11 +127,11 @@
         const GemmVariant v = decode_variant(d->kernel_variant);
         SelQ q;
         select_fp8(d, v, &q, true);
-        return q.splits > 1 ? sizeof(float) * (size_t)q.splits * (size_t)d->M * (size_t)d->N : 0;
+        return q.splits > 1 ? GC_GEMM_TICKET_BYTES + slab_bytes(d, q.splits) : 0;
     }
     int ntw, splits, tps;
     plan(d, &ntw, &splits, &tps);
-    return splits > 1 ? sizeof(float) * (size_t)splits * (size_t)d->M * (size_t)d->N : 0;
+    return splits > 1 ? GC_GEMM_TICKET_BYTES + slab_bytes(d, splits) : 0;
 }
 
 namespace {
@@ -266,6 +277,14 @@
 }
 }
 
+namespace {
+int64_t tiles_of(const gc_gemm_desc *d, const Sel &sel)
+{
+    const int64_t bm = sel.mt8 ? 64 * sel.mt8 : BM, bn = 32 * sel.ntw;
+    return ((d->M + bm - 1) / bm) * ((d->N + bn - 1) / bn);
+}
+}
+
 extern "C" int gc_dn_gemm_selection(const gc_gemm_desc *d, gc_gemm_selection *out)
 {
     GC_REQUIRE(d && out, "null argument");
@@ -279,6 +298,7 @@
         SelQ q;
         select_fp8(d, v, &q, false);
         out->kernel = GC_GEMM_SEL_FP8; out->m_tiles = q.mt; out->splits = q.splits; out->ntw = q.ntw;
+        out->fixup = fixup_in_kernel(d, v.two_kernel_reduce, q.splits, ((d->M + 64 * q.mt - 1) / (64 * q.mt)) * ((d->N + 32 * q.ntw - 1) / (32 * q.ntw)), q.ntw);
         if (d->out_chan_parts) {
             chan_parts_layout(d, v, Sel{}, &rows, &ns, &ct);
             out->parts = rows > 0 ? (q.splits > 1 ? 1 : 2) : -1;
@@ -289,6 +309,7 @@
     route(d, v, &r);
     out->kernel = !r.sel.mt8 ? GC_GEMM_SEL_K4 : r.sel.splits > 1 ? GC_GEMM_SEL_K8_SLICED : GC_GEMM_SEL_K8;
     out->m_tiles = r.sel.mt8; out->splits = r.sel.splits; out->ntw = r.sel.ntw; out->ln_kind = r.lnk; out->persist = r.persist;
+    out->fixup = fixup_in_kernel(d, v.two_kernel_reduce, r.sel.splits, tiles_of(d, r.sel), r.sel.ntw);
     if (d->out_chan_parts) {
         chan_parts_layout(d, v, r.sel, &rows, &ns, &ct);
         out->parts = rows > 0 ? (r.sel.splits > 1 ? 1 : 2) : -1;
@@ -361,6 +382,7 @@
     }
     hipStream_t s = gc::S(stream);
     g.zeros = d->zeros;
+    g.tickets = nullptr;
     if (d->fp8) {
         GC_REQUIRE(d->zeros && d->w_scale, "fp8: zeros page and per-row weight scales are required");
         GC_REQUIRE(d->K % 128 == 0, "fp8: K % 128 == 0");
@@ -371,16 +393,20 @@
         SelQ q;
         select_fp8(d, v, &q, false);
         const int ntw = q.ntw, mt = q.mt;
-        g.splits = q.splits; g.tiles_per_split = q.tps; g.ws = q.splits > 1 ? (float *)d->workspace : nullptr;
+        g.splits = q.splits; g.tiles_per_split = q.tps; g.ws = q.splits > 1 ? slabs_of(d, q.splits) : nullptr;
         GC_REQUIRE(!d->out_chan_parts || q.splits > 1 || (d->mode == 1 && !fuse_of(g)), "fp8: channel partials come from k-sliced problems and fast convs");
         const int64_t nbn_q = (d->N + 32 * ntw - 1) / (32 * ntw), nbm_q = (d->M + 64 * mt - 1) / (64 * mt);
         const dim3 gq((unsigned)(nbm_q * nbn_q), (unsigned)q.splits);
+        const bool fixup = fixup_in_kernel(d, v.two_kernel_reduce, q.splits, nbm_q * nbn_q, ntw);
+        g.tickets = fixup ? (unsigned *)d->workspace : nullptr;
         g.pw = pw_of(d, v, nbm_q, nbn_q, nbm_q * nbn_q * q.splits, 32, 64 * mt, 32 * ntw);
         dn_gemm_launch_fp8(g, d->dtype, d->mode == 1 ? 2 : 3, ntw, mt, gq, s);
-        if (q.splits > 1) { if (g.chan_parts) dn_gemm_launch_splitk_epilogue_cs(g, d->dtype, s); else dn_gemm_launch_splitk_epilogue(g, d->dtype, s); }
+        if (q.splits > 1 && !fixup) { if (g.chan_parts) dn_gemm_launch_splitk_epilogue_cs(g, d->dtype, s); else dn_gemm_launch_splitk_epilogue(g, d->dtype, s); }
         return gc::check_launch("gc_dn_gemm(fp8)");
     }
-    g.splits = sel.splits; g.tiles_per_split = sel.tps; g.ws = (float *)d->workspace;
+    g.splits = sel.splits; g.tiles_per_split = sel.tps; g.ws = sel.splits > 1 ? slabs_of(d, sel.splits) : nullptr;
+    const bool fixup = fixup_in_kernel(d, v.two_kernel_reduce, sel.splits, tiles_of(d, sel), sel.ntw);
+    g.tickets = fixup ? (unsigned *)d->workspace : nullptr;
     const int bn = 32 * sel.ntw;
     const int64_t nbn = (d->N + bn - 1) / bn;
     g.persist = rt.persist;
@@ -404,6 +430,6 @@
         g.pw = pw_of(d, v, nbm, nbn, nbm * nbn * sel.splits, 64, BM, bn);
         if (fuse_of(g)) dn_gemm_launch_fuse(g, d->dtype, sel.mode, sel.ntw, 0, grid, s); else dn_gemm_launch_plain(g, d->dtype, sel.mode, sel.ntw, 0, grid, s);
     }
-    if (sel.splits > 1) { if (g.chan_parts) dn_gemm_launch_splitk_epilogue_cs(g, d->dtype, s); else dn_gemm_launch_splitk_epilogue(g, d->dtype, s); }
+    if (sel.splits > 1 && !fixup) { if (g.chan_parts) dn_gemm_launch_splitk_epilogue_cs(g, d->dtype, s); else dn_gemm_launch_splitk_epilogue(g, d->dtype, s); }
     return gc::check_launch("gc_dn_gemm");
 }
diff --git a/gaussctrl_amd/csrc/dn_gemm_kernels.h b/gaussctrl_amd/csrc/dn_gemm_kernels.h
--- a/gaussctrl_amd/csrc/dn_gemm_kernels.h
+++ b/gaussctrl_amd/csrc/dn_gemm_kernels.h
@@ -18,6 +18,7 @@
     int splits; int tiles_per_split;
     int persist;
     float *ws;
+    unsigned *tickets;
     const void *zeros;
     const float *row_stats; int row_stat_slots; const float *colsum; float ln_eps, ln_inv_k;
     float *out_row_stats;
@@ -364,6 +365,175 @@
                 unsafeAtomicAdd(g.out_group_stats + ((b0 + sl) * g.gn_groups) * 2 + rem, v);
             }
         }
+    }
+}
+
+constexpr int ZC = 8;
+constexpr int CS_RB = 32;
+
+template <class T, int U, int ZCC>
+__device__ __forceinline__ void splitk_reduce_quads(const GemmArgs &g, const int64_t (&m)[U], const int64_t (&n)[U], const bool (&ok)[U])
+{
+    float v[U][4];
+    uint2 rpre[U];
+#pragma unroll
+    for (int u = 0; u < U; ++u) {
+        v[u][0] = 0.f; v[u][1] = 0.f; v[u][2] = 0.f; v[u][3] = 0.f;
+        rpre[u] = (g.residual && ok[u]) ? *reinterpret_cast<const uint2 *>((const unsigned char *)g.residual + (m[u] * g.ldr + n[u]) * 2) : make_uint2(0u, 0u);
+    }
+    for (int z0 = 0; z0 < g.splits; z0 += ZCC) {
+        float4 a[ZCC][U];
+#pragma unroll
+        for (int z = 0; z < ZCC; ++z)
+#pragma unroll
+            for (int u = 0; u < U; ++u)
+                if (z0 + z < g.splits && ok[u]) a[z][u] = *reinterpret_cast<const float4 *>(g.ws + ((int64_t)(z0 + z) * g.M + m[u]) * g.N + n[u]);
+#pragma unroll
+        for (int z = 0; z < ZCC; ++z)
+#pragma unroll
+            for (int u = 0; u < U; ++u)
+                if (z0 + z < g.splits && ok[u]) { v[u][0] += a[z][u].x; v[u][1] += a[z][u].y; v[u][2] += a[z][u].z; v[u][3] += a[z][u].w; }
+    }
+#pragma unroll
+    for (int u = 0; u < U; ++u)
+        if (ok[u]) {
+            float gate[4] = {0.f, 0.f, 0.f, 0.f};
+            epilogue_store<T>(g, m[u], n[u], n[u], v[u], gate, &rpre[u]);
+        }
+}
+
+template <class T, int NB, int ZCC>
+__device__ __forceinline__ void splitk_reduce_cs_block(const GemmArgs &g, int t, int64_t bx, int64_t m0, int64_t m_end, int64_t lim_lo, int64_t lim_hi, bool active,
+                                                       float *red, float *chs)
+{
+    constexpr int RPT = CS_RB / 16;
+    const int64_t nq = g.N / 4;
+    const int cl = t & 15, rl = t >> 4;
+    const int64_t cq4 = bx * 16 + cl;
+    const int64_t n = (cq4 < nq ? cq4 : 0) * 4;
+    const bool okc = active && cq4 < nq && n >= lim_lo && n < lim_hi;
+    float cs[NB][8];
+    float v[NB][RPT][4];
+#pragma unroll
+    for (int b = 0; b < NB; ++b) {
+#pragma unroll
+        for (int j = 0; j < 8; ++j) cs[b][j] = 0.f;
+#pragma unroll
+        for (int i = 0; i < RPT; ++i) { v[b][i][0] = 0.f; v[b][i][1] = 0.f; v[b][i][2] = 0.f; v[b][i][3] = 0.f; }
+    }
+    if (okc) {
+        uint2 rpre[NB][RPT];
+#pragma unroll
+        for (int b = 0; b < NB; ++b)
+#pragma unroll
+            for (int i = 0; i < RPT; ++i) {
+                const int64_t m = m0 + b * CS_RB + rl + 16 * i;
+                rpre[b][i] = (g.residual && m < m_end) ? *reinterpret_cast<const uint2 *>((const unsigned char *)g.residual + (m * g.ldr + n) * 2) : make_uint2(0u, 0u);
+            }
+        for (int z0 = 0; z0 < g.splits; z0 += ZCC) {
+            float4 a[ZCC][NB][RPT];
+#pragma unroll
+            for (int u = 0; u < ZCC; ++u)
+#pragma unroll
+                for (int b = 0; b < NB; ++b)
+#pragma unroll
+                    for (int i = 0; i < RPT; ++i) {
+                        const int64_t m = m0 + b * CS_RB + rl + 16 * i;
+                        if (z0 + u < g.splits && m < m_end) a[u][b][i] = *reinterpret_cast<const float4 *>(g.ws + ((int64_t)(z0 + u) * g.M + m) * g.N + n);
+                    }
+#pragma unroll
+            for (int u = 0; u < ZCC; ++u)
+#pragma unroll
+                for (int b = 0; b < NB; ++b)
+#pragma unroll
+                    for (int i = 0; i < RPT; ++i) {
+                        const int64_t m = m0 + b * CS_RB + rl + 16 * i;
+                        if (z0 + u < g.splits && m < m_end) { v[b][i][0] += a[u][b][i].x; v[b][i][1] += a[u][b][i].y; v[b][i][2] += a[u][b][i].z; v[b][i][3] += a[u][b][i].w; }
+                    }
+        }
+#pragma unroll
+        for (int b = 0; b < NB; ++b)
+#pragma unroll
+            for (int i = 0; i < RPT; ++i) {
+                const int64_t m = m0 + b * CS_RB + rl + 16 * i;
+                if (m >= m_end) break;
+                float gate[4] = {0.f, 0.f, 0.f, 0.f};
+                epilogue_store<T>(g, m, n, n, v[b][i], gate, &rpre[b][i]);
+#pragma unroll
+                for (int r = 0; r < 4; ++r) { cs[b][2 * r] += v[b][i][r]; cs[b][2 * r + 1] += v[b][i][r] * v[b][i][r]; }
+            }
+    }
+#pragma unroll
+    for (int b = 0; b < NB; ++b)
+#pragma unroll
+        for (int j = 0; j < 8; ++j) red[((b * 16 + rl) * 16 + cl) * 8 + j] = cs[b][j];
+    __syncthreads();
+    for (int idx = t; idx < NB * 128; idx += 256) {
+        const int b = idx >> 7, c2 = (idx >> 3) & 15, j = idx & 7;
+        float o = 0.f;
+#pragma unroll
+        for (int r = 0; r < 16; ++r) o += red[((b * 16 + r) * 16 + c2) * 8 + j];
+        chs[(b * 64 + c2 * 4 + (j >> 1)) * 2 + (j & 1)] = o;
+    }
+    __syncthreads();
+    if (active) {
+        const int cpg = g.gn_cpg, G = (int)(g.N / cpg);
+        const int n_base = (int)bx * 64, n_hi = n_base + 64 < (int)g.N ? n_base + 64 : (int)g.N;
+        const int g_first = n_base / cpg, ng = n_base < n_hi ? (n_hi - 1) / cpg - g_first + 1 : 0;
+        for (int idx = t; idx < NB * ng; idx += 256) {
+            const int b = idx / ng, gg = g_first + idx - b * ng;
+            const int64_t ms = m0 + (int64_t)b * CS_RB;
+            const int c_lo = gg * cpg > n_base ? gg * cpg : n_base, c_hi = (gg + 1) * cpg < n_hi ? (gg + 1) * cpg : n_hi;
+            if (ms >= m_end || c_lo < lim_lo || c_hi > lim_hi) continue;
+            float s1 = 0.f, s2 = 0.f;
+            for (int c = c_lo; c < c_hi; ++c) { s1 += chs[(b * 64 + c - n_base) * 2]; s2 += chs[(b * 64 + c - n_base) * 2 + 1]; }
+            const int64_t bt = ms / g.rows_per_batch, slab = (ms - bt * g.rows_per_batch) / CS_RB;
+            const int half = gg * cpg < n_base ? 1 : 0;
+            *reinterpret_cast<float2 *>(g.chan_parts + ((((bt * g.cp_nslab + slab) * G + gg) * 2 + half) * 2)) = make_float2(s1, s2);
+        }
+    }
+}
+
+template <class T, int NTHREADS, int INFL>
+__device__ __forceinline__ void sliced_fixup(const GemmArgs &g, int64_t tile, int64_t m_base, int bm, int64_t n_base, int bn, unsigned char *smem)
+{
+    __threadfence();
+    __syncthreads();
+    unsigned *flag = reinterpret_cast<unsigned *>(smem);
+    if (threadIdx.x == 0) *flag = __hip_atomic_fetch_add(g.tickets + tile, 1u, __ATOMIC_RELAXED, __HIP_MEMORY_SCOPE_AGENT);
+    __syncthreads();
+    if (*flag != (unsigned)(g.splits - 1)) return;
+    __threadfence();
+    if (threadIdx.x == 0) __hip_atomic_store(g.tickets + tile, 0u, __ATOMIC_RELAXED, __HIP_MEMORY_SCOPE_AGENT);
+    const int64_t m_end = m_base + bm < g.M ? m_base + bm : g.M, n_end = n_base + bn < g.N ? n_base + bn : g.N;
+    constexpr int ZCC = 4, U = INFL / ZCC;
+    if (!g.chan_parts) {
+        const int qn = bn / 4, total = bm * qn;
+        for (int q0 = threadIdx.x; q0 < total; q0 += NTHREADS * U) {
+            int64_t m[U], n[U];
+            bool ok[U];
+#pragma unroll
+            for (int u = 0; u < U; ++u) {
+                const int q = q0 + u * NTHREADS, r = q / qn;
+                m[u] = m_base + r; n[u] = n_base + (q - r * qn) * 4;
+                ok[u] = q < total && m[u] < m_end && n[u] < n_end;
+                if (!ok[u]) { m[u] = m_base; n[u] = n_base; }
+            }
+            splitk_reduce_quads<T, U, ZCC>(g, m, n, ok);
+        }
+        return;
+    }
+    constexpr int NB = U / 2, NGRP = NTHREADS / 256;
+    const int grp = threadIdx.x >> 8, t = threadIdx.x & 255;
+    float *red = reinterpret_cast<float *>(smem + 16) + grp * (NB * (16 * 16 * 8 + 64 * 2)), *chs = red + NB * 16 * 16 * 8;
+    const int64_t bx0 = n_base / 64, nbx = (n_end + 63) / 64 - bx0;
+    const int nrg = (int)((m_end - m_base + NB * CS_RB - 1) / (NB * CS_RB));
+    const int units = (int)nbx * nrg;
+    for (int u0 = 0; u0 < units; u0 += NGRP) {
+        const int u = u0 + grp;
+        const bool active = u < units;
+        const int rg = active ? u / (int)nbx : 0;
+        splitk_reduce_cs_block<T, NB, ZCC>(g, t, bx0 + (active ? u - rg * (int)nbx : 0), m_base + (int64_t)rg * (NB * CS_RB), m_end, n_base, n_end, active, red, chs);
     }
 }
 
@@ -556,6 +726,7 @@
                         make_float4(acc[nt][mt][0], acc[nt][mt][1], acc[nt][mt][2], acc[nt][mt][3]);
             }
         }
+        if (g.tickets) sliced_fixup<T, NT, 16>(g, mblk * nbn + nblk, m_base, BM, n_base, BN, smem);
         return;
     }
     float4 bia[NTW];
@@ -915,6 +1086,9 @@
                     *reinterpret_cast<float4 *>(g.ws + ((int64_t)slice * g.M + m) * g.N + n) =
                         make_float4(acc[nt][mt][0], acc[nt][mt][1], acc[nt][mt][2], acc[nt][mt][3]);
             }
+        }
+        if constexpr (MT >= 2 && !CS && LNV == 0) {
+            if (g.tickets) sliced_fixup<T, 512, (MT >= 3 ? 32 : 16)>(g, mblk * nbn + nblk, m_base, BM, n_base, BN, smem);
         }
         return;
     }
@@ -1612,6 +1786,9 @@
                         make_float4(acc[nt][mt][0], acc[nt][mt][1], acc[nt][mt][2], acc[nt][mt][3]);
             }
         }
+        if constexpr (!CS) {
+            if (g.tickets) sliced_fixup<T, 512, (MT >= 3 ? 32 : 16)>(g, mblk * nbn + nblk, m_base, BM, n_base, BN, smem);
+        }
         return;
     }
     if constexpr (CS) {
@@ -1790,26 +1967,14 @@
     }
 }
 
-constexpr int ZC = 8;
 template <class T>
 __global__ __launch_bounds__(256) void k_splitk_epilogue_plain(const GemmArgs g)
 {
     const int64_t nq = g.N / 4;
     for (int64_t q = (int64_t)blockIdx.x * 256 + threadIdx.x; q < g.M * nq; q += (int64_t)gridDim.x * 256) {
-        const int64_t m = q / nq, n = (q - m * nq) * 4;
-        float v[4] = {0.f, 0.f, 0.f, 0.f};
-        const uint2 rpre = g.residual ? *reinterpret_cast<const uint2 *>((const unsigned char *)g.residual + (m * g.ldr + n) * 2) : make_uint2(0u, 0u);
-        for (int z0 = 0; z0 < g.splits; z0 += ZC) {
-            float4 a[ZC];
-#pragma unroll
-            for (int u = 0; u < ZC; ++u)
-                if (z0 + u < g.splits) a[u] = *reinterpret_cast<const float4 *>(g.ws + ((int64_t)(z0 + u) * g.M + m) * g.N + n);
-#pragma unroll
-            for (int u = 0; u < ZC; ++u)
-                if (z0 + u < g.splits) { v[0] += a[u].x; v[1] += a[u].y; v[2] += a[u].z; v[3] += a[u].w; }
-        }
-        float gate[4] = {0.f, 0.f, 0.f, 0.f};
-        epilogue_store<T>(g, m, n, n, v, gate, &rpre);
+        const int64_t m[1] = {q / nq}, n[1] = {(q - m[0] * nq) * 4};
+        const bool ok[1] = {true};
+        splitk_reduce_quads<T, 1, ZC>(g, m, n, ok);
     }
 }
 
@@ -1887,82 +2052,12 @@
 }
 
 
-constexpr int CS_RB = 32;
 template <class T>
 __global__ __launch_bounds__(256) void k_splitk_epilogue_cs(const GemmArgs g)
 {
-    __shared__ float red[16][16][8];
-    constexpr int RPT = CS_RB / 16;
-    const int64_t nq = g.N / 4;
-    const int cl = threadIdx.x & 15, rl = threadIdx.x >> 4;
-    const int64_t cq4 = (int64_t)blockIdx.x * 16 + cl;
-    const int64_t m0 = (int64_t)blockIdx.y * CS_RB;
-    const bool okc = cq4 < nq;
-    const int64_t n = (okc ? cq4 : 0) * 4;
-    float cs[8] = {0.f, 0.f, 0.f, 0.f, 0.f, 0.f, 0.f, 0.f};
-    float v[RPT][4];
-#pragma unroll
-    for (int i = 0; i < RPT; ++i) { v[i][0] = 0.f; v[i][1] = 0.f; v[i][2] = 0.f; v[i][3] = 0.f; }
-    if (okc) {
-        uint2 rpre[RPT];
-#pragma unroll
-        for (int i = 0; i < RPT; ++i) {
-            const int64_t m = m0 + rl + 16 * i;
-            rpre[i] = (g.residual && m < g.M) ? *reinterpret_cast<const uint2 *>((const unsigned char *)g.residual + (m * g.ldr + n) * 2) : make_uint2(0u, 0u);
-        }
-        for (int z0 = 0; z0 < g.splits; z0 += ZC) {
-            float4 a[ZC][RPT];
-#pragma unroll
-            for (int u = 0; u < ZC; ++u)
-#pragma unroll
-                for (int i = 0; i < RPT; ++i) {
-                    const int64_t m = m0 + rl + 16 * i;
-                    if (z0 + u < g.splits && m < g.M) a[u][i] = *reinterpret_cast<const float4 *>(g.ws + ((int64_t)(z0 + u) * g.M + m) * g.N + n);
-                }
-#pragma unroll
-            for (int u = 0; u < ZC; ++u)
-#pragma unroll
-                for (int i = 0; i < RPT; ++i) {
-                    const int64_t m = m0 + rl + 16 * i;
-                    if (z0 + u < g.splits && m < g.M) { v[i][0] += a[u][i].x; v[i][1] += a[u][i].y; v[i][2] += a[u][i].z; v[i][3] += a[u][i].w; }
-                }
-        }
-#pragma unroll
-        for (int i = 0; i < RPT; ++i) {
-            const int64_t m = m0 + rl + 16 * i;
-            if (m >= g.M) break;
-            float gate[4] = {0.f, 0.f, 0.f, 0.f};
-            epilogue_store<T>(g, m, n, n, v[i], gate, &rpre[i]);
-#pragma unroll
-            for (int r = 0; r < 4; ++r) { cs[2 * r] += v[i][r]; cs[2 * r + 1] += v[i][r] * v[i][r]; }
-        }
-    }
-#pragma unroll
-    for (int j = 0; j < 8; ++j) red[rl][cl][j] = cs[j];
-    __syncthreads();
-    __shared__ float chs[64][2];
-    if (threadIdx.x < 128) {
-        const int c2 = threadIdx.x >> 3, j = threadIdx.x & 7;
-        float o = 0.f;
-#pragma unroll
-        for (int r = 0; r < 16; ++r) o += red[r][c2][j];
-        chs[c2 * 4 + (j >> 1)][j & 1] = o;
-    }
-    __syncthreads();
-    if (m0 < g.M) {
-        const int cpg = g.gn_cpg, G = (int)(g.N / cpg);
-        const int n_base = (int)blockIdx.x * 64, n_hi = n_base + 64 < (int)g.N ? n_base + 64 : (int)g.N;
-        const int g_first = n_base / cpg, ng = (n_hi - 1) / cpg - g_first + 1;
-        if ((int)threadIdx.x < ng) {
-            const int gg = g_first + threadIdx.x;
-            const int c_lo = gg * cpg > n_base ? gg * cpg : n_base, c_hi = (gg + 1) * cpg < n_hi ? (gg + 1) * cpg : n_hi;
-            float s1 = 0.f, s2 = 0.f;
-            for (int c = c_lo; c < c_hi; ++c) { s1 += chs[c - n_base][0]; s2 += chs[c - n_base][1]; }
-            const int64_t b = m0 / g.rows_per_batch, slab = (m0 - b * g.rows_per_batch) / CS_RB;
-            const int half = gg * cpg < n_base ? 1 : 0;
-            *reinterpret_cast<float2 *>(g.chan_parts + ((((b * g.cp_nslab + slab) * G + gg) * 2 + half) * 2)) = make_float2(s1, s2);
-        }
-    }
+    __shared__ float red[16 * 16 * 8];
+    __shared__ float chs[64 * 2];
+    splitk_reduce_cs_block<T, 1, ZC>(g, (int)threadIdx.x, blockIdx.x, (int64_t)blockIdx.y * CS_RB, g.M, 0, g.N, true, red, chs);
 }
 
 
diff --git a/gaussctrl_amd/sd/ops.py b/gaussctrl_amd/sd/ops.py
--- a/gaussctrl_amd/sd/ops.py
+++ b/gaussctrl_amd/sd/ops.py
@@ -42,7 +42,7 @@
 
 
 class GemmSelection(C.Structure):
-    _fields_ = [(n, C.c_int) for n in ("kernel", "m_tiles", "splits", "ntw", "parts", "ln_kind", "persist")]
+    _fields_ = [(n, C.c_int) for n in ("kernel", "m_tiles", "splits", "ntw", "parts", "ln_kind", "persist", "fixup")]
 
 
 GEMM_KERNELS = {1: "k4", 2: "k8", 3: "k8_sliced", 4: "fp8"}
@@ -51,7 +51,9 @@
 GC_GEMM_VAR_MT_MASK, GC_GEMM_VAR_MT_SHIFT = 0x7, 0
 GC_GEMM_VAR_K4_ONLY, GC_GEMM_VAR_FORCE_K8, GC_GEMM_VAR_NO_CONV_SLICES, GC_GEMM_VAR_NO_SMALL_CONV_SLICES = 0x10, 0x20, 0x40, 0x80
 GC_GEMM_VAR_NO_WG2, GC_GEMM_VAR_NO_PERSIST, GC_GEMM_VAR_FULL_EPILOGUE, GC_GEMM_VAR_NO_LEAN_LN, GC_GEMM_VAR_TAP_OUTER = 0x100, 0x200, 0x400, 0x800, 0x1000
-GC_GEMM_VAR_PW_MASK, GC_GEMM_VAR_PW_SHIFT = 0xff0000, 16
+GC_GEMM_VAR_PW_MASK, GC_GEMM_VAR_PW_SHIFT = 0x7f0000, 16
+GC_GEMM_VAR_TWO_KERNEL_REDUCE = 0x800000
+GC_GEMM_TICKET_BYTES = 4 * 4096
 GC_GEMM_VAR_SLICE_MT_MASK, GC_GEMM_VAR_SLICE_MT_SHIFT = 0x7000000, 24
 GC_GEMM_VAR_EPI_ABL_MASK, GC_GEMM_VAR_EPI_ABL_SHIFT = 0x70000000, 28
 GC_ATTN_VAR_ONLINE_ONLY, GC_ATTN_VAR_D40_K3, GC_ATTN_VAR_K4_8WAVE, GC_ATTN_VAR_K4_Q64, GC_ATTN_VAR_K4 = 1, 2, 4, 8, 16
@@ -121,6 +123,7 @@
     g |= sum(b for i, b in enumerate(dbg_bits) if dbg >> i & 1)
     g |= field("GC_GEMM_EPI_ABL", GC_GEMM_VAR_EPI_ABL_MASK, GC_GEMM_VAR_EPI_ABL_SHIFT)
     g |= field("GC_GEMM_SPLIT_MT", GC_GEMM_VAR_SLICE_MT_MASK, GC_GEMM_VAR_SLICE_MT_SHIFT)
+    g |= GC_GEMM_VAR_TWO_KERNEL_REDUCE if on("GC_GEMM_TWO_KERNEL_REDUCE", "0") else 0
     g |= field("GC_GEMM_PW", GC_GEMM_VAR_PW_MASK, GC_GEMM_VAR_PW_SHIFT, 1)
     a = (GC_ATTN_VAR_ONLINE_ONLY if on("GC_ATTN_SAFE", "0") else 0) | (GC_ATTN_VAR_D40_K3 if on("GC_ATTN_16", "0") else 0)
     a |= int(e.get("GC_ATTN_V", "0")) * GC_ATTN_VAR_K4_8WAVE
@@ -211,6 +214,18 @@
 DEBUG_FILL = None
 
 
+_gemm_ws = {}
+
+
+def _gemm_workspace(dev, nbytes):
+    key = (dev, stream_handle())
+    ws = _gemm_ws.get(key)
+    if ws is None or ws.numel() < nbytes:
+        ws = _gemm_ws[key] = torch.empty(nbytes, dtype=torch.uint8, device=dev)
+        ws[:GC_GEMM_TICKET_BYTES].zero_()
+    return ws
+
+
 def _run_gemm(d, dev, what, row_stats=None, want_parts=False, gn_groups=32):
     lib = L.lib()
     z = _zero_page.get(dev)
@@ -219,10 +234,9 @@
     d.zeros = z.data_ptr()
     d.kernel_variant = OPTIONS.gemm_variant
     wsb = lib.gc_dn_gemm_workspace_bytes(C.byref(d))
-    ws = None
     if wsb:
-        ws = torch.empty(wsb, dtype=torch.uint8, device=dev)
-        d.workspace = ws.data_ptr(); d.workspace_bytes = wsb
+        ws = _gemm_workspace(dev, wsb)
+        d.workspace = ws.data_ptr(); d.workspace_bytes = ws.numel()
     if row_stats is not None:
         row_stats.slots = int(lib.gc_dn_gemm_row_stat_slots(C.byref(d)))
         row_stats.buf = torch.empty(row_stats.slots, d.M, 2, dtype=torch.float32, device=dev)
diff --git a/include/gaussctrl_hip.h b/include/gaussctrl_hip.h
--- a/include/gaussctrl_hip.h
+++ b/include/gaussctrl_hip.h
@@ -222,9 +222,11 @@
        GC_GEMM_VAR_FULL_EPILOGUE = 0x400,
        GC_GEMM_VAR_NO_LEAN_LN = 0x800,
        GC_GEMM_VAR_TAP_OUTER = 0x1000,
-       GC_GEMM_VAR_PW_MASK = 0xff0000, GC_GEMM_VAR_PW_SHIFT = 16,
+       GC_GEMM_VAR_PW_MASK = 0x7f0000, GC_GEMM_VAR_PW_SHIFT = 16,
+       GC_GEMM_VAR_TWO_KERNEL_REDUCE = 0x800000,
        GC_GEMM_VAR_SLICE_MT_MASK = 0x7000000, GC_GEMM_VAR_SLICE_MT_SHIFT = 24,
        GC_GEMM_VAR_EPI_ABL_MASK = 0x70000000, GC_GEMM_VAR_EPI_ABL_SHIFT = 28 };
+enum { GC_GEMM_TICKET_WORDS = 4096, GC_GEMM_TICKET_BYTES = 4 * GC_GEMM_TICKET_WORDS };
 typedef struct gc_gemm_desc {
     int dtype;
     int mode;
@@ -285,6 +287,7 @@
     int parts;
     int ln_kind;
     int persist;
+    int fixup;
 } gc_gemm_selection;
 int gc_dn_gemm_selection(const gc_gemm_desc *desc, gc_gemm_selection *out);
 int gc_dn_gemm(const gc_gemm_desc *desc, void *stream);
```

Measured after the change: 9.913. 0.918x the previous value.
